# 30stomercury/whisper-char-alignment

Measured on AMD Instinct MI355X. Metric: utterances/sec (whisper-medium, 10s audio, char align) at 1/2/4/8 MI355X, higher is better.
Workload: dtype f16x2 (hi + lo operand pairs on the f16 MFMA pipe: fp32-equivalent operands, fp32 accumulate)

## Files before the change

### include/wca.h

```cpp
#ifndef WCA_H_
#define WCA_H_

#include <stdint.h>

#ifdef __cplusplus
extern "C" {
#endif

typedef struct wca_engine wca_engine;

typedef enum {
  WCA_STATUS_PARTITIONED = 1,
  WCA_OK = 0,
  WCA_ERR_INVALID = -1,
  WCA_ERR_TOO_LONG = -2,
  WCA_ERR_HIP = -3,
  WCA_ERR_STATE = -4,
  WCA_ERR_NOMEM = -5
} wca_status;

typedef struct {
  int32_t n_mels;
  int32_t n_audio_ctx;
  int32_t n_audio_state;
// ... 73 lines not shown
                    int32_t* jump_frame_host);
int wca_probe_strict_tp(wca_engine* e, int n_heads, const int32_t* word_end_row_host, int n_hyp, const double* ref_times_host, int n_ref,
                        const uint8_t* same_word_host, double tolerance, int32_t* tp_host);

int wca_align_batch(wca_engine* e, const float* pcm_dev, int64_t pcm_stride, const int32_t* n_samples_host,
                    const int64_t* tokens_dev, int n_tok_max, const int32_t* n_tok_host,
                    const int32_t* max_frames_host, int batch, const wca_align_opts* opts, int32_t* jump_frame_host,
                    int32_t* sel_idx_host);

typedef struct {
  int32_t sample_len;
  int32_t eot;
  int32_t timestamp_begin;
  int32_t apply_timestamp_rules;
  int32_t max_initial_timestamp_index;
  int32_t no_speech;
} wca_decode_opts;

typedef struct {
  int32_t sample_len;
  int32_t eot;
  int32_t timestamp_begin;
  int32_t apply_timestamp_rules;
  int32_t max_initial_timestamp_index;
  int32_t no_speech;
  int32_t sot_index;
  int32_t prefill;
} wca_decode_opts_ex;

int wca_encode_batch(wca_engine* e, const float* mel_dev, const float* pcm_dev, int64_t pcm_stride,
                     const int32_t* n_samples_host, int batch);

int wca_greedy_decode(wca_engine* e, const float* mel_dev, const float* pcm_dev, int64_t pcm_stride,
                      const int32_t* n_samples_host, int batch, const int32_t* initial_tokens_host, int n_initial,
                      const uint8_t* suppress_mask_host, const uint8_t* blank_mask_host, const wca_decode_opts* opts,
                      int32_t* tokens_out_host, int32_t* n_tokens_host, float* sum_logprob_host,
                      float* no_speech_prob_host);
int wca_greedy_decode_ex(wca_engine* e, const float* mel_dev, const float* pcm_dev, int64_t pcm_stride,
                         const int32_t* n_samples_host, int batch, const int32_t* initial_tokens_host, int n_initial,
                         const uint8_t* suppress_mask_host, const uint8_t* blank_mask_host, const wca_decode_opts_ex* opts,
                         int32_t* tokens_out_host, int32_t* n_tokens_host, float* sum_logprob_host,
                         float* no_speech_prob_host);
int wca_last_decode_positions(wca_engine* e, int32_t* prefill_positions, int32_t* step_positions);

int wca_align_batch_enqueue(wca_engine* e, const float* pcm_dev, int64_t pcm_stride, const int32_t* n_samples_host,
                            const int64_t* tokens_dev, int n_tok_max, const int32_t* n_tok_host,
                            const int32_t* max_frames_host, int batch, const wca_align_opts* opts);
int wca_align_batch_fetch(wca_engine* e, int batch, int n_tok_max, int topk, int32_t* jump_frame_host,
                          int32_t* sel_idx_host);

int wca_align_batch_enqueue_ex(wca_engine* e, const float* pcm_dev, int64_t pcm_stride, const int32_t* n_samples_host,
                               const int64_t* tokens_dev, int n_tok_max, const int32_t* n_tok_host,
                               const int32_t* max_frames_host, int batch, const wca_align_opts* opts, int32_t vocab_end);
int wca_align_batch_fetch_ex(wca_engine* e, int batch, int n_tok_max, int topk, int32_t* jump_frame_host,
                             int32_t* sel_idx_host, float* token_logprob_host);
int wca_token_logprobs(wca_engine* e, const float* logits_dev, int rows, int ld, int vocab_end, const int64_t* targets_dev,
                       float* out_dev);

int wca_flac_info(const uint8_t* buf, int64_t nbytes, int32_t* sample_rate, int32_t* channels, int32_t* bits_per_sample,
                  int64_t* total_samples);
int wca_flac_decode(const uint8_t* buf, int64_t nbytes, float* out, int64_t capacity_per_channel, int64_t* n_decoded);

#define WCA_COMM_ID_BYTES 128
int wca_comm_unique_id(uint8_t* id_out );
int wca_comm_init(wca_engine* e, const uint8_t* id , int rank, int world);
int wca_comm_destroy(wca_engine* e);
int wca_allgather_results(wca_engine* e, const uint8_t* packed_host, int64_t n_bytes, uint8_t* gathered_host,
                          int64_t capacity_per_rank, int64_t* sizes_host );
int wca_allreduce_counters(wca_engine* e, int64_t* counters_host , int n);
int wca_collate_plan(const int64_t* sizes , const int64_t* capacities , int world, int64_t* pad_out);

int wca_test_gemm(wca_engine* e, const void* a_f16_dev, const void* w_f16_dev, const float* bias_dev, void* c_dev, int M,
                  int N, int K, int gelu, int out_mode);
int wca_test_gemm_pairs(wca_engine* e, const void* a2_f16_dev, const void* w_f16_dev, const float* bias_dev, void* c_dev, int M,
                        int N, int K, int gelu, int out_mode);
int wca_test_gemm_ln(wca_engine* e, const void* a_f16_dev, const void* w_f16_dev, const float* bias_dev, float* x_dev,
                     const float* gamma_dev, const float* beta_dev, void* xn_f16_dev, int M, int N, int K, int site);
int wca_test_gemm_rows(wca_engine* e, const void* a_f16_dev, const float* x_f32_dev, const float* gamma_dev, const float* beta_dev,
                       const void* w_f16_dev, const float* bias_dev, void* c_dev, int M, int N, int K, int gelu, int out_mode, int splitk,
                       int groups, void* kv_k_f16_dev, void* kv_v_f16_dev, int T_max, int kv_t);
int wca_test_set_attn_split_drop(int mask);
int wca_test_set_switch(const char* name, int value);
int wca_test_last_scores(wca_engine* e, int batch, float* scores_host);
int wca_test_attention(wca_engine* e, const void* q_dev, const void* k_dev, const void* v_dev, void* o_dev,
                       float* cap_dev, int cap_ld, int cap_cols, int B, int H, int nq, int nk, int causal);
int wca_test_attention_split(wca_engine* e, const void* q2_dev, const void* k2_dev, const void* v2_dev, void* o2_dev,
                             float* cap_dev, int cap_ld, int cap_cols, int B, int H, int nq, int nk, int causal);
int wca_test_decode_select(wca_engine* e, const float* logits_dev, int batch, int n_vocab, int32_t* tokens_dev, int T_max,
                           int cur_len, int n_initial, const uint8_t* suppress_mask_dev, const uint8_t* blank_mask_dev,
                           const wca_decode_opts* opts, float* sum_logprob_dev, int32_t* n_done_dev);
int wca_test_layernorm(wca_engine* e, const float* x_dev, const float* g_dev, const float* b_dev, void* out_f16_dev,
                       int rows, int d);
int wca_test_layernorm_split(wca_engine* e, const float* x_dev, const float* g_dev, const float* b_dev, void* out2_f16_dev,
                             int rows, int d);
int wca_test_encoder(wca_engine* e, const float* mel_dev, int batch, float* xa_out_dev);

int wca_last_stage_ms(wca_engine* e, float* ms8);
enum {
  WCA_SITE_QKV = 0,
  WCA_SITE_ATTN = 1,
  WCA_SITE_OUT = 2,
  WCA_SITE_FC1 = 3,
  WCA_SITE_FC2 = 4,
  WCA_SITE_LN1 = 5,
  WCA_SITE_LN2 = 6,
  WCA_N_SITES = 7
};
int wca_last_kernel_ms(wca_engine* e, int site, int* n_launches, float* total_ms, double* flops_per_launch,
                       double* bytes_per_launch);
int wca_set_fuse_ln(wca_engine* e, int on);
enum { WCA_PRECISION_F16 = 0, WCA_PRECISION_SPLIT = 1, WCA_PRECISION_REFERENCE = 1 };
int wca_set_precision(wca_engine* e, int mode);
int wca_get_precision(wca_engine* e);
int wca_set_overlap(wca_engine* e, int on);
int wca_set_cu_partition(wca_engine* e, int phase2_cus);
int wca_set_decode_mode(wca_engine* e, int fused, int streams);
int wca_set_profiling(wca_engine* e, int on);

#ifdef __cplusplus
}
#endif
#endif
```

### whisper-char-alignment_amd/_lib.py

```python
import ctypes as C
import os

_HERE = os.path.dirname(os.path.abspath(__file__))
LIB_PATH = os.path.join(_HERE, "libwca.so")


class WcaError(RuntimeError):
    def __init__(self, code, msg):
        super().__init__("wca error %d: %s" % (code, msg))
        self.code = code


class TooLongError(WcaError):
    """n_tok > 448 or max_frames > 1500 (the skip condition of infer_ali.py:79)."""


class ModelDims(C.Structure):
    _fields_ = [(n, C.c_int32) for n in (
        "n_mels", "n_audio_ctx", "n_audio_state", "n_audio_head", "n_audio_layer",
        "n_vocab", "n_text_ctx", "n_text_state", "n_text_head", "n_text_layer")]


class AlignOpts(C.Structure):
    _fields_ = [("aggregation", C.c_int32), ("topk", C.c_int32), ("w_colnorm", C.c_float),
                ("w_rownorm", C.c_float), ("w_coverage", C.c_float), ("sot_len", C.c_int32),
                ("medfilt_width", C.c_int32), ("qk_scale", C.c_float)]


class DecodeOpts(C.Structure):
    _fields_ = [("sample_len", C.c_int32), ("eot", C.c_int32), ("timestamp_begin", C.c_int32),
                ("apply_timestamp_rules", C.c_int32), ("max_initial_timestamp_index", C.c_int32), ("no_speech", C.c_int32)]


class DecodeOptsEx(C.Structure):
    _fields_ = DecodeOpts._fields_ + [("sot_index", C.c_int32), ("prefill", C.c_int32)]


ERR_TOO_LONG = -2
AGGR_MEAN, AGGR_TOPK = 0, 1
PRECISION_SITES = ("logmel", "conv", "enc_gemm", "enc_attn", "cross_kv", "dec", "capture")
SITES = {"qkv": 0, "attention": 1, "out_proj": 2, "fc1": 3, "fc2": 4, "ln1": 5, "ln2": 6}
DTYPE_F32, DTYPE_F16 = 0, 1

_vp, _i, _i64, _f = C.c_void_p, C.c_int, C.c_int64, C.c_float
_pi32 = C.POINTER(C.c_int32)
_pf = C.POINTER(C.c_float)

SIGNATURES = {
    "wca_last_error": (C.c_char_p, []),
    "wca_version": (_i, []),
    "wca_engine_create": (_i, [C.POINTER(ModelDims), _i, _i, C.POINTER(_vp)]),
    "wca_engine_create_ex": (_i, [C.POINTER(ModelDims), _i, _i, _i, C.POINTER(_vp)]),
    "wca_engine_destroy": (None, [_vp]),
    "wca_engine_set_stream": (_i, [_vp, _vp]),
    "wca_engine_synchronize": (_i, [_vp]),
    "wca_load_weight": (_i, [_vp, C.c_char_p, _vp, _i, C.POINTER(_i64), _i]),
    "wca_finalize_weights": (_i, [_vp]),
    "wca_weights_inexact": (_i, [_vp, C.POINTER(C.c_longlong), C.POINTER(C.c_longlong), C.c_char_p, _i]),
    "wca_set_allow_rounded_weights": (_i, [_vp, _i]),
    "wca_log_mel": (_i, [_vp, _vp, _i64, _pi32, _i, _vp]),
    "wca_log_mel_long": (_i, [_vp, _vp, _i64, _vp, _i64, C.POINTER(_i64)]),
    "wca_mel_window": (_i, [_vp, _vp, _i64, _i64, _pi32, _pi32, _i, _vp]),
    "wca_get_attentions": (_i, [_vp, _vp, _vp, _i, _i, _pi32, _pi32, _i, _f, _vp, _vp]),
    "wca_median_filter": (_i, [_vp, _vp, _vp, _i64, _i, _i]),
    "wca_filter_attention": (_i, [_vp, _vp, _i, _i, _i, _i, _i, _f, _f, _f, _pf, _pi32, _pf]),
    "wca_force_align": (_i, [_vp, _vp, _i, _i, _i, _i, C.POINTER(AlignOpts), _pf, _pi32, _pi32, _pi32, _pi32, _pf]),
    "wca_default_find_alignment": (_i, [_vp, _vp, _i, _i, _i, _i, _pi32, _i, _i, _vp, _pf, _pi32, _pi32, _pi32]),
    "wca_attention_weights": (_i, [_vp, _vp, _i, _i, _i, _i, _i, _i, _f, _vp]),
    "wca_flac_info": (_i, [_vp, _i64, _pi32, _pi32, _pi32, C.POINTER(_i64)]),
    "wca_flac_decode": (_i, [_vp, _i64, _vp, _i64, C.POINTER(_i64)]),
    "wca_dtw": (_i, [_vp, _pf, _i, _i, _pi32, _pi32, _pi32]),
    "wca_dtw_batch_dev": (_i, [_vp, _vp, _i, _i, _i, _pi32]),
    "wca_probe_heads": (_i, [_vp, _vp, _i, _i, _i, _i, _i, _pf, _pi32]),
    "wca_align_batch": (_i, [_vp, _vp, _i64, _pi32, _vp, _i, _pi32, _pi32, _i, C.POINTER(AlignOpts), _pi32, _pi32]),
    "wca_align_batch_enqueue": (_i, [_vp, _vp, _i64, _pi32, _vp, _i, _pi32, _pi32, _i, C.POINTER(AlignOpts)]),
    "wca_align_batch_fetch": (_i, [_vp, _i, _i, _i, _pi32, _pi32]),
    "wca_align_batch_enqueue_ex": (_i, [_vp, _vp, _i64, _pi32, _vp, _i, _pi32, _pi32, _i, C.POINTER(AlignOpts), C.c_int32]),
    "wca_align_batch_fetch_ex": (_i, [_vp, _i, _i, _i, _pi32, _pi32, _pf]),
    "wca_token_logprobs": (_i, [_vp, _vp, _i, _i, _i, _vp, _vp]),
    "wca_encode_batch": (_i, [_vp, _vp, _vp, _i64, _pi32, _i]),
    "wca_greedy_decode": (_i, [_vp, _vp, _vp, _i64, _pi32, _i, _pi32, _i, _vp, _vp, C.POINTER(DecodeOpts), _pi32, _pi32, _pf, _pf]),
    "wca_greedy_decode_ex": (_i, [_vp, _vp, _vp, _i64, _pi32, _i, _pi32, _i, _vp, _vp, C.POINTER(DecodeOptsEx), _pi32, _pi32, _pf, _pf]),
    "wca_last_decode_positions": (_i, [_vp, _pi32, _pi32]),
    "wca_test_decode_select": (_i, [_vp, _vp, _i, _i, _vp, _i, _i, _i, _vp, _vp, C.POINTER(DecodeOpts), _vp, _vp]),
    "wca_test_gemm": (_i, [_vp, _vp, _vp, _vp, _vp, _i, _i, _i, _i, _i]),
    "wca_test_gemm_ln": (_i, [_vp, _vp, _vp, _vp, _vp, _vp, _vp, _vp, _i, _i, _i, _i]),
    "wca_test_set_attn_split_drop": (_i, [_i]),
    "wca_test_set_switch": (_i, [C.c_char_p, _i]),
    "wca_test_last_scores": (_i, [_vp, _i, _pf]),
    "wca_test_gemm_pairs": (_i, [_vp, _vp, _vp, _vp, _vp, _i, _i, _i, _i, _i]),
    "wca_test_attention": (_i, [_vp, _vp, _vp, _vp, _vp, _vp, _i, _i, _i, _i, _i, _i, _i]),
    "wca_test_attention_split": (_i, [_vp, _vp, _vp, _vp, _vp, _vp, _i, _i, _i, _i, _i, _i, _i]),
    "wca_test_layernorm": (_i, [_vp, _vp, _vp, _vp, _vp, _i, _i]),
    "wca_test_layernorm_split": (_i, [_vp, _vp, _vp, _vp, _vp, _i, _i]),
    "wca_test_encoder": (_i, [_vp, _vp, _i, _vp]),
    "wca_last_stage_ms": (_i, [_vp, _pf]),
    "wca_set_profiling": (_i, [_vp, _i]),
    "wca_last_kernel_ms": (_i, [_vp, _i, C.POINTER(C.c_int), _pf, C.POINTER(C.c_double), C.POINTER(C.c_double)]),
    "wca_set_overlap": (_i, [_vp, _i]),
    "wca_set_cu_partition": (_i, [_vp, _i]),
    "wca_set_fuse_ln": (_i, [_vp, _i]),
    "wca_set_precision": (_i, [_vp, _i]),
    "wca_get_precision": (_i, [_vp]),
    "wca_set_decode_mode": (_i, [_vp, _i, _i]),
    "wca_comm_unique_id": (_i, [_vp]),
    "wca_comm_init": (_i, [_vp, _vp, _i, _i]),
    "wca_comm_destroy": (_i, [_vp]),
    "wca_allgather_results": (_i, [_vp, _vp, _i64, _vp, _i64, C.POINTER(_i64)]),
    "wca_allreduce_counters": (_i, [_vp, C.POINTER(_i64), _i]),
    "wca_collate_plan": (_i, [C.POINTER(_i64), C.POINTER(_i64), _i, C.POINTER(_i64)]),
    "wca_probe_strict_tp": (_i, [_vp, _i, _vp, _i, _vp, _i, _vp, C.c_double, _vp]),
    "wca_test_gemm_rows": (_i, [_vp, _vp, _vp, _vp, _vp, _vp, _vp, _vp, _i, _i, _i, _i, _i, _i, _i, _vp, _vp, _i, _i]),
}

_lib = None


def load():
    global _lib
    if _lib is not None:
        return _lib
    if not os.path.exists(LIB_PATH):
        raise ImportError(
            "libwca.so not found at %s: build it with `python whisper-char-alignment_amd/build.py` "
            "(or __graft_entry__.build()). The alignment engine has no CPU fallback." % LIB_PATH)
    lib = C.CDLL(LIB_PATH)
    for name, (res, args) in SIGNATURES.items():
        fn = getattr(lib, name)
        fn.restype = res
        fn.argtypes = args
    _lib = lib
    return lib


def check(code):
    if code == 0:
        return
    msg = load().wca_last_error()
    msg = msg.decode("utf-8", "replace") if msg else ""
    if code == -2:
        raise TooLongError(code, msg)
    raise WcaError(code, msg)


def i32_array(values):
    arr = (C.c_int32 * len(values))(*[int(v) for v in values])
    return arr
```

### whisper-char-alignment_amd/csrc/attention.hip

```cpp
#include <cstdlib>

#include "kernels.h"
#include "wca_common.h"

namespace wca {

namespace {

constexpr int KT = 64;
constexpr int TILE = 64 * 64;
constexpr float LOG2E = 1.4426950408889634f;
constexpr float RESCALE_THR = 8.0f;

__device__ __forceinline__ float xor16_max(float v) {
  const unsigned u = __float_as_uint(v);
  auto r = __builtin_amdgcn_permlane16_swap(u, u, false, false);
  return fmaxf(__uint_as_float(r[0]), __uint_as_float(r[1]));
}
__device__ __forceinline__ float xor32_max(float v) {
  const unsigned u = __float_as_uint(v);
  auto r = __builtin_amdgcn_permlane32_swap(u, u, false, false);
  return fmaxf(__uint_as_float(r[0]), __uint_as_float(r[1]));
}

__device__ __forceinline__ half4 tr_read4(const half_t* p) {
  s16x4 r = __builtin_amdgcn_ds_read_tr16_b64_v4i16((WCA_LDS s16x4*)(p));
  return __builtin_bit_cast(half4, r);
}

__device__ __forceinline__ unsigned lds_off(const void* p) { return (unsigned)(size_t)(const WCA_LDS char*)p; }
template <int OFF>
__device__ __forceinline__ half8 lds_read_b128_asm(unsigned addr) {
  half8 r;
  asm volatile("ds_read_b128 %0, %1 offset:%2" : "=v"(r) : "v"(addr), "i"(OFF));
  return r;
}
template <int OFF>
__device__ __forceinline__ half4 lds_read_tr_asm(unsigned addr) {
  half4 r;
  asm volatile("ds_read_b64_tr_b16 %0, %1 offset:%2" : "=v"(r) : "v"(addr), "i"(OFF));
  return r;
}
#define WCA_LGKM_WAIT4(N, A, B, C, D)                                                                         \
  do {                                                                                                        \
    asm volatile("s_waitcnt lgkmcnt(" #N ")" : "+v"(A), "+v"(B), "+v"(C), "+v"(D)::"memory");              \
    __builtin_amdgcn_sched_barrier(0);                                                                        \
  } while (0)
#define WCA_LGKM_WAIT8(N, A, B, C, D, E, F, G, H)                                                             \
  do {                                                                                                        \
    asm volatile("s_waitcnt lgkmcnt(" #N ")" : "+v"(A), "+v"(B), "+v"(C), "+v"(D), "+v"(E), "+v"(F), "+v"(G), "+v"(H)::"memory"); \
    __builtin_amdgcn_sched_barrier(0);                                                                        \
  } while (0)

template <bool CAUSAL, bool CAPTURE>
__global__ __launch_bounds__(256) void attn_kernel(AttnArgs a) {
  extern __shared__ __attribute__((aligned(16))) char smem[];
  half_t* lds = reinterpret_cast<half_t*>(smem);
  const int tid = threadIdx.x;
  const int lane = tid & 63;
  const int wave = __builtin_amdgcn_readfirstlane(tid >> 6);
  const int fr = lane & 15, fg = lane >> 4;
  const int n_qt = (a.nq + 127) / 128;
  const int lid = xcd_remap(blockIdx.x, n_qt * a.H * a.B);
  const int bh = lid / n_qt;
  const int b = bh / a.H, h = bh - b * a.H;
  const int q_blk = (lid - bh * n_qt) * 128;
  const int q_wave = q_blk + wave * 32;

  half8 qf[2][2];
  int qrow[2];
#pragma unroll
  for (int sub = 0; sub < 2; ++sub) {
    qrow[sub] = q_wave + sub * 16 + fr;
    const int qc = qrow[sub] < a.nq ? qrow[sub] : a.nq - 1;
    const half_t* qp = a.Q + (long)b * a.q_bs + (long)qc * a.q_rs + h * 64 + fg * 8;
    qf[sub][0] = *reinterpret_cast<const half8*>(qp);
    qf[sub][1] = *reinterpret_cast<const half8*>(qp + 32);
  }

  constexpr bool LAZY = !CAPTURE;
  const float c_log2 = a.scale * LOG2E;
  if (LAZY) {
#pragma unroll
    for (int sub = 0; sub < 2; ++sub)
#pragma unroll
      for (int ks = 0; ks < 2; ++ks)
#pragma unroll
        for (int j = 0; j < 8; ++j) qf[sub][ks][j] = (half_t)((float)qf[sub][ks][j] * c_log2);
  }

  int nk_eff = a.nk;
  if (CAUSAL) {
    const int qhi = q_blk + 128;
    nk_eff = qhi < a.nk ? qhi : a.nk;
  }
  const int nkt = (nk_eff + KT - 1) / KT;

  const half_t* Kb = a.K + (long)b * a.k_bs + h * 64;
  const half_t* Vb = a.V + (long)b * a.v_bs + h * 64;

  auto stage = [&](int buf, int kt) {
    half_t* Kt = lds + buf * (2 * TILE);
    half_t* Vt = Kt + TILE;
#pragma unroll
    for (int i = 0; i < 2; ++i) {
      const int rbase = (wave * 2 + i) * 8;
      const int r = rbase + (lane >> 3);
      int key = kt * KT + r;
      key = key < a.nk ? key : a.nk - 1;
      const int ck = (lane & 7) ^ swz128(r);
      const int cv = (lane & 7) ^ (r & 6);
      glds16(Kb + (long)key * a.k_rs + ck * 8, Kt + rbase * 64);
      glds16(Vb + (long)key * a.v_rs + cv * 8, Vt + rbase * 64);
    }
  };

  f32x4 ot[2][4];
#pragma unroll
  for (int s = 0; s < 2; ++s)
#pragma unroll
    for (int d = 0; d < 4; ++d) ot[s][d] = f32x4{0.f, 0.f, 0.f, 0.f};
  half8 ones;
#pragma unroll
  for (int j = 0; j < 8; ++j) ones[j] = (half_t)1.0f;
  float m_run[2] = {-INFINITY, -INFINITY};
  float l_run[2] = {0.f, 0.f};

  stage(0, 0);
  if (nkt > 1) stage(1, 1);
  int slot = 0;
  for (int kt = 0; kt < nkt; ++kt) {
    if (kt + 1 < nkt) {
      asm volatile("s_waitcnt vmcnt(4)" ::: "memory");
    } else {
      asm volatile("s_waitcnt vmcnt(0)" ::: "memory");
    }
    __builtin_amdgcn_s_barrier();
    asm volatile("" ::: "memory");
    if (kt + 2 < nkt) {
      int nslot = slot + 2;
      nslot = nslot >= 3 ? nslot - 3 : nslot;
      stage(nslot, kt + 2);
    }
    const half_t* Kt = lds + slot * (2 * TILE);
    const half_t* Vt = Kt + TILE;
    slot = (slot == 2) ? 0 : slot + 1;

    f32x4 st[2][4];
    {
      half8 kf0[4], kf1[4];
#pragma unroll
      for (int t = 0; t < 4; ++t) {
        const int r = t * 16 + fr;
        kf0[t] = *reinterpret_cast<const half8*>(Kt + r * 64 + (((0 + fg) ^ swz128(r)) << 3));
        kf1[t] = *reinterpret_cast<const half8*>(Kt + r * 64 + (((4 + fg) ^ swz128(r)) << 3));
      }
      f32x4 cinit[2];
#pragma unroll
      for (int s = 0; s < 2; ++s) {
        const float c0 = (LAZY && m_run[s] != -INFINITY) ? -m_run[s] : 0.f;
        cinit[s] = f32x4{c0, c0, c0, c0};
      }
#pragma unroll
      for (int s = 0; s < 2; ++s)
#pragma unroll
        for (int t = 0; t < 4; ++t) st[s][t] = __builtin_amdgcn_mfma_f32_16x16x32_f16(kf0[t], qf[s][0], cinit[s], 0, 0, 0);
#pragma unroll
      for (int s = 0; s < 2; ++s)
#pragma unroll
        for (int t = 0; t < 4; ++t) st[s][t] = __builtin_amdgcn_mfma_f32_16x16x32_f16(kf1[t], qf[s][1], st[s][t], 0, 0, 0);
    }

    if (CAPTURE) {
#pragma unroll
      for (int s = 0; s < 2; ++s) {
        if (qrow[s] < a.nq) {
#pragma unroll
          for (int t = 0; t < 4; ++t) {
            const int key4 = kt * KT + t * 16 + 4 * fg;
            if (key4 < a.cap_cols) {
              float* cp = a.cap + (long)b * a.cap_bs + (long)h * a.cap_hs + (long)qrow[s] * a.cap_ld + key4;
              *reinterpret_cast<f32x4*>(cp) = st[s][t] * a.scale;
            }
          }
        }
      }
    }
    const bool tail_tile = (kt * KT + KT > a.nk);
    const bool diag_tile = CAUSAL && (kt * KT + KT - 1 > q_wave);
    if (tail_tile || diag_tile) {
#pragma unroll
      for (int s = 0; s < 2; ++s)
#pragma unroll
        for (int t = 0; t < 4; ++t)
#pragma unroll
          for (int r = 0; r < 4; ++r) {
            const int key = kt * KT + t * 16 + 4 * fg + r;
            bool dead = key >= a.nk;
            if (CAUSAL) dead = dead || (key > qrow[s]);
            st[s][t][r] = dead ? -INFINITY : st[s][t][r];
          }
    }
    float mx[2];
#pragma unroll
    for (int s = 0; s < 2; ++s) {
      float m = st[s][0][0];
#pragma unroll
      for (int t = 0; t < 4; ++t)
#pragma unroll
        for (int r = 0; r < 4; r += 2) m = fmaxf(fmaxf(m, st[s][t][r]), st[s][t][r + 1]);
      mx[s] = m;
    }
#pragma unroll
    for (int s = 0; s < 2; ++s) mx[s] = xor16_max(mx[s]);
#pragma unroll
    for (int s = 0; s < 2; ++s) mx[s] = xor32_max(mx[s]);
    if (LAZY) {
      if (__any((mx[0] > RESCALE_THR) || (mx[1] > RESCALE_THR) || (m_run[0] == -INFINITY && mx[0] != -INFINITY) ||
                (m_run[1] == -INFINITY && mx[1] != -INFINITY))) {
#pragma unroll
        for (int s = 0; s < 2; ++s) {
          const float m_eff = (m_run[s] == -INFINITY) ? 0.f : m_run[s];
          const float m_new = fmaxf(m_run[s], mx[s] + m_eff);
          const float delta = (m_new == -INFINITY) ? 0.f : m_new - m_eff;
          const float alpha = (m_run[s] == -INFINITY) ? 1.0f : __builtin_amdgcn_exp2f(m_run[s] - m_new);
          l_run[s] *= alpha;
#pragma unroll
          for (int d = 0; d < 4; ++d) ot[s][d] *= alpha;
#pragma unroll
          for (int t = 0; t < 4; ++t)
#pragma unroll
            for (int r = 0; r < 4; ++r) st[s][t][r] -= delta;
          m_run[s] = m_new;
        }
      }
#pragma unroll
      for (int s = 0; s < 2; ++s)
#pragma unroll
        for (int t = 0; t < 4; ++t)
#pragma unroll
          for (int r = 0; r < 4; ++r) st[s][t][r] = __builtin_amdgcn_exp2f(st[s][t][r]);
    } else {
    if (__any((mx[0] > m_run[0]) || (mx[1] > m_run[1]))) {
#pragma unroll
      for (int s = 0; s < 2; ++s) {
        const float m_new = fmaxf(m_run[s], mx[s]);
        const float alpha = (m_new == -INFINITY) ? 1.0f : __builtin_amdgcn_exp2f((m_run[s] - m_new) * c_log2);
        l_run[s] *= alpha;
#pragma unroll
        for (int d = 0; d < 4; ++d) ot[s][d] *= alpha;
        m_run[s] = m_new;
      }
    }
    float mc[2];
#pragma unroll
    for (int s = 0; s < 2; ++s) mc[s] = (m_run[s] == -INFINITY) ? 0.f : m_run[s] * c_log2;
#pragma unroll
    for (int s = 0; s < 2; ++s)
#pragma unroll
      for (int t = 0; t < 4; ++t)
#pragma unroll
        for (int r = 0; r < 4; ++r) st[s][t][r] = __builtin_amdgcn_exp2f(fmaf(st[s][t][r], c_log2, -mc[s]));
    }
    half8 pf[2][2];
#pragma unroll
    for (int s = 0; s < 2; ++s)
#pragma unroll
      for (int k2 = 0; k2 < 2; ++k2) {
        half8 f;
#pragma unroll
        for (int r = 0; r < 4; ++r) {
          f[r] = (half_t)st[s][2 * k2][r];
          f[4 + r] = (half_t)st[s][2 * k2 + 1][r];
        }
        pf[s][k2] = f;
      }
#pragma unroll
    for (int s = 0; s < 2; ++s) {
      f32x4 rsum = __builtin_amdgcn_mfma_f32_16x16x32_f16(ones, pf[s][0], f32x4{0.f, 0.f, 0.f, 0.f}, 0, 0, 0);
      rsum = __builtin_amdgcn_mfma_f32_16x16x32_f16(ones, pf[s][1], rsum, 0, 0, 0);
      l_run[s] += rsum[0];
    }

    {
      const int qd = fr >> 2, pd = fr & 3;
#pragma unroll
      for (int dt = 0; dt < 4; ++dt) {
        const int d = dt * 16 + 4 * pd;
        const int c = d >> 3, w = d & 7;
#pragma unroll
        for (int k2 = 0; k2 < 2; ++k2) {
          const int key0 = (2 * k2) * 16 + 4 * fg + qd;
          const int key1 = key0 + 16;
          const half4 v0 = tr_read4(Vt + key0 * 64 + ((c ^ (key0 & 6)) << 3) + w);
          const half4 v1 = tr_read4(Vt + key1 * 64 + ((c ^ (key1 & 6)) << 3) + w);
          half8 vf;
#pragma unroll
          for (int r = 0; r < 4; ++r) {
            vf[r] = v0[r];
            vf[4 + r] = v1[r];
          }
#pragma unroll
          for (int s = 0; s < 2; ++s)
            ot[s][dt] = __builtin_amdgcn_mfma_f32_16x16x32_f16(vf, pf[s][k2], ot[s][dt], 0, 0, 0);
        }
      }
    }
  }

#pragma unroll
  for (int s = 0; s < 2; ++s) {
    if (qrow[s] >= a.nq) continue;
    const float inv = 1.0f / l_run[s];
    half_t* op = a.O + (long)b * a.o_bs + (long)qrow[s] * a.o_rs + h * 64 + 4 * fg;
#pragma unroll
    for (int dt = 0; dt < 4; ++dt) {
      half4 o;
#pragma unroll
      for (int r = 0; r < 4; ++r) o[r] = (half_t)(ot[s][dt][r] * inv);
      *reinterpret_cast<half4*>(op + dt * 16) = o;
    }
  }
}


typedef float f32x16 __attribute__((ext_vector_type(16)));

__device__ __forceinline__ float max3f(float a, float b, float c) { return fmaxf(fmaxf(a, b), c); }

template <int V>
struct IntC {
  static constexpr int value = V;
};

__global__ __launch_bounds__(256) void attn32_kernel(AttnArgs a) {
  constexpr int NW = 4;
  extern __shared__ __attribute__((aligned(16))) char smem[];
  half_t* lds = reinterpret_cast<half_t*>(smem);
  const int tid = threadIdx.x;
  const int lane = tid & 63;
  const int wave = __builtin_amdgcn_readfirstlane(tid >> 6);
  const int l31 = lane & 31, hh = lane >> 5;
  constexpr int QB = NW * 32;
  constexpr int SLOT_BYTES = 2 * TILE * (int)sizeof(half_t);
  const int n_qt = (a.nq + QB - 1) / QB;
  const int lid = xcd_remap(blockIdx.x, n_qt * a.H * a.B);
  const int bh = lid / n_qt;
  const int b = bh / a.H, h = bh - b * a.H;
  const int q_wave = (lid - bh * n_qt) * QB + wave * 32;
  const int qrow = q_wave + l31;

  const float c_log2 = a.scale * LOG2E;
  half8 qf[4];
  {
    const int qc = qrow < a.nq ? qrow : a.nq - 1;
    const half_t* qp = a.Q + (long)b * a.q_bs + (long)qc * a.q_rs + h * 64 + hh * 8;
#pragma unroll
    for (int ks = 0; ks < 4; ++ks) {
      const half8 raw = *reinterpret_cast<const half8*>(qp + ks * 16);
#pragma unroll
      for (int j = 0; j < 8; ++j) qf[ks][j] = (half_t)((float)raw[j] * c_log2);
    }
  }
  const int nkt = (a.nk + KT - 1) / KT;
  const __amdgpu_buffer_rsrc_t rk = __builtin_amdgcn_make_buffer_rsrc(const_cast<half_t*>(a.K + (long)b * a.k_bs + h * 64), 0,
                                                                      (int)(((long)(a.nk - 1) * a.k_rs + 64) * 2), 0x00020000);
  const __amdgpu_buffer_rsrc_t rv = __builtin_amdgcn_make_buffer_rsrc(const_cast<half_t*>(a.V + (long)b * a.v_bs + h * 64), 0,
                                                                      (int)(((long)(a.nk - 1) * a.v_rs + 64) * 2), 0x00020000);
  unsigned dk[8 / NW], dv[8 / NW];
#pragma unroll
  for (int i = 0; i < 8 / NW; ++i) {
    const int r = (wave * (8 / NW) + i) * 8 + (lane >> 3);
    dk[i] = (unsigned)(r * a.k_rs * 2 + (((lane & 7) ^ ((r >> 1) & 7)) << 4));
    dv[i] = (unsigned)(r * a.v_rs * 2 + (((lane & 7) ^ ((r & 2) << 1)) << 4));
  }
  const unsigned k_tile_bytes = (unsigned)(KT * a.k_rs * 2), v_tile_bytes = (unsigned)(KT * a.v_rs * 2);
  auto stage = [&](int buf, int kt) {
    half_t* Kt = lds + buf * (2 * TILE);
    half_t* Vt = Kt + TILE;
#pragma unroll
    for (int i = 0; i < 8 / NW; ++i) {
      const int rbase = (wave * (8 / NW) + i) * 8;
      __builtin_amdgcn_raw_ptr_buffer_load_lds(rk, (WCA_LDS void*)(Kt + rbase * 64), 16, (int)dk[i], (int)(kt * k_tile_bytes), 0, 0);
      __builtin_amdgcn_raw_ptr_buffer_load_lds(rv, (WCA_LDS void*)(Vt + rbase * 64), 16, (int)dv[i], (int)(kt * v_tile_bytes), 0, 0);
    }
  };

  const int kswz = (l31 >> 1) & 7;
  const unsigned lds_base = lds_off(lds);
  unsigned ka[4];
#pragma unroll
  for (int ks = 0; ks < 4; ++ks) ka[ks] = lds_base + (unsigned)(l31 * 128 + 16 * ((hh ^ kswz) & 1) + 32 * (ks ^ (kswz >> 1)));
// ... 207 lines not shown
    bool live[U];
#pragma unroll
    for (int u = 0; u < U; ++u) {
      const int key = k0 + u * 8 + grp;
      live[u] = key < k_hi;
      const int kc = live[u] ? key : a.nk - 1;
      kf[u] = *reinterpret_cast<const half8*>(Kb + (long)kc * a.k_rs);
      vf[u] = *reinterpret_cast<const half8*>(Vb + (long)kc * a.v_rs);
    }
    float sc[U];
#pragma unroll
    for (int u = 0; u < U; ++u) {
      float d = 0.f;
#pragma unroll
      for (int j = 0; j < 8; ++j) d = fmaf(q[j], (float)kf[u][j], d);
      d += __shfl_xor(d, 1);
      d += __shfl_xor(d, 2);
      d += __shfl_xor(d, 4);
      sc[u] = live[u] ? d : -INFINITY;
    }
    float mb = sc[0];
#pragma unroll
    for (int u = 1; u < U; ++u) mb = fmaxf(mb, sc[u]);
    const float m_new = fmaxf(m, mb);
    if (m_new != -INFINITY) {
      const float alpha = (m == -INFINITY) ? 0.f : __builtin_amdgcn_exp2f(m - m_new);
      l *= alpha;
#pragma unroll
      for (int j = 0; j < 8; ++j) o[j] *= alpha;
#pragma unroll
      for (int u = 0; u < U; ++u) {
        const float p = __builtin_amdgcn_exp2f(sc[u] - m_new);
        l += p;
#pragma unroll
        for (int j = 0; j < 8; ++j) o[j] = fmaf(p, (float)vf[u][j], o[j]);
      }
      m = m_new;
    }
  }
#pragma unroll
  for (int off = 8; off <= 32; off <<= 1) {
    const float m2 = __shfl_xor(m, off), l2 = __shfl_xor(l, off);
    const float mn = fmaxf(m, m2);
    const float a1 = (m == -INFINITY) ? 0.f : __builtin_amdgcn_exp2f(m - mn);
    const float a2 = (m2 == -INFINITY) ? 0.f : __builtin_amdgcn_exp2f(m2 - mn);
    l = l * a1 + l2 * a2;
#pragma unroll
    for (int j = 0; j < 8; ++j) o[j] = o[j] * a1 + __shfl_xor(o[j], off) * a2;
    m = mn;
  }
  if (lane < 8) {
    if (lane == 0) {
      part[wave][0] = m;
      part[wave][1] = l;
    }
#pragma unroll
    for (int j = 0; j < 8; ++j) part[wave][2 + lane * 8 + j] = o[j];
  }
  __syncthreads();
  if (tid < 64) {
    float mn = part[0][0];
#pragma unroll
    for (int w = 1; w < 4; ++w) mn = fmaxf(mn, part[w][0]);
    float lt = 0.f, ov = 0.f;
#pragma unroll
    for (int w = 0; w < 4; ++w) {
      const float aw = (part[w][0] == -INFINITY) ? 0.f : __builtin_amdgcn_exp2f(part[w][0] - mn);
      lt += part[w][1] * aw;
      ov += part[w][2 + tid] * aw;
    }
    a.O[(long)b * a.o_bs + h * 64 + tid] = (half_t)(ov / lt);
  }
}

}

hipError_t launch_attention(const AttnArgs& a, hipStream_t s) {
  if (a.split) return launch_attention_split(a, s);
  if (a.nq <= 0 || a.B <= 0) return hipSuccess;
  if (a.nk <= 0) return hipErrorInvalidValue;
  if ((a.q_rs % 8) || (a.k_rs % 8) || (a.v_rs % 8) || (a.o_rs % 4)) return hipErrorInvalidValue;
  if (a.cap != nullptr && ((a.cap_ld % 4) != 0 || a.cap_ld < ((a.cap_cols + 3) & ~3))) return hipErrorInvalidValue;
  const bool cap = a.cap != nullptr && a.cap_cols > 0;
  if (a.nq == 1 && !cap && (!a.causal || a.nk == 1)) {
    hipLaunchKernelGGL(attn_decode_kernel, dim3(a.H * a.B), dim3(256), 0, s, a);
    return hipGetLastError();
  }
  dim3 grid(((a.nq + 127) / 128) * a.H * a.B), block(256);
  const size_t shmem = 3 * 2 * TILE * sizeof(half_t);
  const bool use32 = !a.causal && !cap && (a.o_rs % 8) == 0 && a.variant != 1 && (a.nq >= 64 || a.variant == 2);
  if (use32) {
    hipLaunchKernelGGL(attn32_kernel, grid, block, shmem, s, a);
    return hipGetLastError();
  }
  if (a.causal) {
    if (cap) hipLaunchKernelGGL((attn_kernel<true, true>), grid, block, shmem, s, a);
    else hipLaunchKernelGGL((attn_kernel<true, false>), grid, block, shmem, s, a);
  } else {
    if (cap) hipLaunchKernelGGL((attn_kernel<false, true>), grid, block, shmem, s, a);
    else hipLaunchKernelGGL((attn_kernel<false, false>), grid, block, shmem, s, a);
  }
  return hipGetLastError();
}

}
```

### whisper-char-alignment_amd/csrc/attention_split.hip

```cpp
#include <cstdlib>

#include "kernels.h"
#include "wca_common.h"

namespace wca {

namespace {

constexpr int KT = 64;
constexpr int TILE = 64 * 64;
constexpr float LOG2E = 1.4426950408889634f;

__device__ __forceinline__ float xor16_maxf(float v) {
  const unsigned u = __float_as_uint(v);
  auto r = __builtin_amdgcn_permlane16_swap(u, u, false, false);
  return fmaxf(__uint_as_float(r[0]), __uint_as_float(r[1]));
}
__device__ __forceinline__ float xor32_maxf(float v) {
  const unsigned u = __float_as_uint(v);
  auto r = __builtin_amdgcn_permlane32_swap(u, u, false, false);
  return fmaxf(__uint_as_float(r[0]), __uint_as_float(r[1]));
}
__device__ __forceinline__ float xor16_sumf(float v) {
  const unsigned u = __float_as_uint(v);
  auto r = __builtin_amdgcn_permlane16_swap(u, u, false, false);
  return __uint_as_float(r[0]) + __uint_as_float(r[1]);
}
__device__ __forceinline__ float xor32_sumf(float v) {
  const unsigned u = __float_as_uint(v);
  auto r = __builtin_amdgcn_permlane32_swap(u, u, false, false);
  return __uint_as_float(r[0]) + __uint_as_float(r[1]);
}

__device__ __forceinline__ unsigned lds_off_s(const void* p) { return (unsigned)(size_t)(const WCA_LDS char*)p; }
template <int OFF>
__device__ __forceinline__ half4 tr_read_asm(unsigned addr) {
  half4 r;
  asm volatile("ds_read_b64_tr_b16 %0, %1 offset:%2" : "=v"(r) : "v"(addr), "i"(OFF));
  return r;
}
template <int OFF>
__device__ __forceinline__ half8 b128_read_asm(unsigned addr) {
  half8 r;
  asm volatile("ds_read_b128 %0, %1 offset:%2" : "=v"(r) : "v"(addr), "i"(OFF));
  return r;
}
#define WCA_S_LGKM_WAIT4(N, A, B, C, D)                                                                       \
  do {                                                                                                        \
    asm volatile("s_waitcnt lgkmcnt(" #N ")" : "+v"(A), "+v"(B), "+v"(C), "+v"(D)::"memory");              \
    __builtin_amdgcn_sched_barrier(0);                                                                        \
  } while (0)
#define WCA_S_LGKM_WAIT8(N, A, B, C, D, E, F, G, H)                                                                                  \
  do {                                                                                                                               \
    asm volatile("s_waitcnt lgkmcnt(" #N ")" : "+v"(A), "+v"(B), "+v"(C), "+v"(D), "+v"(E), "+v"(F), "+v"(G), "+v"(H)::"memory");  \
    __builtin_amdgcn_sched_barrier(0);                                                                                               \
  } while (0)

template <bool CAUSAL, bool CAPTURE, int NW = 4>
__global__ __launch_bounds__(NW * 64, (2 * NW * 64) / 256) void attn_split_kernel(AttnArgs a) {
  extern __shared__ __attribute__((aligned(16))) char smem[];
  half_t* lds = reinterpret_cast<half_t*>(smem);
  const int tid = threadIdx.x;
  const int lane = tid & 63;
  const int wave = __builtin_amdgcn_readfirstlane(tid >> 6);
  const int fr = lane & 15, fg = lane >> 4;
  constexpr int QB = NW * 32;
  const int n_qt = (a.nq + QB - 1) / QB;
  const int lid = xcd_remap(blockIdx.x, n_qt * a.H * a.B);
  const int bh = lid / n_qt;
  const int b = bh / a.H, h = bh - b * a.H;
  const int q_blk = (lid - bh * n_qt) * QB;
  const int q_wave = q_blk + wave * 32;

  half8 qh[2][2], ql[2][2];
  int qrow[2];
#pragma unroll
  for (int sub = 0; sub < 2; ++sub) {
    qrow[sub] = q_wave + sub * 16 + fr;
    const int qc = qrow[sub] < a.nq ? qrow[sub] : a.nq - 1;
    const half_t* qp = a.Q + (long)b * a.q_bs + (long)qc * a.q_rs + h * 64 + fg * 8;
    qh[sub][0] = *reinterpret_cast<const half8*>(qp);
    qh[sub][1] = *reinterpret_cast<const half8*>(qp + 32);
    ql[sub][0] = *reinterpret_cast<const half8*>(qp + a.q_lo);
    ql[sub][1] = *reinterpret_cast<const half8*>(qp + a.q_lo + 32);
  }
  const float c_log2 = a.scale * LOG2E;
  constexpr bool PRE = !CAPTURE;
  if (PRE) {
#pragma unroll
    for (int sub = 0; sub < 2; ++sub)
#pragma unroll
      for (int ks = 0; ks < 2; ++ks)
#pragma unroll
        for (int j = 0; j < 8; ++j) {
          const HalfPair pr = split_pair(((float)qh[sub][ks][j] + (float)ql[sub][ks][j]) * c_log2);
          qh[sub][ks][j] = pr.hi;
          ql[sub][ks][j] = pr.lo;
        }
  }
  const float cm = PRE ? 1.0f : c_log2;

  int nk_eff = a.nk;
  if (CAUSAL) {
    const int qhi = q_blk + QB;
    nk_eff = qhi < a.nk ? qhi : a.nk;
  }
  const int nkt = (nk_eff + KT - 1) / KT;

  const half_t* Kb = a.K + (long)b * a.k_bs + h * 64;
  const half_t* Vb = a.V + (long)b * a.v_bs + h * 64;

  auto stage = [&](int buf, int kt) {
    half_t* Kh = lds + buf * (4 * TILE);
    half_t* Kl = Kh + TILE;
    half_t* Vh = Kl + TILE;
    half_t* Vl = Vh + TILE;
#pragma unroll
    for (int i = 0; i < (8 + NW - 1) / NW; ++i) {
      const int piece = wave + NW * i;
      if (piece >= 8) break;
      const int rbase = piece * 8;
      const int r = rbase + (lane >> 3);
      int key = kt * KT + r;
      key = key < a.nk ? key : a.nk - 1;
      const int ck = (lane & 7) ^ swz128(r);
      const int cv = (lane & 7) ^ (r & 6);
      const half_t* kp = Kb + (long)key * a.k_rs + ck * 8;
      const half_t* vp = Vb + (long)key * a.v_rs + cv * 8;
      glds16(kp, Kh + rbase * 64);
      glds16(kp + a.k_lo, Kl + rbase * 64);
      glds16(vp, Vh + rbase * 64);
      glds16(vp + a.v_lo, Vl + rbase * 64);
    }
  };

  f32x4 ot[2][4];
#pragma unroll
  for (int s = 0; s < 2; ++s)
#pragma unroll
    for (int d = 0; d < 4; ++d) ot[s][d] = f32x4{0.f, 0.f, 0.f, 0.f};
  unsigned vaddr[4];
  {
    const int qd = fr >> 2, pd = fr & 3;
    const int swz = (4 * (fg & 1)) | (qd & 2);
#pragma unroll
    for (int dt = 0; dt < 4; ++dt)
      vaddr[dt] = lds_off_s(lds) + 2u * (unsigned)((4 * fg + qd) * 64 + (((2 * dt + (pd >> 1)) ^ swz) << 3) + 4 * (pd & 1));
  }
  unsigned kaddr[2][4];
#pragma unroll
  for (int ks = 0; ks < 2; ++ks)
#pragma unroll
    for (int t = 0; t < 4; ++t) {
      const int r = t * 16 + fr;
      kaddr[ks][t] = lds_off_s(lds) + 2u * (unsigned)(r * 64 + (((ks * 4 + fg) ^ swz128(r)) << 3));
    }
  float m_run[2] = {-INFINITY, -INFINITY};
  float l_part[2] = {0.f, 0.f};

  stage(0, 0);
  for (int kt = 0; kt < nkt; ++kt) {
    wait_vm0();
    __builtin_amdgcn_s_barrier();
    asm volatile("" ::: "memory");
    if (kt + 1 < nkt) stage((kt + 1) & 1, kt + 1);
    f32x4 st[2][4];
#pragma unroll
    for (int s = 0; s < 2; ++s)
#pragma unroll
      for (int t = 0; t < 4; ++t) st[s][t] = f32x4{0.f, 0.f, 0.f, 0.f};
    {
      constexpr int KLO = TILE * (int)sizeof(half_t);
      const unsigned sbk = (unsigned)(kt & 1) * (unsigned)(4 * TILE * sizeof(half_t));
      half8 kh[2][4], kl[2][4];
#pragma unroll
      for (int ks = 0; ks < 2; ++ks) {
#pragma unroll
        for (int t = 0; t < 4; ++t) kl[ks][t] = b128_read_asm<KLO>(kaddr[ks][t] + sbk);
#pragma unroll
        for (int t = 0; t < 4; ++t) kh[ks][t] = b128_read_asm<0>(kaddr[ks][t] + sbk);
      }
      WCA_S_LGKM_WAIT4(12, kl[0][0], kl[0][1], kl[0][2], kl[0][3]);
#pragma unroll
      for (int s = 0; s < 2; ++s)
#pragma unroll
        for (int t = 0; t < 4; ++t) st[s][t] = __builtin_amdgcn_mfma_f32_16x16x32_f16(kl[0][t], qh[s][0], st[s][t], 0, 0, 0);
      WCA_S_LGKM_WAIT4(8, kh[0][0], kh[0][1], kh[0][2], kh[0][3]);
#pragma unroll
      for (int s = 0; s < 2; ++s)
#pragma unroll
        for (int t = 0; t < 4; ++t) st[s][t] = __builtin_amdgcn_mfma_f32_16x16x32_f16(kh[0][t], ql[s][0], st[s][t], 0, 0, 0);
#pragma unroll
      for (int s = 0; s < 2; ++s)
#pragma unroll
        for (int t = 0; t < 4; ++t) st[s][t] = __builtin_amdgcn_mfma_f32_16x16x32_f16(kh[0][t], qh[s][0], st[s][t], 0, 0, 0);
      WCA_S_LGKM_WAIT4(4, kl[1][0], kl[1][1], kl[1][2], kl[1][3]);
#pragma unroll
      for (int s = 0; s < 2; ++s)
#pragma unroll
        for (int t = 0; t < 4; ++t) st[s][t] = __builtin_amdgcn_mfma_f32_16x16x32_f16(kl[1][t], qh[s][1], st[s][t], 0, 0, 0);
      WCA_S_LGKM_WAIT4(0, kh[1][0], kh[1][1], kh[1][2], kh[1][3]);
#pragma unroll
      for (int s = 0; s < 2; ++s)
#pragma unroll
        for (int t = 0; t < 4; ++t) st[s][t] = __builtin_amdgcn_mfma_f32_16x16x32_f16(kh[1][t], ql[s][1], st[s][t], 0, 0, 0);
#pragma unroll
      for (int s = 0; s < 2; ++s)
#pragma unroll
        for (int t = 0; t < 4; ++t) st[s][t] = __builtin_amdgcn_mfma_f32_16x16x32_f16(kh[1][t], qh[s][1], st[s][t], 0, 0, 0);
    }

    if (CAPTURE) {
#pragma unroll
      for (int s = 0; s < 2; ++s) {
        if (qrow[s] < a.nq) {
#pragma unroll
          for (int t = 0; t < 4; ++t) {
            const int key4 = kt * KT + t * 16 + 4 * fg;
            if (key4 < a.cap_cols) {
              float* cp = a.cap + (long)b * a.cap_bs + (long)h * a.cap_hs + (long)qrow[s] * a.cap_ld + key4;
              *reinterpret_cast<f32x4*>(cp) = st[s][t] * a.scale;
            }
          }
        }
      }
    }
    const bool tail_tile = (kt * KT + KT > a.nk);
    const bool diag_tile = CAUSAL && (kt * KT + KT - 1 > q_wave);
    if (tail_tile || diag_tile) {
#pragma unroll
      for (int s = 0; s < 2; ++s)
#pragma unroll
        for (int t = 0; t < 4; ++t)
#pragma unroll
          for (int r = 0; r < 4; ++r) {
            const int key = kt * KT + t * 16 + 4 * fg + r;
            bool dead = key >= a.nk;
            if (CAUSAL) dead = dead || (key > qrow[s]);
            st[s][t][r] = dead ? -INFINITY : st[s][t][r];
          }
    }
    float mx[2];
#pragma unroll
    for (int s = 0; s < 2; ++s) {
      float m = fmaxf(fmaxf(st[s][0][0], st[s][0][1]), fmaxf(st[s][0][2], st[s][0][3]));
#pragma unroll
      for (int t = 1; t < 4; ++t) {
        m = fmaxf(fmaxf(m, st[s][t][0]), st[s][t][1]);
        m = fmaxf(fmaxf(m, st[s][t][2]), st[s][t][3]);
      }
      mx[s] = xor32_maxf(xor16_maxf(m));
    }
    const float thr_raw = 8.0f / cm;
    if (__any((mx[0] > m_run[0] + thr_raw) || (mx[1] > m_run[1] + thr_raw) || (m_run[0] == -INFINITY && mx[0] != -INFINITY) ||
              (m_run[1] == -INFINITY && mx[1] != -INFINITY))) {
#pragma unroll
      for (int s = 0; s < 2; ++s) {
        const float m_new = fmaxf(m_run[s], mx[s]);
        const float alpha = (m_run[s] == -INFINITY) ? 1.0f : __builtin_amdgcn_exp2f((m_run[s] - m_new) * cm);
        l_part[s] *= alpha;
#pragma unroll
        for (int d = 0; d < 4; ++d) ot[s][d] *= alpha;
        m_run[s] = m_new;
      }
    }
    half8 ph[2][2], pl[2][2];
#pragma unroll
    for (int s = 0; s < 2; ++s) {
      const float mref = (m_run[s] == -INFINITY) ? 0.f : m_run[s];
      const f32x2 mm = f32x2{mref, mref};
      f32x2 psum2 = f32x2{0.f, 0.f};
#pragma unroll
      for (int k2 = 0; k2 < 2; ++k2) {
        half2_ hh[4], ll[4];
#pragma unroll
        for (int u = 0; u < 4; ++u) {
          const int t = 2 * k2 + (u >> 1), r0 = 2 * (u & 1);
          f32x2 x = f32x2{st[s][t][r0], st[s][t][r0 + 1]} - mm;
          if (!PRE) x = x * f32x2{cm, cm};
          const f32x2 p = f32x2{__builtin_amdgcn_exp2f(x[0]), __builtin_amdgcn_exp2f(x[1])};
          psum2 += p;
          hh[u] = __builtin_convertvector(p, half2_);
          {
            const unsigned hu = __builtin_bit_cast(unsigned, hh[u]);
            unsigned lu;
            asm("v_fma_mixlo_f16 %0, %1, 1.0, -%2 op_sel:[0,0,0] op_sel_hi:[0,0,1]" : "=v"(lu) : "v"(p[0]), "v"(hu));
            asm("v_fma_mixhi_f16 %0, %1, 1.0, -%2 op_sel:[0,0,1] op_sel_hi:[0,0,1]" : "+v"(lu) : "v"(p[1]), "v"(hu));
            ll[u] = __builtin_bit_cast(half2_, lu);
          }
        }
        ph[s][k2] = half8{hh[0][0], hh[0][1], hh[1][0], hh[1][1], hh[2][0], hh[2][1], hh[3][0], hh[3][1]};
        pl[s][k2] = half8{ll[0][0], ll[0][1], ll[1][0], ll[1][1], ll[2][0], ll[2][1], ll[3][0], ll[3][1]};
      }
      l_part[s] += psum2[0] + psum2[1];
    }

    {
      const unsigned sb = (unsigned)(kt & 1) * (unsigned)(4 * TILE * sizeof(half_t));
      constexpr int VH = 2 * TILE * (int)sizeof(half_t), VL = 3 * TILE * (int)sizeof(half_t);
      constexpr int K2 = 32 * 64 * (int)sizeof(half_t), B16 = 16 * 64 * (int)sizeof(half_t);
      half4 c_[8], n_[8];
#define WCA_ISSUE_V(R, A)                                                                    \
  do {                                                                                       \
    R[0] = tr_read_asm<VH>(A);                                                               \
    R[1] = tr_read_asm<VH + B16>(A);                                                         \
    R[2] = tr_read_asm<VL>(A);                                                               \
    R[3] = tr_read_asm<VL + B16>(A);                                                         \
    R[4] = tr_read_asm<VH + K2>(A);                                                          \
    R[5] = tr_read_asm<VH + K2 + B16>(A);                                                    \
    R[6] = tr_read_asm<VL + K2>(A);                                                          \
    R[7] = tr_read_asm<VL + K2 + B16>(A);                                                    \
  } while (0)
      WCA_ISSUE_V(c_, vaddr[0] + sb);
#pragma unroll
      for (int dt = 0; dt < 4; ++dt) {
        if (dt < 3) {
          WCA_ISSUE_V(n_, vaddr[dt + 1] + sb);
          WCA_S_LGKM_WAIT8(8, c_[0], c_[1], c_[2], c_[3], c_[4], c_[5], c_[6], c_[7]);
        } else {
          WCA_S_LGKM_WAIT8(0, c_[0], c_[1], c_[2], c_[3], c_[4], c_[5], c_[6], c_[7]);
        }
#pragma unroll
        for (int k2 = 0; k2 < 2; ++k2) {
          const half8 vh = __builtin_shufflevector(c_[4 * k2], c_[4 * k2 + 1], 0, 1, 2, 3, 4, 5, 6, 7);
          const half8 vl = __builtin_shufflevector(c_[4 * k2 + 2], c_[4 * k2 + 3], 0, 1, 2, 3, 4, 5, 6, 7);
#pragma unroll
          for (int s = 0; s < 2; ++s) {
            ot[s][dt] = __builtin_amdgcn_mfma_f32_16x16x32_f16(vl, ph[s][k2], ot[s][dt], 0, 0, 0);
            ot[s][dt] = __builtin_amdgcn_mfma_f32_16x16x32_f16(vh, pl[s][k2], ot[s][dt], 0, 0, 0);
            ot[s][dt] = __builtin_amdgcn_mfma_f32_16x16x32_f16(vh, ph[s][k2], ot[s][dt], 0, 0, 0);
          }
        }
        if (dt < 3) {
#pragma unroll
          for (int i = 0; i < 8; ++i) c_[i] = n_[i];
        }
      }
#undef WCA_ISSUE_V
    }
  }

#pragma unroll
  for (int s = 0; s < 2; ++s) {
    const float l = xor32_sumf(xor16_sumf(l_part[s]));
    if (qrow[s] >= a.nq) continue;
    const float inv = 1.0f / l;
    half_t* op = a.O + (long)b * a.o_bs + (long)qrow[s] * a.o_rs + h * 64 + 4 * fg;
#pragma unroll
    for (int dt = 0; dt < 4; ++dt) {
      half4 oh, ol;
#pragma unroll
      for (int r = 0; r < 4; ++r) {
        const HalfPair pr = split_pair(ot[s][dt][r] * inv);
        oh[r] = pr.hi;
        ol[r] = pr.lo;
      }
      *reinterpret_cast<half4*>(op + dt * 16) = oh;
      *reinterpret_cast<half4*>(op + a.o_lo + dt * 16) = ol;
    }
  }
}



typedef float f32x16 __attribute__((ext_vector_type(16)));
constexpr float RESCALE_THR32 = 8.0f;

__device__ __forceinline__ float max3f_(float a, float b, float c) { return fmaxf(fmaxf(a, b), c); }
template <int V>
struct IntC32 {
  static constexpr int value = V;
};
#define WCA_S_PIN8(A, B, C, D, E, F, G, H) asm volatile("" : "+v"(A), "+v"(B), "+v"(C), "+v"(D), "+v"(E), "+v"(F), "+v"(G), "+v"(H)::"memory")

template <int DROP>
__global__ __launch_bounds__(256, 2) void attn_split32_kernel(AttnArgs a) {
  constexpr int NW = 4;
  extern __shared__ __attribute__((aligned(16))) char smem[];
  half_t* lds = reinterpret_cast<half_t*>(smem);
  const int tid = threadIdx.x;
  const int lane = tid & 63;
  const int wave = __builtin_amdgcn_readfirstlane(tid >> 6);
  const int l31 = lane & 31, hh = lane >> 5;
  constexpr int QB = NW * 32;
  constexpr int TB = TILE * (int)sizeof(half_t);
  constexpr int SLOT_BYTES = 4 * TB;
  const int n_qt = (a.nq + QB - 1) / QB;
  const int lid = xcd_remap(blockIdx.x, n_qt * a.H * a.B);
  const int bh = lid / n_qt;
  const int b = bh / a.H, h = bh - b * a.H;
  const int q_wave = (lid - bh * n_qt) * QB + wave * 32;
  const int qrow = q_wave + l31;
  const float c_log2 = a.scale * LOG2E;
  half8 qh[4], ql[4];
  {
    const int qc = qrow < a.nq ? qrow : a.nq - 1;
    const half_t* qp = a.Q + (long)b * a.q_bs + (long)qc * a.q_rs + h * 64 + hh * 8;
#pragma unroll
    for (int ks = 0; ks < 4; ++ks) {
      const half8 rh = *reinterpret_cast<const half8*>(qp + ks * 16);
      const half8 rl = *reinterpret_cast<const half8*>(qp + a.q_lo + ks * 16);
#pragma unroll
      for (int j = 0; j < 8; ++j) {
        const HalfPair pr = split_pair(((float)rh[j] + (float)rl[j]) * c_log2);
        qh[ks][j] = pr.hi;
        ql[ks][j] = pr.lo;
      }
    }
  }
  const int nkt = (a.nk + KT - 1) / KT;
  const int kbytes = (int)(((long)(a.nk - 1) * a.k_rs + 64) * 2), vbytes = (int)(((long)(a.nk - 1) * a.v_rs + 64) * 2);
  const half_t* Kb = a.K + (long)b * a.k_bs + h * 64;
  const half_t* Vb = a.V + (long)b * a.v_bs + h * 64;
  const __amdgpu_buffer_rsrc_t rkh = __builtin_amdgcn_make_buffer_rsrc(const_cast<half_t*>(Kb), 0, kbytes, 0x00020000);
  const __amdgpu_buffer_rsrc_t rkl = __builtin_amdgcn_make_buffer_rsrc(const_cast<half_t*>(Kb + a.k_lo), 0, kbytes, 0x00020000);
  const __amdgpu_buffer_rsrc_t rvh = __builtin_amdgcn_make_buffer_rsrc(const_cast<half_t*>(Vb), 0, vbytes, 0x00020000);
  const __amdgpu_buffer_rsrc_t rvl = __builtin_amdgcn_make_buffer_rsrc(const_cast<half_t*>(Vb + a.v_lo), 0, vbytes, 0x00020000);
  unsigned dk[2], dv[2];
#pragma unroll
  for (int i = 0; i < 2; ++i) {
    const int r = (wave * 2 + i) * 8 + (lane >> 3);
    dk[i] = (unsigned)(r * a.k_rs * 2 + (((lane & 7) ^ ((r >> 1) & 7)) << 4));
    dv[i] = (unsigned)(r * a.v_rs * 2 + (((lane & 7) ^ ((r & 2) << 1)) << 4));
  }
// ... 183 lines not shown
          const f32x2 p = f32x2{__builtin_amdgcn_exp2f(st[s4 >> 1][r0]), __builtin_amdgcn_exp2f(st[s4 >> 1][r0 + 1])};
          psum += p;
          hq[u] = __builtin_convertvector(p, half2_);
          const unsigned hu = __builtin_bit_cast(unsigned, hq[u]);
          unsigned lu;
          asm("v_fma_mixlo_f16 %0, %1, 1.0, -%2 op_sel:[0,0,0] op_sel_hi:[0,0,1]" : "=v"(lu) : "v"(p[0]), "v"(hu));
          asm("v_fma_mixhi_f16 %0, %1, 1.0, -%2 op_sel:[0,0,1] op_sel_hi:[0,0,1]" : "+v"(lu) : "v"(p[1]), "v"(hu));
          lq[u] = __builtin_bit_cast(half2_, lu);
        }
        ph[s4] = half8{hq[0][0], hq[0][1], hq[1][0], hq[1][1], hq[2][0], hq[2][1], hq[3][0], hq[3][1]};
        pl[s4] = half8{lq[0][0], lq[0][1], lq[1][0], lq[1][1], lq[2][0], lq[2][1], lq[3][0], lq[3][1]};
      }
      l_run += psum[0] + psum[1];
    }
    WCA_S_LGKM_WAIT8(0, v0ha[0], v0hb[0], v0ha[1], v0hb[1], v0ha[2], v0hb[2], v0ha[3], v0hb[3]);
    WCA_S_PIN8(v0la[0], v0lb[0], v0la[1], v0lb[1], v0la[2], v0lb[2], v0la[3], v0lb[3]);
    WCA_ISSUE_V32(v1, 1);
#pragma unroll
    for (int s4 = 0; s4 < 4; ++s4) {
      const half8 wh = __builtin_shufflevector(v0ha[s4], v0hb[s4], 0, 1, 2, 3, 4, 5, 6, 7);
      const half8 wl = __builtin_shufflevector(v0la[s4], v0lb[s4], 0, 1, 2, 3, 4, 5, 6, 7);
      if (!(DROP & 4)) ot[0] = __builtin_amdgcn_mfma_f32_32x32x16_f16(wl, ph[s4], ot[0], 0, 0, 0);
      if (!(DROP & 8)) ot[0] = __builtin_amdgcn_mfma_f32_32x32x16_f16(wh, pl[s4], ot[0], 0, 0, 0);
      ot[0] = __builtin_amdgcn_mfma_f32_32x32x16_f16(wh, ph[s4], ot[0], 0, 0, 0);
    }
    WCA_S_LGKM_WAIT8(0, v1ha[0], v1hb[0], v1ha[1], v1hb[1], v1ha[2], v1hb[2], v1ha[3], v1hb[3]);
    WCA_S_PIN8(v1la[0], v1lb[0], v1la[1], v1lb[1], v1la[2], v1lb[2], v1la[3], v1lb[3]);
#pragma unroll
    for (int s4 = 0; s4 < 4; ++s4) {
      const half8 wh = __builtin_shufflevector(v1ha[s4], v1hb[s4], 0, 1, 2, 3, 4, 5, 6, 7);
      const half8 wl = __builtin_shufflevector(v1la[s4], v1lb[s4], 0, 1, 2, 3, 4, 5, 6, 7);
      if (!(DROP & 4)) ot[1] = __builtin_amdgcn_mfma_f32_32x32x16_f16(wl, ph[s4], ot[1], 0, 0, 0);
      if (!(DROP & 8)) ot[1] = __builtin_amdgcn_mfma_f32_32x32x16_f16(wh, pl[s4], ot[1], 0, 0, 0);
      ot[1] = __builtin_amdgcn_mfma_f32_32x32x16_f16(wh, ph[s4], ot[1], 0, 0, 0);
    }
#undef WCA_ISSUE_V32
  };
  for (int kt = 0; kt < nkt; kt += 2) {
    tile(IntC32<0>{}, kt);
    if (kt + 1 < nkt) tile(IntC32<1>{}, kt + 1);
  }

  const float inv = 1.0f / xor32_sumf(l_run);
  half_t* op = a.O + (long)b * a.o_bs + (long)qrow * a.o_rs + h * 64;
#pragma unroll
  for (int db = 0; db < 2; ++db)
#pragma unroll
    for (int g2 = 0; g2 < 2; ++g2) {
      unsigned wh[2][2], wl[2][2];
#pragma unroll
      for (int e = 0; e < 2; ++e)
#pragma unroll
        for (int k2 = 0; k2 < 2; ++k2) {
          const Half2Pair pr = split_pair2(ot[db][4 * (2 * g2 + e) + 2 * k2] * inv, ot[db][4 * (2 * g2 + e) + 2 * k2 + 1] * inv);
          wh[e][k2] = __builtin_bit_cast(unsigned, pr.hi);
          wl[e][k2] = __builtin_bit_cast(unsigned, pr.lo);
        }
      typedef unsigned u32x4 __attribute__((ext_vector_type(4)));
      u32x4 oh, ol;
      {
        auto r0 = __builtin_amdgcn_permlane32_swap(wh[0][0], wh[1][0], false, false);
        auto r1 = __builtin_amdgcn_permlane32_swap(wh[0][1], wh[1][1], false, false);
        oh = u32x4{r0[0], r1[0], r0[1], r1[1]};
        auto s0 = __builtin_amdgcn_permlane32_swap(wl[0][0], wl[1][0], false, false);
        auto s1 = __builtin_amdgcn_permlane32_swap(wl[0][1], wl[1][1], false, false);
        ol = u32x4{s0[0], s1[0], s0[1], s1[1]};
      }
      if (qrow < a.nq) {
        *reinterpret_cast<u32x4*>(op + 32 * db + 16 * g2 + 8 * hh) = oh;
        *reinterpret_cast<u32x4*>(op + a.o_lo + 32 * db + 16 * g2 + 8 * hh) = ol;
      }
    }
}

}

hipError_t launch_attention_split(const AttnArgs& a, hipStream_t s) {
  if (a.nq <= 0 || a.B <= 0) return hipSuccess;
  if (a.nk <= 0) return hipErrorInvalidValue;
  if ((a.q_rs % 8) || (a.k_rs % 8) || (a.v_rs % 8) || (a.o_rs % 4)) return hipErrorInvalidValue;
  if ((a.q_lo % 8) || (a.k_lo % 8) || (a.v_lo % 8) || (a.o_lo % 4) || a.q_lo <= 0 || a.k_lo <= 0 || a.v_lo <= 0 || a.o_lo <= 0) return hipErrorInvalidValue;
  if (a.cap != nullptr && ((a.cap_ld % 4) != 0 || a.cap_ld < ((a.cap_cols + 3) & ~3))) return hipErrorInvalidValue;
  const bool cap = a.cap != nullptr && a.cap_cols > 0;
  const size_t shmem = 2 * 4 * TILE * sizeof(half_t);
#define WCA_LAUNCH_AS(C, P, W)                                                                                               \
  do {                                                                                                                       \
    hipError_t e = hipFuncSetAttribute(reinterpret_cast<const void*>(attn_split_kernel<C, P, W>),                            \
                                       hipFuncAttributeMaxDynamicSharedMemorySize, (int)shmem);                             \
    if (e != hipSuccess) return e;                                                                                           \
    hipLaunchKernelGGL((attn_split_kernel<C, P, W>), dim3(((a.nq + (W) * 32 - 1) / ((W) * 32)) * a.H * a.B), dim3((W) * 64), shmem, s, a); \
  } while (0)
  const int variant = a.variant ? a.variant : debug_switch(DBG_ATTN_SPLIT_VARIANT);
  if (!a.causal && !cap && a.nq >= 64 && variant != 1 && (a.o_rs % 8) == 0 && (a.o_lo % 8) == 0) {
#define WCA_LAUNCH_A32(D)                                                                                                             \
  do {                                                                                                                                \
    hipError_t e = hipFuncSetAttribute(reinterpret_cast<const void*>(attn_split32_kernel<D>), hipFuncAttributeMaxDynamicSharedMemorySize, (int)shmem); \
    if (e != hipSuccess) return e;                                                                                                    \
    hipLaunchKernelGGL(attn_split32_kernel<D>, dim3(((a.nq + 127) / 128) * a.H * a.B), dim3(256), shmem, s, a);                       \
  } while (0)
    switch (debug_switch(DBG_ATTN_SPLIT_DROP)) {
      case 0: WCA_LAUNCH_A32(0); break;
      case 1: WCA_LAUNCH_A32(1); break;
      case 2: WCA_LAUNCH_A32(2); break;
      case 3: WCA_LAUNCH_A32(3); break;
      case 4: WCA_LAUNCH_A32(4); break;
      case 8: WCA_LAUNCH_A32(8); break;
      case 9: WCA_LAUNCH_A32(9); break;
      case 12: WCA_LAUNCH_A32(12); break;
      case 15: WCA_LAUNCH_A32(15); break;
      default: return hipErrorInvalidValue;
    }
#undef WCA_LAUNCH_A32
    return hipGetLastError();
  }
  if (a.causal) {
    if (cap) WCA_LAUNCH_AS(true, true, 4); else WCA_LAUNCH_AS(true, false, 4);
  } else {
    if (cap) WCA_LAUNCH_AS(false, true, 4); else WCA_LAUNCH_AS(false, false, 4);
  }
#undef WCA_LAUNCH_AS
  return hipGetLastError();
}

}
```

### whisper-char-alignment_amd/csrc/engine.hip

```cpp
#include <hip/hip_runtime.h>
#include <dlfcn.h>
#include <rccl/rccl.h>

#include <chrono>
#include <cmath>
#include <cstdarg>
#include <cstdio>
#include <cstdlib>
#include <cstring>
#include <deque>
#include <map>
#include <set>
#include <string>
#include <vector>

#include "../../include/wca.h"
#include "kernels.h"

using namespace wca;

namespace {

thread_local std::string g_err;

// ... 337 lines not shown
  e->sw.conv2_w = carve<half_t>(cur, d * 6 * d);
  e->sw.conv1_wlo = carve<half_t>(cur, d * e->sw.k1pad);
  e->sw.conv2_wlo = carve<half_t>(cur, d * 6 * d);
  e->sw.enc.assign(D.n_audio_layer, LayerW{});
  for (auto& l : e->sw.enc) {
    l.qkv_w = carve<half_t>(cur, 3 * d * 2 * d);
    l.out_w = carve<half_t>(cur, d * 2 * d);
    l.fc1_w = carve<half_t>(cur, 4 * d * 2 * d);
    l.fc2_w = carve<half_t>(cur, d * 8 * d);
  }
  e->sw.tok_emb = carve<half_t>(cur, (size_t)D.n_vocab * 2 * dt);
  e->sw.kv_w = carve<half_t>(cur, (size_t)D.n_text_layer * 2 * dt * 2 * d);
  e->sw.dec.assign(D.n_text_layer, LayerW{});
  for (auto& l : e->sw.dec) {
    l.qkv_w = carve<half_t>(cur, 3 * dt * 2 * dt);
    l.out_w = carve<half_t>(cur, dt * 2 * dt);
    l.cq_w = carve<half_t>(cur, dt * 2 * dt);
    l.co_w = carve<half_t>(cur, dt * 2 * dt);
    l.fc1_w = carve<half_t>(cur, 4 * dt * 2 * dt);
    l.fc2_w = carve<half_t>(cur, dt * 8 * dt);
  }
  return (size_t)(cur - base) + 4096;
}

__global__ void dup_cols_kernel(const half_t* __restrict__ src, int ld_src, half_t* __restrict__ dst, int ld_dst, long N, int K, int grp, int second_zero) {
  const long i = (long)blockIdx.x * blockDim.x + threadIdx.x;
  if (i >= N * K) return;
  const long n = i / K;
  const int j = (int)(i - n * K);
  const half_t v = src[n * ld_src + j];
  const int g = j / grp, c = j - g * grp;
  half_t* o = dst + n * ld_dst + (long)g * 2 * grp + c;
  o[0] = v;
  o[grp] = second_zero ? (half_t)0.f : v;
}

int dup_cols(hipStream_t s, const half_t* src, int ld_src, half_t* dst, int ld_dst, long N, int K, int grp, int second_zero = 0) {
  const long tot = N * K;
  hipLaunchKernelGGL(dup_cols_kernel, dim3((unsigned)((tot + 255) / 256)), dim3(256), 0, s, src, ld_src, dst, ld_dst, N, K, grp, second_zero);
  HIPCHK(hipGetLastError());
  return WCA_OK;
}

int ensure_split_weights(wca_engine* e) {
  if (!e->split || !e->sw_dirty) return WCA_OK;
  const wca_model_dims& D = e->dims;
  const int d = D.n_audio_state, dt = D.n_text_state, C = D.n_mels;
  hipStream_t s = e->stream;
  WCA_TRY(dup_cols(s, e->conv1_w, e->k1pad, e->sw.conv1_w, e->sw.k1pad, d, 3 * C, C));
  WCA_TRY(dup_cols(s, e->conv2_w, 3 * d, e->sw.conv2_w, 6 * d, d, 3 * d, d));
  if (e->wslab_lo) {
    WCA_TRY(dup_cols(s, wlo_of(e, e->conv1_w), e->k1pad, e->sw.conv1_wlo, e->sw.k1pad, d, 3 * C, C, 1));
    WCA_TRY(dup_cols(s, wlo_of(e, e->conv2_w), 3 * d, e->sw.conv2_wlo, 6 * d, d, 3 * d, d, 1));
  }
  for (int li = 0; li < D.n_audio_layer; ++li) {
    const LayerW& l = e->enc[li];
    const LayerW& w = e->sw.enc[li];
    WCA_TRY(dup_cols(s, l.qkv_w, d, w.qkv_w, 2 * d, 3 * d, d, d));
    WCA_TRY(dup_cols(s, l.out_w, d, w.out_w, 2 * d, d, d, d));
    WCA_TRY(dup_cols(s, l.fc1_w, d, w.fc1_w, 2 * d, 4 * d, d, d));
    WCA_TRY(dup_cols(s, l.fc2_w, 4 * d, w.fc2_w, 8 * d, d, 4 * d, 4 * d));
  }
  WCA_TRY(dup_cols(s, e->tok_emb, dt, e->sw.tok_emb, 2 * dt, D.n_vocab, dt, dt));
  WCA_TRY(dup_cols(s, e->kv_w, d, e->sw.kv_w, 2 * d, (long)D.n_text_layer * 2 * dt, d, d));
  for (int li = 0; li < D.n_text_layer; ++li) {
    const LayerW& l = e->dec[li];
    const LayerW& w = e->sw.dec[li];
    WCA_TRY(dup_cols(s, l.qkv_w, dt, w.qkv_w, 2 * dt, 3 * dt, dt, dt));
    WCA_TRY(dup_cols(s, l.out_w, dt, w.out_w, 2 * dt, dt, dt, dt));
    WCA_TRY(dup_cols(s, l.cq_w, dt, w.cq_w, 2 * dt, dt, dt, dt));
    WCA_TRY(dup_cols(s, l.co_w, dt, w.co_w, 2 * dt, dt, dt, dt));
    WCA_TRY(dup_cols(s, l.fc1_w, dt, w.fc1_w, 2 * dt, 4 * dt, dt, dt));
    WCA_TRY(dup_cols(s, l.fc2_w, 4 * dt, w.fc2_w, 8 * dt, dt, 4 * dt, 4 * dt));
  }
  HIPCHK(hipStreamSynchronize(s));
  e->sw_dirty = false;
  return WCA_OK;
}

thread_local int g_gemm_cu_limit = 0;

hipError_t gemm(hipStream_t s, const half_t* A, int lda, const half_t* W, int ldw, const float* bias, void* C, int ldc, int M,
                int N, int K, int gelu, int out_mode, int site = 0, float* sk_ws = nullptr, size_t sk_bytes = 0, long c_lo = 0, long a_lo = 0,
                wca_engine* wlo_e = nullptr, const half_t* w_plain = nullptr, int k_plain = 0) {
  GemmArgs g{};
  g.a_lo = a_lo;
  g.cu_limit = g_gemm_cu_limit;
  g.sk_part = sk_ws;
  g.sk_bytes = sk_bytes;
  g.c_lo = c_lo;
  if (c_lo > 0 && out_mode == 0) out_mode = 4;
  g.A = A;
  g.lda = lda;
  g.W = W;
  g.ldw = ldw;
  g.bias = bias;
  g.C = C;
  g.ldc = ldc;
  g.M = M;
  g.N = N;
  g.K = K;
  g.gelu = gelu;
  g.out_mode = out_mode;
  g.site = site;
  if (wlo_e != nullptr && w_plain != nullptr && use_wlo(wlo_e) && wlo_e->wlo_bases.count(w_plain)) {
    GemmArgs x{};
    x.cu_limit = g_gemm_cu_limit;
    x.A = A;
    x.lda = lda;
    x.W = wlo_of(wlo_e, w_plain);
    x.ldw = k_plain;
    x.M = M;
    x.N = N;
    x.K = k_plain;
    x.site = site;
    if (out_mode == 2) {
      x.C = C;
      x.ldc = ldc;
      x.out_mode = 2;
    } else {
      GrowBuf& tmp = wlo_e->wlo_tmp[s == wlo_e->stream ? 0 : 1];
      if (hipError_t he = tmp.ensure((size_t)M * N * sizeof(float)); he != hipSuccess) return he;
      x.C = tmp.p;
      x.ldc = N;
      x.out_mode = 1;
      g.addend = (const float*)tmp.p;
      g.ld_addend = N;
    }
    if (hipError_t he = launch_gemm(x, s); he != hipSuccess) return he;
  }
  return launch_gemm(g, s);
}

int dec_gemm(wca_engine* e, hipStream_t s, int ws, const half_t* A, int lda, const float* xln, const float* ln_g, const float* ln_b,
             half_t* xn_scratch, const half_t* W, int ldw, const float* bias, void* C, int ldc, int M, int N, int K, int gelu, int out_mode,
             int site, half_t* kv_k = nullptr, half_t* kv_v = nullptr, int T_max = 0, int kv_t = 0) {
  const bool ln = xln != nullptr;
  const int sk = gemm_rows_pick_splitk(K);
  const bool fits = sk <= 1 || (kv_k == nullptr && (size_t)((M + 63) / 64) * ((N + 15) / 16) <= e->sk_tiles &&
                                gemm_rows_workspace_bytes(M, N, sk) <= e->sk_floats * sizeof(float));
  if (e->dec_fused && M <= DEC_ROWS_MAX && gemm_rows_supported(M, N, K, ln) && fits) {
    GemmArgs g{};
    g.A = A;
    g.lda = lda;
    g.A32 = xln;
    g.lda32 = K;
    g.ln_gamma = ln_g;
    g.ln_beta = ln_b;
    g.ln_eps = 1e-5f;
    g.W = W;
    g.ldw = ldw;
    g.bias = bias;
    g.C = C;
    g.ldc = ldc;
    g.M = M;
    g.N = N;
    g.K = K;
    g.gelu = gelu;
    g.out_mode = out_mode;
    g.site = site;
    g.splitk = sk;
    g.sk_part = e->sk_part[ws];
    g.sk_cnt = e->sk_cnt[ws];
    g.kv_k = kv_k;
    g.kv_v = kv_v;
    g.kv_bs = (long)T_max * K;
    g.kv_t = kv_t;
    g.kv_d = kv_k ? N / 3 : 0;
    HIPCHK(launch_gemm_rows(g, s));
// ... 237 lines not shown
    g.C = e->x;
    g.ldc = d;
    g.pos = e->enc_pos;
    g.pos_period = N_CTX;
    g.M = B * N_CTX;
    g.N = d;
    g.K = 3 * om * d;
    g.gelu = 1;
    g.out_mode = 1;
    g.site = 3;
    if (sp && use_wlo(e) && e->wlo_bases.count(e->conv2_w)) {
      GemmArgs x = g;
      x.W = e->sw.conv2_wlo;
      x.bias = nullptr;
      x.pos = nullptr;
      x.gelu = 0;
      x.out_mode = 1;
      HIPCHK(e->wlo_tmp[0].ensure((size_t)g.M * g.N * sizeof(float)));
      x.C = e->wlo_tmp[0].p;
      x.ldc = g.N;
      HIPCHK(launch_gemm(x, s));
      g.addend = (const float*)e->wlo_tmp[0].p;
      g.ld_addend = g.N;
    }
    HIPCHK(launch_gemm(g, s));
  }
  const int M = B * N_CTX;
  const float scale = 1.0f / std::sqrt((float)(d / H));
  memset(e->kev_set, 0, sizeof(e->kev_set));
  auto mark = [&](int site, int li, int which) {
    if (e->profiling && li < 33) {
      (void)hipEventRecord(e->kev[site][li][which], s);
      e->kev_set[site][li] = true;
    }
  };
  mark(WCA_SITE_LN1, 0, 0);
  HIPCHK(launch_layernorm_f16(e->x, e->enc[0].ln1_g, e->enc[0].ln1_b, e->xn, M, d, 1e-5f, s, om * d, sp ? d : 0));
  mark(WCA_SITE_LN1, 0, 1);
  for (int li = 0; li < D.n_audio_layer; ++li) {
    const LayerW& l = e->enc[li];
    const LayerW& w2 = sp ? e->sw.enc[li] : l;
    const GemmOpnd oq = pick_operands(sp, l.qkv_w, w2.qkv_w, d, M, 3 * d, sp ? 4 : 0, e);
    mark(WCA_SITE_QKV, li, 0);
    HIPCHK(gemm(s, e->xn, oq.lda, oq.W, oq.ldw, l.qkv_b, e->qkv, om * 3 * d, M, 3 * d, oq.K, 0, 0, 1, nullptr, 0, sp ? 3 * d : 0, oq.a_lo, e, oq.Wp, oq.Kp));
    mark(WCA_SITE_QKV, li, 1);
    AttnArgs a{};
    a.Q = e->qkv;
    a.K = e->qkv + d;
    a.V = e->qkv + 2 * d;
    a.q_bs = a.k_bs = a.v_bs = (long)N_CTX * om * 3 * d;
    a.q_rs = a.k_rs = a.v_rs = om * 3 * d;
    a.O = e->att;
    a.o_bs = (long)N_CTX * om * d;
    a.o_rs = om * d;
    a.split = sp ? 1 : 0;
    a.q_lo = a.k_lo = a.v_lo = 3 * d;
    a.o_lo = d;
    a.nq = N_CTX;
    a.nk = N_CTX;
    a.H = H;
    a.B = B;
    a.scale = scale;
    a.causal = 0;
    mark(WCA_SITE_ATTN, li, 0);
    HIPCHK(launch_attention(a, s));
    mark(WCA_SITE_ATTN, li, 1);
    const GemmOpnd oo = pick_operands(sp, l.out_w, w2.out_w, d, M, d, 2, e);
    if (int rc = gemm_residual_ln(e, s, e->att, oo.lda, oo.W, oo.ldw, l.out_b, e->x, M, d, oo.K, l.ln2_g, l.ln2_b, e->xn, 1, e->fuse_ln, WCA_SITE_OUT, li,
                                  WCA_SITE_LN2, li, oo.a_lo, oo.Wp, oo.Kp))
      return rc;
    const GemmOpnd o1 = pick_operands(sp, l.fc1_w, w2.fc1_w, d, M, 4 * d, sp ? 4 : 0, e);
    mark(WCA_SITE_FC1, li, 0);
    HIPCHK(gemm(s, e->xn, o1.lda, o1.W, o1.ldw, l.fc1_b, e->hid, om * 4 * d, M, 4 * d, o1.K, 1, 0, 1, nullptr, 0, sp ? 4 * d : 0, o1.a_lo, e, o1.Wp, o1.Kp));
    mark(WCA_SITE_FC1, li, 1);
    const bool last = li + 1 == D.n_audio_layer;
    const GemmOpnd o2 = pick_operands(sp, l.fc2_w, w2.fc2_w, 4 * d, M, d, 2, e);
    if (int rc = gemm_residual_ln(e, s, e->hid, o2.lda, o2.W, o2.ldw, l.fc2_b, e->x, M, d, o2.K, last ? e->lnpost_g : e->enc[li + 1].ln1_g,
                                  last ? e->lnpost_b : e->enc[li + 1].ln1_b, e->xn, 4, e->fuse_ln, WCA_SITE_FC2, li, WCA_SITE_LN1, li + 1, o2.a_lo, o2.Wp, o2.Kp))
      return rc;
  }
  return WCA_OK;
}

int run_cross_kv(wca_engine* e, int B, half_t* kvbuf = nullptr, bool skip_last_v = false) {
  if (!kvbuf) kvbuf = e->kv;
  const wca_model_dims& D = e->dims;
  const int d = D.n_audio_state, dt = D.n_text_state, L = D.n_text_layer;
  const int n_cols = L * 2 * dt - (skip_last_v ? dt : 0);
  const bool sp = e->split;
  const GemmOpnd o = pick_operands(sp, e->kv_w, sp ? e->sw.kv_w : e->kv_w, d, B * N_CTX, n_cols, sp ? 4 : 0, e);
  HIPCHK(gemm(e->stream, e->xn, o.lda, o.W, o.ldw, e->kv_b, kvbuf, (sp ? 2 : 1) * L * 2 * dt, B * N_CTX, n_cols, o.K, 0, 0, 3, nullptr, 0,
              sp ? (long)L * 2 * dt : 0, o.a_lo, e, o.Wp, o.Kp));
  return WCA_OK;
}

int run_decoder_split(wca_engine* e, const int64_t* tokens_dev, int B, int n, float* cap, int Fpad, int Fcap, float* logits_out, hipStream_t s,
                      const half_t* kvbuf, bool finish_last = false) {
  const wca_model_dims& D = e->dims;
  const int dt = D.n_text_state, H = D.n_text_head, L = D.n_text_layer;
  const int M = B * n;
  const float scale = 1.0f / std::sqrt((float)(dt / H));
  const int kv_ld = 2 * L * 2 * dt;
  const long kv_lo = (long)L * 2 * dt;
  HIPCHK(launch_embed(tokens_dev, e->tok_emb, e->dec_pos, e->xd, B, n, dt, D.n_vocab, e->err_dev, s,
                      (use_wlo(e) && e->wlo_bases.count(e->tok_emb)) ? wlo_of(e, e->tok_emb) : nullptr));
  auto ln = [&](const float* g, const float* b) -> int {
    HIPCHK(launch_layernorm_f16(e->xd, g, b, e->xdn, M, dt, 1e-5f, s, 2 * dt, dt));
    return WCA_OK;
  };
  auto mm = [&](const half_t* A, const half_t* W1, const half_t* W2, const float* bias, void* C, int ldc, int N, int K, int gelu, int out_mode,
                long c_lo, int site) -> int {
    const GemmOpnd o = pick_operands(true, W1, W2, K, M, N, (c_lo > 0 && out_mode == 0) ? 4 : out_mode, e);
    HIPCHK(gemm(s, A, o.lda, o.W, o.ldw, bias, C, ldc, M, N, o.K, gelu, out_mode, site, e->sk_big[1], e->sk_big_bytes, c_lo, o.a_lo, e, o.Wp, o.Kp));
    return WCA_OK;
  };
  for (int li = 0; li < L; ++li) {
    const LayerW& l = e->dec[li];
    const LayerW& w = e->sw.dec[li];
    WCA_TRY(ln(l.ln1_g, l.ln1_b));
    WCA_TRY(mm(e->xdn, l.qkv_w, w.qkv_w, l.qkv_b, e->qkv_d, 2 * 3 * dt, 3 * dt, dt, 0, 0, 3 * dt, 2));
    {
      AttnArgs a{};
      a.Q = e->qkv_d;
      a.K = e->qkv_d + dt;
      a.V = e->qkv_d + 2 * dt;
      a.q_bs = a.k_bs = a.v_bs = (long)n * 2 * 3 * dt;
      a.q_rs = a.k_rs = a.v_rs = 2 * 3 * dt;
      a.O = e->att_d;
      a.o_bs = (long)n * 2 * dt;
      a.o_rs = 2 * dt;
      a.split = 1;
      a.q_lo = a.k_lo = a.v_lo = 3 * dt;
      a.o_lo = dt;
      a.nq = n;
      a.nk = n;
      a.H = H;
      a.B = B;
      a.scale = scale;
      a.causal = 1;
      HIPCHK(launch_attention(a, s));
    }
    WCA_TRY(mm(e->att_d, l.out_w, w.out_w, l.out_b, e->xd, dt, dt, dt, 0, 2, 0, 2));
    WCA_TRY(ln(l.lnc_g, l.lnc_b));
    WCA_TRY(mm(e->xdn, l.cq_w, w.cq_w, l.cq_b, e->q_d, 2 * dt, dt, dt, 0, 0, dt, 2));
    {
      AttnArgs a{};
      a.Q = e->q_d;
      a.q_bs = (long)n * 2 * dt;
      a.q_rs = 2 * dt;
      a.K = kvbuf + (size_t)(2 * li) * dt;
      a.V = kvbuf + (size_t)(2 * li + 1) * dt;
      a.k_bs = a.v_bs = (long)N_CTX * kv_ld;
      a.k_rs = a.v_rs = kv_ld;
      a.O = e->att_d;
      a.o_bs = (long)n * 2 * dt;
      a.o_rs = 2 * dt;
      a.split = 1;
      a.q_lo = dt;
      a.k_lo = a.v_lo = kv_lo;
      a.o_lo = dt;
      a.cap = cap ? cap + (size_t)li * H * n * Fpad : nullptr;
      a.cap_bs = (long)L * H * n * Fpad;
      a.cap_hs = (long)n * Fpad;
      a.cap_ld = Fpad;
      a.cap_cols = Fcap;
      a.nq = n;
      a.nk = N_CTX;
      a.H = H;
      a.B = B;
      a.scale = scale;
      a.causal = 0;
      HIPCHK(launch_attention(a, s));
    }
    if (li == L - 1 && !logits_out && !finish_last) break;
    WCA_TRY(mm(e->att_d, l.co_w, w.co_w, l.co_b, e->xd, dt, dt, dt, 0, 2, 0, 2));
    WCA_TRY(ln(l.ln2_g, l.ln2_b));
    WCA_TRY(mm(e->xdn, l.fc1_w, w.fc1_w, l.fc1_b, e->hid_d, 2 * 4 * dt, 4 * dt, dt, 1, 0, 4 * dt, 2));
    WCA_TRY(mm(e->hid_d, l.fc2_w, w.fc2_w, l.fc2_b, e->xd, dt, dt, 4 * dt, 0, 2, 0, 2));
  }
  if (logits_out) {
    WCA_TRY(ln(e->lnf_g, e->lnf_b));
    WCA_TRY(mm(e->xdn, e->tok_emb, e->sw.tok_emb, nullptr, logits_out, D.n_vocab, D.n_vocab, dt, 0, 1, 0, 3));
  }
  return WCA_OK;
}

int run_decoder(wca_engine* e, const int64_t* tokens_dev, int B, int n, float* cap, int Fpad, int Fcap, float* logits_out,
                hipStream_t s = nullptr, const half_t* kvbuf = nullptr, bool finish_last = false) {
  const wca_model_dims& D = e->dims;
  const int dt = D.n_text_state, H = D.n_text_head, L = D.n_text_layer;
  if (!s) s = e->stream;
  if (!kvbuf) kvbuf = e->kv;
  if (e->split) return run_decoder_split(e, tokens_dev, B, n, cap, Fpad, Fcap, logits_out, s, kvbuf, finish_last);
  const int M = B * n;
  const float scale = 1.0f / std::sqrt((float)(dt / H));
  HIPCHK(launch_embed(tokens_dev, e->tok_emb, e->dec_pos, e->xd, B, n, dt, D.n_vocab, e->err_dev, s));
  for (int li = 0; li < L; ++li) {
    const LayerW& l = e->dec[li];
    WCA_TRY(dec_gemm(e, s, 0, nullptr, 0, e->xd, l.ln1_g, l.ln1_b, e->xdn, l.qkv_w, dt, l.qkv_b, e->qkv_d, 3 * dt, M, 3 * dt, dt, 0, 0, 2));
    {
      AttnArgs a{};
      a.Q = e->qkv_d;
      a.K = e->qkv_d + dt;
      a.V = e->qkv_d + 2 * dt;
      a.q_bs = a.k_bs = a.v_bs = (long)n * 3 * dt;
      a.q_rs = a.k_rs = a.v_rs = 3 * dt;
      a.O = e->att_d;
      a.o_bs = (long)n * dt;
      a.o_rs = dt;
      a.nq = n;
      a.nk = n;
      a.H = H;
      a.B = B;
      a.scale = scale;
      a.causal = 1;
      HIPCHK(launch_attention(a, s));
    }
    WCA_TRY(dec_gemm(e, s, 0, e->att_d, dt, nullptr, nullptr, nullptr, nullptr, l.out_w, dt, l.out_b, e->xd, dt, M, dt, dt, 0, 2, 2));
    WCA_TRY(dec_gemm(e, s, 0, nullptr, 0, e->xd, l.lnc_g, l.lnc_b, e->xdn, l.cq_w, dt, l.cq_b, e->q_d, dt, M, dt, dt, 0, 0, 2));
    {
      AttnArgs a{};
      a.Q = e->q_d;
      a.q_bs = (long)n * dt;
      a.q_rs = dt;
      a.K = kvbuf + (size_t)(2 * li) * dt;
      a.V = kvbuf + (size_t)(2 * li + 1) * dt;
      a.k_bs = a.v_bs = (long)N_CTX * L * 2 * dt;
      a.k_rs = a.v_rs = L * 2 * dt;
      a.O = e->att_d;
      a.o_bs = (long)n * dt;
      a.o_rs = dt;
      a.cap = cap ? cap + (size_t)li * H * n * Fpad : nullptr;
      a.cap_bs = (long)L * H * n * Fpad;
      a.cap_hs = (long)n * Fpad;
      a.cap_ld = Fpad;
      a.cap_cols = Fcap;
      a.nq = n;
      a.nk = N_CTX;
      a.H = H;
      a.B = B;
      a.scale = scale;
      a.causal = 0;
      HIPCHK(launch_attention(a, s));
    }
    if (li == L - 1 && !logits_out && !finish_last) break;
    WCA_TRY(dec_gemm(e, s, 0, e->att_d, dt, nullptr, nullptr, nullptr, nullptr, l.co_w, dt, l.co_b, e->xd, dt, M, dt, dt, 0, 2, 2));
    WCA_TRY(dec_gemm(e, s, 0, nullptr, 0, e->xd, l.ln2_g, l.ln2_b, e->xdn, l.fc1_w, dt, l.fc1_b, e->hid_d, 4 * dt, M, 4 * dt, dt, 1, 0, 2));
    WCA_TRY(dec_gemm(e, s, 0, e->hid_d, 4 * dt, nullptr, nullptr, nullptr, nullptr, l.fc2_w, 4 * dt, l.fc2_b, e->xd, dt, M, dt, 4 * dt, 0, 2, 2));
  }
  if (logits_out) {
    WCA_TRY(dec_gemm(e, s, 0, nullptr, 0, e->xd, e->lnf_g, e->lnf_b, e->xdn, e->tok_emb, dt, nullptr, logits_out, D.n_vocab, M, D.n_vocab, dt, 0, 1, 3));
  }
  return WCA_OK;
}

int run_decode_step(wca_engine* e, hipStream_t s, int ws, const half_t* kvbuf, const int* tokens, int b0, int B, int B_all, int t, int T_max,
                    bool want_logits, int phase = -2) {
  const wca_model_dims& D = e->dims;
  const int dt = D.n_text_state, H = D.n_text_head, L = D.n_text_layer;
  const float scale = 1.0f / std::sqrt((float)(dt / H));
  half_t* cache = (half_t*)e->dec_cache.p;
  const size_t plane = (size_t)B_all * T_max * dt;
  float* xd = e->xd + (size_t)b0 * dt;
  half_t* xdn = e->xdn + (size_t)b0 * dt;
  half_t* qkv_d = e->qkv_d + (size_t)b0 * 3 * dt;
  half_t* att_d = e->att_d + (size_t)b0 * dt;
  half_t* q_d = e->q_d + (size_t)b0 * dt;
  half_t* hid_d = e->hid_d + (size_t)b0 * 4 * dt;
  const int kv_ld = (e->split ? 2 : 1) * L * 2 * dt;
  const half_t* kvb = kvbuf + (size_t)b0 * N_CTX * kv_ld;
  if (phase == -2 || phase == -1)
    HIPCHK(launch_embed_step(tokens + (size_t)b0 * T_max, T_max, t, e->tok_emb, e->dec_pos, xd, B, dt, D.n_vocab, s));
  for (int li = 0; li < L; ++li) {
    if (phase != -2 && phase != li) continue;
    const LayerW& l = e->dec[li];
    half_t* kc = cache + (size_t)(2 * li) * plane + (size_t)b0 * T_max * dt;
    half_t* vc = kc + plane;
    WCA_TRY(dec_gemm(e, s, ws, nullptr, 0, xd, l.ln1_g, l.ln1_b, xdn, l.qkv_w, dt, l.qkv_b, qkv_d, 3 * dt, B, 3 * dt, dt, 0, 0, 2, kc, vc, T_max, t));
    {
      AttnArgs a{};
      a.Q = qkv_d;
      a.q_bs = 3 * dt;
      a.q_rs = 3 * dt;
      a.K = kc;
      a.V = vc;
      a.k_bs = a.v_bs = (long)T_max * dt;
      a.k_rs = a.v_rs = dt;
      a.O = att_d;
      a.o_bs = dt;
      a.o_rs = dt;
      a.nq = 1;
      a.nk = t + 1;
      a.H = H;
      a.B = B;
      a.scale = scale;
      a.causal = 0;
      HIPCHK(launch_attention(a, s));
    }
    WCA_TRY(dec_gemm(e, s, ws, att_d, dt, nullptr, nullptr, nullptr, nullptr, l.out_w, dt, l.out_b, xd, dt, B, dt, dt, 0, 2, 2));
    WCA_TRY(dec_gemm(e, s, ws, nullptr, 0, xd, l.lnc_g, l.lnc_b, xdn, l.cq_w, dt, l.cq_b, q_d, dt, B, dt, dt, 0, 0, 2));
    {
      AttnArgs a{};
      a.Q = q_d;
      a.q_bs = dt;
      a.q_rs = dt;
      a.K = kvb + (size_t)(2 * li) * dt;
      a.V = kvb + (size_t)(2 * li + 1) * dt;
      a.k_bs = a.v_bs = (long)N_CTX * kv_ld;
      a.k_rs = a.v_rs = kv_ld;
      a.O = att_d;
      a.o_bs = dt;
      a.o_rs = dt;
      a.nq = 1;
      a.nk = N_CTX;
      a.H = H;
      a.B = B;
      a.scale = scale;
      a.causal = 0;
      HIPCHK(launch_attention(a, s));
    }
    WCA_TRY(dec_gemm(e, s, ws, att_d, dt, nullptr, nullptr, nullptr, nullptr, l.co_w, dt, l.co_b, xd, dt, B, dt, dt, 0, 2, 2));
    WCA_TRY(dec_gemm(e, s, ws, nullptr, 0, xd, l.ln2_g, l.ln2_b, xdn, l.fc1_w, dt, l.fc1_b, hid_d, 4 * dt, B, 4 * dt, dt, 1, 0, 2));
    WCA_TRY(dec_gemm(e, s, ws, hid_d, 4 * dt, nullptr, nullptr, nullptr, nullptr, l.fc2_w, 4 * dt, l.fc2_b, xd, dt, B, dt, 4 * dt, 0, 2, 2));
  }
  if (want_logits && (phase == -2 || phase == L))
    WCA_TRY(dec_gemm(e, s, ws, nullptr, 0, xd, e->lnf_g, e->lnf_b, xdn, e->tok_emb, dt, nullptr, (float*)e->dec_logits.p + (size_t)b0 * D.n_vocab,
                     D.n_vocab, B, D.n_vocab, dt, 0, 1, 3));
  return WCA_OK;
}

int run_decode_prefill(wca_engine* e, hipStream_t s, const half_t* kvbuf, const int* tokens, int B, int n, int T_max, int sot_index) {
  const wca_model_dims& D = e->dims;
  const int dt = D.n_text_state, H = D.n_text_head, L = D.n_text_layer;
  const int M = B * n;
  const float scale = 1.0f / std::sqrt((float)(dt / H));
  half_t* cache = (half_t*)e->dec_cache.p;
  const size_t plane = (size_t)B * T_max * dt;
  const int kv_ld = (e->split ? 2 : 1) * L * 2 * dt;
  HIPCHK(launch_embed_prefix(tokens, T_max, n, e->tok_emb, e->dec_pos, e->xd, B, dt, D.n_vocab, s));
  for (int li = 0; li < L; ++li) {
    const LayerW& l = e->dec[li];
    half_t* kc = cache + (size_t)(2 * li) * plane;
    half_t* vc = kc + plane;
    WCA_TRY(dec_gemm(e, s, 0, nullptr, 0, e->xd, l.ln1_g, l.ln1_b, e->xdn, l.qkv_w, dt, l.qkv_b, e->qkv_d, 3 * dt, M, 3 * dt, dt, 0, 0, 2));
    HIPCHK(launch_kv_scatter(e->qkv_d, kc, vc, B, n, T_max, dt, s));
    {
      AttnArgs a{};
      a.Q = e->qkv_d;
      a.K = e->qkv_d + dt;
      a.V = e->qkv_d + 2 * dt;
      a.q_bs = a.k_bs = a.v_bs = (long)n * 3 * dt;
      a.q_rs = a.k_rs = a.v_rs = 3 * dt;
      a.O = e->att_d;
      a.o_bs = (long)n * dt;
      a.o_rs = dt;
      a.nq = n;
      a.nk = n;
      a.H = H;
      a.B = B;
      a.scale = scale;
      a.causal = 1;
      HIPCHK(launch_attention(a, s));
    }
    WCA_TRY(dec_gemm(e, s, 0, e->att_d, dt, nullptr, nullptr, nullptr, nullptr, l.out_w, dt, l.out_b, e->xd, dt, M, dt, dt, 0, 2, 2));
    WCA_TRY(dec_gemm(e, s, 0, nullptr, 0, e->xd, l.lnc_g, l.lnc_b, e->xdn, l.cq_w, dt, l.cq_b, e->q_d, dt, M, dt, dt, 0, 0, 2));
    {
      AttnArgs a{};
      a.Q = e->q_d;
      a.q_bs = (long)n * dt;
      a.q_rs = dt;
      a.K = kvbuf + (size_t)(2 * li) * dt;
      a.V = kvbuf + (size_t)(2 * li + 1) * dt;
      a.k_bs = a.v_bs = (long)N_CTX * kv_ld;
      a.k_rs = a.v_rs = kv_ld;
      a.O = e->att_d;
      a.o_bs = (long)n * dt;
      a.o_rs = dt;
      a.nq = n;
      a.nk = N_CTX;
      a.H = H;
      a.B = B;
      a.scale = scale;
      a.causal = 0;
      HIPCHK(launch_attention(a, s));
    }
    WCA_TRY(dec_gemm(e, s, 0, e->att_d, dt, nullptr, nullptr, nullptr, nullptr, l.co_w, dt, l.co_b, e->xd, dt, M, dt, dt, 0, 2, 2));
    WCA_TRY(dec_gemm(e, s, 0, nullptr, 0, e->xd, l.ln2_g, l.ln2_b, e->xdn, l.fc1_w, dt, l.fc1_b, e->hid_d, 4 * dt, M, 4 * dt, dt, 1, 0, 2));
    WCA_TRY(dec_gemm(e, s, 0, e->hid_d, 4 * dt, nullptr, nullptr, nullptr, nullptr, l.fc2_w, 4 * dt, l.fc2_b, e->xd, dt, M, dt, 4 * dt, 0, 2, 2));
  }
  const int R = (sot_index >= 0 ? 2 : 1) * B;
  float* xg = (float*)e->dec_gather.p;
  HIPCHK(launch_gather_rows(e->xd, xg, B, n, n - 1, sot_index, dt, s));
  WCA_TRY(dec_gemm(e, s, 0, nullptr, 0, xg, e->lnf_g, e->lnf_b, e->xdn, e->tok_emb, dt, nullptr, (float*)e->dec_logits.p, D.n_vocab, R, D.n_vocab,
                   dt, 0, 1, 3));
  return WCA_OK;
}

int check_ready(wca_engine* e) {
  if (!e) return fail(WCA_ERR_INVALID, "null engine");
  if (!e->finalized) return fail(WCA_ERR_STATE, "weights not finalized (call wca_finalize_weights)");
  HIPCHK(hipSetDevice(e->device));
  return ensure_split_weights(e);
}

int stage_meta(wca_engine* e, int B, const int32_t* a0, const int32_t* a1, const int32_t* a2, const int32_t* a3, int** dev_rows,
               hipStream_t s = nullptr) {
  const int slot = e->meta_slot;
  e->meta_slot = (e->meta_slot + 1) % META_SLOTS;
  int* h = e->meta_host + (size_t)slot * 4 * e->max_batch;
  int* dv = e->meta_dev + (size_t)slot * 4 * e->max_batch;
  const int32_t* src[4] = {a0, a1, a2, a3};
  for (int r = 0; r < 4; ++r)
    for (int b = 0; b < B; ++b) h[r * e->max_batch + b] = src[r] ? src[r][b] : 0;
  HIPCHK(hipMemcpyAsync(dv, h, sizeof(int) * 4 * e->max_batch, hipMemcpyHostToDevice, s ? s : e->stream));
  for (int r = 0; r < 4; ++r) dev_rows[r] = dv + r * e->max_batch;
  return WCA_OK;
}

int run_logmel(wca_engine* e, const float* pcm_dev, int64_t pcm_stride, const int* n_samples_dev, int B, float* mel_out, bool want_tm) {
  if (!e->have_filters) return fail(WCA_ERR_STATE, "mel_filters not loaded (wca_load_weight(\"mel_filters\"))");
  LogMelArgs a{};
  a.pcm = pcm_dev;
  a.pcm_stride = pcm_stride;
  a.n_samples = n_samples_dev;
  a.filters = e->mel_filters;
  a.filt_lo = e->filt_lo;
  a.filt_hi = e->filt_hi;
  a.window = e->window;
  a.twiddle = e->twiddle;
  a.mel_out = mel_out;
  a.mel_tm = want_tm ? e->mel_tm : nullptr;
  a.n_mels_pad = (e->split ? 2 : 1) * e->dims.n_mels;
  a.tm_lo = e->split ? e->dims.n_mels : 0;
  a.precise = e->split ? 1 : 0;
  a.scratch = e->mel_scratch;
  a.gmax = e->gmax;
  a.n_mels = e->dims.n_mels;
  a.B = B;
  HIPCHK(launch_logmel(a, e->stream));
  return WCA_OK;
}

__global__ void mel_to_tm_kernel(const float* __restrict__ mel, half_t* __restrict__ tm, int n_mels, int B, int row, int lo_off) {
  const int b = blockIdx.y;
  const long e0 = (long)blockIdx.x * blockDim.x + threadIdx.x;
  if (e0 >= (long)n_mels * N_FRAMES) return;
  const int t = (int)(e0 / n_mels), m = (int)(e0 - (long)t * n_mels);
  const float v = mel[((long)b * n_mels + m) * N_FRAMES + t];
  const half_t hv = (half_t)v;
  half_t* o = tm + ((long)b * (N_FRAMES + 2) + t + 1) * row + m;
  o[0] = hv;
  if (lo_off) o[lo_off] = (half_t)(v - (float)hv);
}

int mel_to_tm(wca_engine* e, const float* mel_dev, int batch) {
// ... 1768 lines not shown
  HIPCHK(hipMemcpyAsync(e->err_host, e->err_dev, sizeof(int), hipMemcpyDeviceToHost, e->stream));
  HIPCHK(hipStreamSynchronize(e->stream));
  if (e->err_host[0] & 2) return fail(WCA_ERR_HIP, "LayerNorm statistics hand-off timed out");
  return WCA_OK;
}

int wca_test_gemm_rows(wca_engine* e, const void* a_f16, const float* x_f32, const float* gamma, const float* beta, const void* w,
                       const float* bias, void* c, int M, int N, int K, int gelu, int out_mode, int splitk, int groups, void* kv_k, void* kv_v,
                       int T_max, int kv_t) {
  if (!e || !w || !c || (!a_f16 && !x_f32) || (x_f32 && (!gamma || !beta))) return fail(WCA_ERR_INVALID, "null argument");
  HIPCHK(hipSetDevice(e->device));
  if (splitk <= 0) splitk = gemm_rows_pick_splitk(K);
  if (splitk <= 0) return fail(WCA_ERR_INVALID, "no split of K=%d fits the few-row kernel", K);
  const size_t tiles = (size_t)((M + 63) / 64) * ((N + 15) / 16);
  if (splitk > 1) {
    HIPCHK(e->tmp0.ensure(gemm_rows_workspace_bytes(M, N, splitk)));
    HIPCHK(e->tmp1.ensure(sizeof(unsigned) * tiles));
    HIPCHK(hipMemsetAsync(e->tmp1.p, 0, sizeof(unsigned) * tiles, e->stream));
  }
  GemmArgs g{};
  g.A = (const half_t*)a_f16;
  g.lda = K;
  g.A32 = x_f32;
  g.lda32 = K;
  g.ln_gamma = gamma;
  g.ln_beta = beta;
  g.ln_eps = 1e-5f;
  g.W = (const half_t*)w;
  g.ldw = K;
  g.bias = bias;
  g.C = c;
  g.ldc = N;
  g.M = M;
  g.N = N;
  g.K = K;
  g.gelu = gelu;
  g.out_mode = out_mode;
  g.splitk = splitk;
  g.groups = groups;
  g.sk_part = (float*)e->tmp0.p;
  g.sk_cnt = (unsigned*)e->tmp1.p;
  g.kv_k = (half_t*)kv_k;
  g.kv_v = (half_t*)kv_v;
  g.kv_bs = (long)T_max * (N / 3);
  g.kv_t = kv_t;
  g.kv_d = kv_k ? N / 3 : 0;
  HIPCHK(launch_gemm_rows(g, e->stream));
  if (splitk > 1) {
    std::vector<unsigned> cnt(tiles);
    HIPCHK(hipMemcpyAsync(cnt.data(), e->tmp1.p, sizeof(unsigned) * tiles, hipMemcpyDeviceToHost, e->stream));
    HIPCHK(hipStreamSynchronize(e->stream));
    for (unsigned v : cnt)
      if (v != 0) return fail(WCA_ERR_HIP, "split-K arrival counter left at %u", v);
  }
  HIPCHK(hipStreamSynchronize(e->stream));
  return WCA_OK;
}

int wca_test_set_attn_split_drop(int mask) {
  if (mask != 0 && mask != 1 && mask != 2 && mask != 3 && mask != 4 && mask != 8 && mask != 9 && mask != 12 && mask != 15)
    return fail(WCA_ERR_INVALID, "attention pass mask %d is not instantiated", mask);
  set_debug_switch("attn_split_drop", mask);
  return WCA_OK;
}

int wca_test_set_switch(const char* name, int value) {
  if (!name) return fail(WCA_ERR_INVALID, "null argument");
  if (set_debug_switch(name, value) != 0) return fail(WCA_ERR_INVALID, "unknown switch %s", name);
  return WCA_OK;
}

int wca_test_last_scores(wca_engine* e, int batch, float* scores_host) {
  if (!e || !scores_host) return fail(WCA_ERR_INVALID, "null argument");
  if (e->enq_count != e->fetch_count) return fail(WCA_ERR_STATE, "fetch the batches in flight first");
  HIPCHK(hipSetDevice(e->device));
  const size_t n = (size_t)batch * e->dims.n_text_layer * e->dims.n_text_head;
  if (batch < 1 || e->scores.bytes < n * sizeof(float)) return fail(WCA_ERR_INVALID, "no head scores of a batch of %d are held", batch);
  HIPCHK(hipStreamSynchronize(e->stream));
  HIPCHK(hipStreamSynchronize(e->stream2));
  HIPCHK(hipMemcpy(scores_host, e->scores.p, n * sizeof(float), hipMemcpyDeviceToHost));
  return WCA_OK;
}

int wca_test_attention(wca_engine* e, const void* q, const void* k, const void* v, void* o, float* cap_dev, int cap_ld, int cap_cols,
                       int B, int H, int nq, int nk, int causal) {
  if (!e) return fail(WCA_ERR_INVALID, "null engine");
  const int variant = (causal >> 8) & 3;
  if (variant == 3) return fail(WCA_ERR_INVALID, "attention variant 3 does not exist");
  HIPCHK(hipSetDevice(e->device));
  AttnArgs a{};
  const int d = H * 64;
  a.Q = (const half_t*)q;
  a.q_bs = (long)nq * d;
  a.q_rs = d;
  a.K = (const half_t*)k;
  a.k_bs = (long)nk * d;
  a.k_rs = d;
  a.V = (const half_t*)v;
  a.v_bs = (long)nk * d;
  a.v_rs = d;
  a.O = (half_t*)o;
  a.o_bs = (long)nq * d;
  a.o_rs = d;
  a.cap = cap_dev;
  a.cap_bs = (long)H * nq * cap_ld;
  a.cap_hs = (long)nq * cap_ld;
  a.cap_ld = cap_ld;
  a.cap_cols = cap_cols;
  a.nq = nq;
  a.nk = nk;
  a.H = H;
  a.B = B;
  a.scale = 0.125f;
  a.causal = causal & 1;
  a.variant = variant;
  HIPCHK(launch_attention(a, e->stream));
  return WCA_OK;
}

int wca_test_attention_split(wca_engine* e, const void* q2, const void* k2, const void* v2, void* o2, float* cap_dev, int cap_ld, int cap_cols,
                             int B, int H, int nq, int nk, int causal) {
  if (!e || !q2 || !k2 || !v2 || !o2) return fail(WCA_ERR_INVALID, "null argument");
  HIPCHK(hipSetDevice(e->device));
  AttnArgs a{};
  const int d = H * 64;
  a.Q = (const half_t*)q2;
  a.q_bs = (long)nq * 2 * d;
  a.q_rs = 2 * d;
  a.K = (const half_t*)k2;
  a.k_bs = (long)nk * 2 * d;
  a.k_rs = 2 * d;
  a.V = (const half_t*)v2;
  a.v_bs = (long)nk * 2 * d;
  a.v_rs = 2 * d;
  a.O = (half_t*)o2;
  a.o_bs = (long)nq * 2 * d;
  a.o_rs = 2 * d;
  a.split = 1;
  a.q_lo = a.k_lo = a.v_lo = a.o_lo = d;
  a.cap = cap_dev;
  a.cap_bs = (long)H * nq * cap_ld;
  a.cap_hs = (long)nq * cap_ld;
  a.cap_ld = cap_ld;
  a.cap_cols = cap_cols;
  a.nq = nq;
  a.nk = nk;
  a.H = H;
  a.B = B;
  a.scale = 0.125f;
  a.causal = causal & 1;
  HIPCHK(launch_attention(a, e->stream));
  return WCA_OK;
}

int wca_test_decode_select(wca_engine* e, const float* logits_dev, int batch, int n_vocab, int32_t* tokens_dev, int T_max, int cur_len,
                           int n_initial, const uint8_t* suppress_mask_dev, const uint8_t* blank_mask_dev, const wca_decode_opts* o,
                           float* sum_logprob_dev, int32_t* n_done_dev) {
  if (!e || !logits_dev || !tokens_dev || !suppress_mask_dev || !o || !sum_logprob_dev || !n_done_dev) return fail(WCA_ERR_INVALID, "null argument");
  HIPCHK(hipSetDevice(e->device));
  DecodeSelectArgs a{};
  a.logits = logits_dev;
  a.ld = n_vocab;
  a.n_vocab = n_vocab;
  a.tokens = tokens_dev;
  a.T_max = T_max;
  a.cur_len = cur_len;
// ... 48 lines not shown
```

### whisper-char-alignment_amd/csrc/gemm.hip

```cpp
#include <atomic>

#include "gemm_epilogue.h"
#include <cstdlib>
#include "kernels.h"
#include "wca_common.h"

namespace wca {

namespace {

constexpr int BM = 128, BN = 128, BK = 64;
constexpr int TILE_ELEMS = 128 * 64;

struct RowPtrs {
  const half_t* p[4];
};

__device__ __forceinline__ half8 ldfrag(const half_t* tile, int r, int c) {
  return *reinterpret_cast<const half8*>(tile + r * 64 + ((c ^ swz128(r)) << 3));
}

template <int OUT_MODE, bool GELU, int MT>
__device__ __forceinline__ void epilogue(const GemmArgs& a, f32x4 (&acc)[MT][4], int mbase, int nb, int fr) {
  float bv[16];
#pragma unroll
  for (int j = 0; j < 16; ++j) bv[j] = (a.bias != nullptr && nb + j < a.N) ? a.bias[nb + j] : 0.f;
  const bool full_n = (nb + 16 <= a.N);

#pragma unroll
  for (int mt = 0; mt < MT; ++mt) {
    const int m = mbase + mt * 16 + fr;
    if (m >= a.M) continue;
    float v[16];
#pragma unroll
    for (int nt = 0; nt < 4; ++nt)
#pragma unroll
      for (int r = 0; r < 4; ++r) v[nt * 4 + r] = acc[mt][nt][r] + bv[nt * 4 + r];
    if (OUT_MODE != 2 && a.addend != nullptr) {
      const float* ap = a.addend + (long)m * a.ld_addend + nb;
#pragma unroll
      for (int j = 0; j < 16; ++j)
        if (nb + j < a.N) v[j] += ap[j];
    }
    if (GELU) {
#pragma unroll
      for (int j = 0; j < 16; j += 2) {
        if (OUT_MODE == 4) {
          const f32x2 g = gelu_erfc2(f32x2{v[j], v[j + 1]});
          v[j] = g[0];
          v[j + 1] = g[1];
        } else {
          v[j] = gelu_erf(v[j]);
          v[j + 1] = gelu_erf(v[j + 1]);
        }
      }
    }
    if (a.pos != nullptr) {
      const float* pp = a.pos + (long)(m % a.pos_period) * a.N + nb;
#pragma unroll
      for (int j = 0; j < 16; ++j)
        if (nb + j < a.N) v[j] += pp[j];
    }
    long coff;
    if (a.c_rows_per_batch > 0) {
      const int b = m / a.c_rows_per_batch;
      const int t = m - b * a.c_rows_per_batch;
      coff = (long)b * a.c_batch_stride + (long)t * a.ldc;
    } else {
      coff = (long)m * a.ldc;
    }
    if (OUT_MODE == 0 || OUT_MODE == 4) {
      half_t* cp = reinterpret_cast<half_t*>(a.C) + coff + nb;
      if (full_n && ((reinterpret_cast<uintptr_t>(cp) & 15) == 0)) {
        half8 h0, h1, l0, l1;
        if (OUT_MODE == 4) {
#pragma unroll
          for (int j = 0; j < 8; j += 2) {
            const Half2Pair p0 = split_pair2(v[j], v[j + 1]), p1 = split_pair2(v[8 + j], v[8 + j + 1]);
            h0[j] = p0.hi[0];
            h0[j + 1] = p0.hi[1];
            l0[j] = p0.lo[0];
            l0[j + 1] = p0.lo[1];
            h1[j] = p1.hi[0];
            h1[j + 1] = p1.hi[1];
            l1[j] = p1.lo[0];
            l1[j + 1] = p1.lo[1];
          }
        } else {
#pragma unroll
          for (int j = 0; j < 8; ++j) {
            h0[j] = (half_t)v[j];
            h1[j] = (half_t)v[8 + j];
          }
        }
        reinterpret_cast<half8*>(cp)[0] = h0;
        reinterpret_cast<half8*>(cp)[1] = h1;
        if (OUT_MODE == 4) {
          reinterpret_cast<half8*>(cp + a.c_lo)[0] = l0;
          reinterpret_cast<half8*>(cp + a.c_lo)[1] = l1;
        }
      } else {
#pragma unroll
        for (int j = 0; j < 16; ++j)
          if (nb + j < a.N) {
            if (OUT_MODE == 4) {
              const HalfPair pr = split_pair(v[j]);
              cp[j] = pr.hi;
              cp[a.c_lo + j] = pr.lo;
            } else {
              cp[j] = (half_t)v[j];
            }
          }
      }
    } else {
      float* cp = reinterpret_cast<float*>(a.C) + coff + nb;
      if (full_n && ((reinterpret_cast<uintptr_t>(cp) & 15) == 0)) {
        f32x4* c4 = reinterpret_cast<f32x4*>(cp);
#pragma unroll
        for (int q = 0; q < 4; ++q) {
          f32x4 o = f32x4{v[q * 4 + 0], v[q * 4 + 1], v[q * 4 + 2], v[q * 4 + 3]};
          if (OUT_MODE == 2) o += c4[q];
          c4[q] = o;
        }
      } else {
#pragma unroll
        for (int j = 0; j < 16; ++j)
          if (nb + j < a.N) cp[j] = (OUT_MODE == 2) ? cp[j] + v[j] : v[j];
      }
    }
  }
}

template <int OUT_MODE, bool GELU, int SITE>
__global__ __launch_bounds__(256, 2) void gemm_f16_kernel(GemmArgs a) {
  extern __shared__ __attribute__((aligned(16))) char smem[];
  half_t* lds = reinterpret_cast<half_t*>(smem);
  const int tid = threadIdx.x;
  const int lane = tid & 63;
  const int wave = __builtin_amdgcn_readfirstlane(tid >> 6);
  const int wm = wave >> 1, wn = wave & 1;

  const int ntn = (a.N + BN - 1) / BN;
  const int ntm = (a.M + BM - 1) / BM;
  const int nwg = ntm * ntn;
  const int id = xcd_remap(blockIdx.x, nwg);
  const int tm = id / ntn, tn = id - tm * ntn;
  const int m0 = tm * BM, n0 = tn * BN;

  const half_t* asrc[4];
  const half_t* wsrc[4];
#pragma unroll
  for (int i = 0; i < 4; ++i) {
    const int r = (wave * 4 + i) * 8 + (lane >> 3);
    const int c = (lane & 7) ^ swz128(r);
    int gm = m0 + r;
    gm = gm < a.M ? gm : a.M - 1;
    long aoff;
    if (a.a_rows_per_batch > 0) {
      const int b = gm / a.a_rows_per_batch;
      const int t = gm - b * a.a_rows_per_batch;
      aoff = (long)b * a.a_batch_stride + (long)t * a.lda;
    } else {
      aoff = (long)gm * a.lda;
    }
    const int kbeg = (int)blockIdx.y * (a.K / (int)gridDim.y);
    asrc[i] = a.A + aoff + c * 8 + kbeg;
    int gn = n0 + r;
    gn = gn < a.N ? gn : a.N - 1;
    wsrc[i] = a.W + (long)gn * a.ldw + c * 8 + kbeg;
  }

  auto stage = [&](int buf, int k0) {
    half_t* At = lds + buf * (2 * TILE_ELEMS);
    half_t* Wt = At + TILE_ELEMS;
#pragma unroll
    for (int i = 0; i < 4; ++i) {
      const int rbase = (wave * 4 + i) * 8;
      glds16(asrc[i] + k0, At + rbase * 64);
      glds16(wsrc[i] + k0, Wt + rbase * 64);
    }
  };

  f32x4 acc[4][4];
#pragma unroll
  for (int i = 0; i < 4; ++i)
#pragma unroll
    for (int j = 0; j < 4; ++j) acc[i][j] = f32x4{0.f, 0.f, 0.f, 0.f};

  const int fr = lane & 15;
  const int fg = lane >> 4;
  int xrow[4], wrow[4];
#pragma unroll
  for (int t = 0; t < 4; ++t) {
    xrow[t] = wm * 64 + t * 16 + fr;
    wrow[t] = wn * 64 + (fr >> 2) * 16 + t * 4 + (fr & 3);
  }

  const int nk = a.K / BK / (int)gridDim.y;
  stage(0, 0);
  wait_vm0();
  __syncthreads();
  int cur = 0;
  for (int kt = 0; kt < nk; ++kt) {
    if (kt + 1 < nk) stage(cur ^ 1, (kt + 1) * BK);
    const half_t* At = lds + cur * (2 * TILE_ELEMS);
    const half_t* Wt = At + TILE_ELEMS;
#pragma unroll
    for (int ks = 0; ks < 2; ++ks) {
      half8 xf[4], wf[4];
#pragma unroll
      for (int t = 0; t < 4; ++t) {
        xf[t] = ldfrag(At, xrow[t], ks * 4 + fg);
        wf[t] = ldfrag(Wt, wrow[t], ks * 4 + fg);
      }
#pragma unroll
      for (int mt = 0; mt < 4; ++mt)
#pragma unroll
        for (int nt = 0; nt < 4; ++nt)
          acc[mt][nt] = __builtin_amdgcn_mfma_f32_16x16x32_f16(wf[nt], xf[mt], acc[mt][nt], 0, 0, 0);
    }
    wait_vm0();
    __syncthreads();
    cur ^= 1;
  }

  if (OUT_MODE == 2 && gridDim.y > 1) {
    GemmArgs p = a;
    p.C = a.sk_part + (long)blockIdx.y * a.M * a.N;
    p.ldc = a.N;
    p.c_rows_per_batch = 0;
    p.bias = nullptr;
    p.pos = nullptr;
    epilogue<1, false, 4>(p, acc, m0 + wm * 64, n0 + wn * 64 + fg * 16, fr);
    return;
  }
  epilogue<OUT_MODE, GELU, 4>(a, acc, m0 + wm * 64, n0 + wn * 64 + fg * 16, fr);
}

__global__ __launch_bounds__(256) void splitk_reduce_kernel(const float* __restrict__ part, int S, int M, int N, const float* __restrict__ bias,
                                                            float* __restrict__ x, int ldc) {
  const long i4 = (long)blockIdx.x * blockDim.x + threadIdx.x;
  const int n4 = N >> 2;
  if (i4 >= (long)M * n4) return;
  const int m = (int)(i4 / n4), n = (int)(i4 - (long)m * n4) * 4;
  f32x4 v = *reinterpret_cast<const f32x4*>(part + (long)m * N + n);
  for (int s = 1; s < S; ++s) v += *reinterpret_cast<const f32x4*>(part + ((long)s * M + m) * N + n);
  if (bias != nullptr) v += *reinterpret_cast<const f32x4*>(bias + n);
  f32x4* xp = reinterpret_cast<f32x4*>(x + (long)m * ldc + n);
  *xp = *xp + v;
}


template <int OUT_MODE, bool GELU, int SITE>
__global__ __launch_bounds__(512) void gemm256_f16_kernel(GemmArgs a) {
  extern __shared__ __attribute__((aligned(16))) char smem[];
  half_t* lds = reinterpret_cast<half_t*>(smem);
  constexpr int TILE256 = 256 * 64;
  const int tid = threadIdx.x;
  const int lane = tid & 63;
  const int wave = __builtin_amdgcn_readfirstlane(tid >> 6);
  const int wr = wave >> 2, wc = wave & 3;

  const int ntn = (a.N + 255) / 256;
  const int ntm = (a.M + 255) / 256;
  const int nwg = ntm * ntn;
  const int id = xcd_remap(blockIdx.x, nwg);
  const int tm = id / ntn, tn = id - tm * ntn;
  const int m0 = tm * 256, n0 = tn * 256;

  const half_t* asrc[4];
  const half_t* wsrc[4];
#pragma unroll
  for (int i = 0; i < 4; ++i) {
    const int r = (wave * 4 + i) * 8 + (lane >> 3);
    const int c = (lane & 7) ^ swz128(r);
    int gm = m0 + r;
    gm = gm < a.M ? gm : a.M - 1;
    long aoff;
    if (a.a_rows_per_batch > 0) {
      const int b = gm / a.a_rows_per_batch;
      const int t = gm - b * a.a_rows_per_batch;
      aoff = (long)b * a.a_batch_stride + (long)t * a.lda;
    } else {
      aoff = (long)gm * a.lda;
    }
    asrc[i] = a.A + aoff + c * 8;
    int gn = n0 + r;
    gn = gn < a.N ? gn : a.N - 1;
    wsrc[i] = a.W + (long)gn * a.ldw + c * 8;
  }

  auto stage = [&](int buf, int k0) {
    half_t* At = lds + buf * (2 * TILE256);
    half_t* Wt = At + TILE256;
#pragma unroll
    for (int i = 0; i < 4; ++i) {
      const int rbase = (wave * 4 + i) * 8;
      glds16(asrc[i] + k0, At + rbase * 64);
      glds16(wsrc[i] + k0, Wt + rbase * 64);
    }
  };

  f32x4 acc[8][4];
#pragma unroll
  for (int i = 0; i < 8; ++i)
#pragma unroll
    for (int j = 0; j < 4; ++j) acc[i][j] = f32x4{0.f, 0.f, 0.f, 0.f};

  const int fr = lane & 15, fg = lane >> 4;
  int xrow[8], wrow[4];
#pragma unroll
  for (int t = 0; t < 8; ++t) xrow[t] = wr * 128 + t * 16 + fr;
#pragma unroll
  for (int t = 0; t < 4; ++t) wrow[t] = wc * 64 + (fr >> 2) * 16 + t * 4 + (fr & 3);

  const int nk = a.K / BK;
  stage(0, 0);
  if (nk > 1) stage(1, BK);
  for (int kt = 0; kt < nk; ++kt) {
    const int cur = kt & 1;
    const half_t* At = lds + cur * (2 * TILE256);
    const half_t* Wt = At + TILE256;
    if (kt + 1 < nk) {
      asm volatile("s_waitcnt vmcnt(8)" ::: "memory");
    } else {
      asm volatile("s_waitcnt vmcnt(0)" ::: "memory");
    }
    __builtin_amdgcn_s_barrier();
    asm volatile("" ::: "memory");

    half8 wf[2][4], xf[2][4];
#pragma unroll
    for (int ks = 0; ks < 2; ++ks)
#pragma unroll
      for (int t = 0; t < 4; ++t) {
        wf[ks][t] = ldfrag(Wt, wrow[t], ks * 4 + fg);
        xf[ks][t] = ldfrag(At, xrow[t], ks * 4 + fg);
      }
    __builtin_amdgcn_s_setprio(1);
#pragma unroll
    for (int ks = 0; ks < 2; ++ks)
#pragma unroll
      for (int mt = 0; mt < 4; ++mt)
#pragma unroll
        for (int nt = 0; nt < 4; ++nt)
          acc[mt][nt] = __builtin_amdgcn_mfma_f32_16x16x32_f16(wf[ks][nt], xf[ks][mt], acc[mt][nt], 0, 0, 0);
    __builtin_amdgcn_s_setprio(0);

    half8 xg[2][4];
#pragma unroll
    for (int ks = 0; ks < 2; ++ks)
#pragma unroll
      for (int t = 0; t < 4; ++t) xg[ks][t] = ldfrag(At, xrow[4 + t], ks * 4 + fg);
    asm volatile("s_waitcnt lgkmcnt(0)" ::: "memory");
    __builtin_amdgcn_s_barrier();
    asm volatile("" ::: "memory");
    if (kt + 2 < nk) stage(cur, (kt + 2) * BK);
    __builtin_amdgcn_s_setprio(1);
#pragma unroll
    for (int ks = 0; ks < 2; ++ks)
#pragma unroll
      for (int mt = 0; mt < 4; ++mt)
#pragma unroll
        for (int nt = 0; nt < 4; ++nt)
          acc[4 + mt][nt] = __builtin_amdgcn_mfma_f32_16x16x32_f16(wf[ks][nt], xg[ks][mt], acc[4 + mt][nt], 0, 0, 0);
    __builtin_amdgcn_s_setprio(0);
  }

  epilogue<OUT_MODE, GELU, 8>(a, acc, m0 + wr * 128, n0 + wc * 64 + fg * 16, fr);
}

template <int V>
struct GemmIntC {
  static constexpr int value = V;
};

template <int OUT_MODE, bool GELU, int SITE, int SPLITW_MODE = 0>
__global__ __launch_bounds__(512) void gemm256p_f16_kernel(GemmArgs a) {
  constexpr bool SPLITW = SPLITW_MODE != 0;
  constexpr bool RING3 = SPLITW_MODE == 2;
  extern __shared__ __attribute__((aligned(16))) char smem[];
  half_t* lds = reinterpret_cast<half_t*>(smem);
  constexpr int TILE256 = 256 * 64;
  float* bias_lds = reinterpret_cast<float*>(smem + 4 * TILE256 * sizeof(half_t));
  float* gamma_lds = bias_lds + 512;
  float* beta_lds = gamma_lds + 512;
  float* ln_lds = beta_lds + 512;
  const int tid = threadIdx.x;
  const int lane = tid & 63;
  const int wave = __builtin_amdgcn_readfirstlane(tid >> 6);
  const int wr = wave >> 2, wc = wave & 3;

  const int ntn = (a.N + 255) / 256;
  const int ntm = (a.M + 255) / 256;
  const int nwg = ntm * ntn;
  const int G = gridDim.x;

  const __amdgpu_buffer_rsrc_t ra = __builtin_amdgcn_make_buffer_rsrc(const_cast<half_t*>(a.A), 0, (int)a.a_bytes, 0x00020000);
  const __amdgpu_buffer_rsrc_t rw = __builtin_amdgcn_make_buffer_rsrc(const_cast<half_t*>(a.W), 0, (int)a.w_bytes, 0x00020000);
  const __amdgpu_buffer_rsrc_t rb = __builtin_amdgcn_make_buffer_rsrc(const_cast<float*>(a.bias), 0, a.bias != nullptr ? a.N * 4 : 0, 0x00020000);
  const __amdgpu_buffer_rsrc_t rg = __builtin_amdgcn_make_buffer_rsrc(const_cast<float*>(a.ln_gamma), 0, OUT_MODE == 3 ? a.N * 4 : 0, 0x00020000);
  const __amdgpu_buffer_rsrc_t rbeta = __builtin_amdgcn_make_buffer_rsrc(const_cast<float*>(a.ln_beta), 0, OUT_MODE == 3 ? a.N * 4 : 0, 0x00020000);
  const int l8 = lane >> 3;
  const int rho = wave * 8 + l8;
  const int c0 = (lane & 7) ^ ((rho >> 1) & 7);
  const int nt_r = rho >> 4, i_r = rho & 15;
  const int wsrc_row = (OUT_MODE == 0 || OUT_MODE == 3 || OUT_MODE == 4) ? ((nt_r >> 1) * 32 + (i_r >> 2) * 8 + (nt_r & 1) * 4 + (i_r & 3)) : rho;
  const unsigned va = (unsigned)(rho * a.lda + c0 * 8) * 2u;
  const unsigned vw = (unsigned)(wsrc_row * a.ldw + c0 * 8) * 2u;
  const unsigned sa64 = 64u * a.lda * 2u, sw64 = 64u * a.ldw * 2u;

  auto a_slot = [&](int buf) -> half_t* { return RING3 ? lds + buf * TILE256 : lds + buf * (2 * TILE256); };
  auto w_slot = [&](int bufw) -> half_t* { return RING3 ? lds + 3 * TILE256 : lds + bufw * (2 * TILE256) + TILE256; };
  auto stage_one = [&](int buf, int bufw, unsigned ta, unsigned tw, int g) {
    half_t* At = a_slot(buf);
    half_t* Wt = w_slot(bufw);
    const int i = g >> 1;
    unsigned so = ((g & 1) == 0) ? ta + i * sa64 : tw + i * sw64;
    asm volatile("" : "+s"(so));
    if ((g & 1) == 0)
      __builtin_amdgcn_raw_ptr_buffer_load_lds(ra, (WCA_LDS void*)(At + (i * 64 + wave * 8) * 64), 16, (int)(va + so), 0, 0, 0);
    else
      __builtin_amdgcn_raw_ptr_buffer_load_lds(rw, (WCA_LDS void*)(Wt + (i * 64 + wave * 8) * 64), 16, (int)(vw + so), 0, 0, 0);
  };

  auto stage_bias = [&](int par, int ncol0) {
    if (wave < 4) {
      __builtin_amdgcn_raw_ptr_buffer_load_lds(rb, (WCA_LDS void*)(bias_lds + par * 256 + wave * 64), 4, (ncol0 + wave * 64 + lane) * 4, 0, 0, 0);
      if (OUT_MODE == 3) {
        __builtin_amdgcn_raw_ptr_buffer_load_lds(rg, (WCA_LDS void*)(gamma_lds + par * 256 + wave * 64), 4, (ncol0 + wave * 64 + lane) * 4, 0, 0, 0);
        __builtin_amdgcn_raw_ptr_buffer_load_lds(rbeta, (WCA_LDS void*)(beta_lds + par * 256 + wave * 64), 4, (ncol0 + wave * 64 + lane) * 4, 0, 0, 0);
      }
    }
  };
  constexpr int RING3_A_REQS_IN_FLIGHT = 4;
  static_assert(RING3_A_REQS_IN_FLIGHT * 64 == 256, "one request per 64-row block of the 256-row A tile");

  const int fr = lane & 15, fg = lane >> 4;
  const int pos0 = fg ^ ((fr >> 1) & 7);
  const int xb0 = (wr * 128 + fr) * 64 + pos0 * 8, xb1 = (wr * 128 + fr) * 64 + (pos0 ^ 4) * 8;
  const int wb0 = (wc * 64 + fr) * 64 + pos0 * 8, wb1 = (wc * 64 + fr) * 64 + (pos0 ^ 4) * 8;

#define WCA_LOAD_HALF(AT, WT, XB, WB, WF, XF)                                                      \
  do {                                                                                             \
    _Pragma("unroll") for (int t = 0; t < 4; ++t) WF[t] = *reinterpret_cast<const half8*>((WT) + (WB) + t * 1024); \
    _Pragma("unroll") for (int t = 0; t < 8; ++t) XF[t] = *reinterpret_cast<const half8*>((AT) + (XB) + t * 1024); \
  } while (0)

  const int nk = SPLITW ? 2 * (a.K / BK) : a.K / BK;
  auto a_koff = [&](int s_) -> unsigned {
    return SPLITW ? (unsigned)(((s_ & 1) * (int)a.a_lo + (s_ >> 1) * BK) * 2) : (unsigned)(s_ * (BK * 2));
  };
// ... 73 lines not shown
    }
    const int m0n = tmn_ * 256, n0n = tnn_ * 256;
    const unsigned tan = (unsigned)m0n * a.lda * 2u, twn = (unsigned)n0n * a.ldw * 2u;
    auto kstep = [&](auto par_c, const int kt) {
      constexpr int PAR = decltype(par_c)::value;
      const int cur = RING3 ? ring_a : (PAR >= 0 ? PAR : (kt & 1));
      const int nxt = RING3 ? (ring_a == 2 ? 0 : ring_a + 1) : (cur ^ 1);
      const int wslot = SPLITW ? ((kt >> 1) & 1) : cur;
      const int wslot_n = SPLITW ? (((kt + 1) >> 1) & 1) : (cur ^ 1);
      const bool W_FRESH = !SPLITW || (PAR >= 0 ? PAR == 0 : (kt & 1) == 0);
      const bool W_NEXT_FRESH = !SPLITW || (PAR >= 0 ? PAR == 1 : (kt & 1) == 1);
      const half_t* At = a_slot(cur);
      const half_t* Wt = w_slot(wslot);
      const bool in_tile2 = kt + 2 < nk;
      const bool more1 = kt + 1 < nk, more2 = in_tile2 || has_next;
      const unsigned ka = (in_tile2 ? ta + a_koff(kt + 2) : tan + a_koff(kt + 2 - nk));
      const unsigned kw = (in_tile2 ? tw + w_koff(kt + 2) : twn + w_koff(kt + 2 - nk));
      const int prv = RING3 ? (ring_a == 0 ? 2 : ring_a - 1) : 0;
#pragma unroll
      for (int g = 0; g < 8; ++g) {
        __builtin_amdgcn_s_setprio(1);
#pragma unroll
        for (int nt = 0; nt < 4; ++nt) acc[g][nt] = __builtin_amdgcn_mfma_f32_16x16x32_f16(w0[nt], x0[g], acc[g][nt], 0, 0, 0);
        __builtin_amdgcn_s_setprio(0);
        __builtin_amdgcn_sched_barrier(0);
        if (g < 2) {
          if (W_FRESH) {
            w1[2 * g] = *reinterpret_cast<const half8*>(Wt + wb1 + (2 * g) * 1024);
            w1[2 * g + 1] = *reinterpret_cast<const half8*>(Wt + wb1 + (2 * g + 1) * 1024);
          }
        } else if (g < 6) {
          x1[2 * (g - 2)] = *reinterpret_cast<const half8*>(At + xb1 + (2 * (g - 2)) * 1024);
          x1[2 * (g - 2) + 1] = *reinterpret_cast<const half8*>(At + xb1 + (2 * (g - 2) + 1) * 1024);
        }
        if (RING3 && (g & 1) == 0 && (g >> 1) < RING3_A_REQS_IN_FLIGHT && more2) stage_one(prv, 0, ka, kw, g);
        __builtin_amdgcn_sched_barrier(0);
      }
      if (RING3 && more2) asm volatile("s_waitcnt vmcnt(%0) lgkmcnt(0)" ::"i"(RING3_A_REQS_IN_FLIGHT) : "memory");
      else asm volatile("s_waitcnt vmcnt(0) lgkmcnt(0)" ::: "memory");
      __builtin_amdgcn_s_barrier();
      asm volatile("" ::: "memory");
      const int wslot_2 = SPLITW ? (wslot ^ 1) : cur;
      const half_t* An = a_slot(nxt);
      const half_t* Wn = w_slot(wslot_n);
#pragma unroll
      for (int g = 0; g < 8; ++g) {
        __builtin_amdgcn_s_setprio(1);
#pragma unroll
        for (int nt = 0; nt < 4; ++nt) acc[g][nt] = __builtin_amdgcn_mfma_f32_16x16x32_f16(w1[nt], x1[g], acc[g][nt], 0, 0, 0);
        __builtin_amdgcn_s_setprio(0);
        __builtin_amdgcn_sched_barrier(0);
        if (RING3) {
          if (W_FRESH && (g & 1) == 1 && more2) stage_one(cur, 0, ka, kw, g);
        } else if (more2 && (W_FRESH || (g & 1) == 0)) {
          stage_one(cur, wslot_2, ka, kw, g);
        }
        if (more1) {
          if (g < 2) {
            if (W_NEXT_FRESH) {
              w0[2 * g] = *reinterpret_cast<const half8*>(Wn + wb0 + (2 * g) * 1024);
              w0[2 * g + 1] = *reinterpret_cast<const half8*>(Wn + wb0 + (2 * g + 1) * 1024);
            }
          } else if (g < 6) {
            x0[2 * (g - 2)] = *reinterpret_cast<const half8*>(An + xb0 + (2 * (g - 2)) * 1024);
            x0[2 * (g - 2) + 1] = *reinterpret_cast<const half8*>(An + xb0 + (2 * (g - 2) + 1) * 1024);
          }
        }
        __builtin_amdgcn_sched_barrier(0);
      }
      if (RING3) ring_a = nxt;
    };
    for (int kt = 0; kt < nk; ++kt) kstep(GemmIntC<-1>{}, kt);

    {
      int fr_e = fr, fg_e = fg;
      asm volatile("" : "+v"(fr_e), "+v"(fg_e));
      typedef __attribute__((address_space(4))) GemmArgs KernArgs;
      const KernArgs* ap = (const KernArgs*)__builtin_amdgcn_kernarg_segment_ptr();
      asm volatile("" : "+s"(ap));
      if constexpr (OUT_MODE == 3)
        epilogue_ln<KernArgs>(*ap, acc, m0, m0 >> 8, n0 >> 8, ntn, wr, wc, fr_e, fg_e, bias_lds + par * 256 + wc * 64, gamma_lds + par * 256,
                              beta_lds + par * 256, ln_lds);
      else
        epilogue_wide<OUT_MODE, GELU, KernArgs>(*ap, acc, m0 + wr * 128, n0 + wc * 64, fr_e, fg_e, bias_lds + par * 256 + wc * 64);
    }
    if (!has_next) break;
    par ^= 1;
    stage_bias(par, n0n);
    v = vn;
    id = idn;
    ++round;
    m0 = m0n;
    n0 = n0n;
    ta = tan;
    tw = twn;
#pragma unroll
    for (int i = 0; i < 8; ++i)
#pragma unroll
      for (int j = 0; j < 4; ++j) acc[i][j] = f32x4{0.f, 0.f, 0.f, 0.f};
    WCA_LOAD_HALF(a_slot(RING3 ? ring_a : 0), w_slot(0), xb0, wb0, w0, x0);
  }
#undef WCA_LOAD_HALF
}


template <int OUT_MODE, bool GELU>
__global__ __launch_bounds__(256) void gemm_skinny_f16_kernel(GemmArgs a) {
  __shared__ float red[4][4][4][64];
  const int tid = threadIdx.x;
  const int lane = tid & 63;
  const int wave = __builtin_amdgcn_readfirstlane(tid >> 6);
  const int fr = lane & 15, fg = lane >> 4;
  const int n0 = blockIdx.x * 16;
  const int kq = a.K >> 2;
  const int kbeg = wave * kq;
  int nrow = n0 + fr;
  nrow = nrow < a.N ? nrow : a.N - 1;
  const half_t* wp = a.W + (long)nrow * a.ldw + kbeg + fg * 8;
  const half_t* xp[4];
#pragma unroll
  for (int mt = 0; mt < 4; ++mt) {
    int m = mt * 16 + fr;
    m = m < a.M ? m : a.M - 1;
    xp[mt] = a.A + (long)m * a.lda + kbeg + fg * 8;
  }
  f32x4 acc[4];
#pragma unroll
  for (int mt = 0; mt < 4; ++mt) acc[mt] = f32x4{0.f, 0.f, 0.f, 0.f};
  half8 wf[2][4], xf[2][4][4];
  auto load_chunk = [&](int buf, int k) {
#pragma unroll
    for (int u = 0; u < 4; ++u) {
      wf[buf][u] = *reinterpret_cast<const half8*>(wp + k + u * 32);
#pragma unroll
      for (int mt = 0; mt < 4; ++mt) xf[buf][u][mt] = *reinterpret_cast<const half8*>(xp[mt] + k + u * 32);
    }
  };
  auto mul_chunk = [&](int buf) {
#pragma unroll
    for (int u = 0; u < 4; ++u)
#pragma unroll
      for (int mt = 0; mt < 4; ++mt) acc[mt] = __builtin_amdgcn_mfma_f32_16x16x32_f16(wf[buf][u], xf[buf][u][mt], acc[mt], 0, 0, 0);
  };
  load_chunk(0, 0);
  for (int k = 0; k < kq; k += 256) {
    if (k + 128 < kq) load_chunk(1, k + 128);
    mul_chunk(0);
    if (k + 256 < kq) load_chunk(0, k + 256);
    if (k + 128 < kq) mul_chunk(1);
  }
#pragma unroll
  for (int mt = 0; mt < 4; ++mt)
#pragma unroll
    for (int r = 0; r < 4; ++r) red[wave][mt][r][lane] = acc[mt][r];
  __syncthreads();
  const int m = wave * 16 + fr;
  float v[4];
#pragma unroll
  for (int r = 0; r < 4; ++r) v[r] = red[0][wave][r][lane] + red[1][wave][r][lane] + red[2][wave][r][lane] + red[3][wave][r][lane];
  if (m >= a.M) return;
  const int nb = n0 + 4 * fg;
#pragma unroll
  for (int r = 0; r < 4; ++r) {
    const int n = nb + r;
    if (a.bias != nullptr && n < a.N) v[r] += a.bias[n];
    if (GELU) v[r] = gelu_erf(v[r]);
  }
  long coff;
  if (a.c_rows_per_batch > 0) {
    const int b = m / a.c_rows_per_batch;
    coff = (long)b * a.c_batch_stride + (long)(m - b * a.c_rows_per_batch) * a.ldc;
  } else {
    coff = (long)m * a.ldc;
  }
  if (OUT_MODE == 0) {
    half_t* cp = reinterpret_cast<half_t*>(a.C) + coff + nb;
    if (nb + 4 <= a.N && (reinterpret_cast<uintptr_t>(cp) & 7) == 0) {
      half4 o;
#pragma unroll
      for (int r = 0; r < 4; ++r) o[r] = (half_t)v[r];
      *reinterpret_cast<half4*>(cp) = o;
    } else {
#pragma unroll
      for (int r = 0; r < 4; ++r)
        if (nb + r < a.N) cp[r] = (half_t)v[r];
    }
  } else {
    float* cp = reinterpret_cast<float*>(a.C) + coff + nb;
#pragma unroll
    for (int r = 0; r < 4; ++r)
      if (nb + r < a.N) cp[r] = (OUT_MODE == 2) ? cp[r] + v[r] : v[r];
  }
}

}

bool gemm_ln_supported(int M, int N, int K, int n_cu) {
  if (N % 256 != 0 || N > 2048 || K % 128 != 0 || M < 1) return false;
  const long tiles = (long)((M + 255) / 256) * (N / 256);
  if (tiles < 192) return false;
  return (n_cu >> 3) >= N / 256;
}

bool gemm_splitw_supported(int M, int N, int K, int lda, int out_mode) {
  if (M < 1 || N < 1 || K < 128 || (K % 128) != 0) return false;
  if (out_mode != 0 && out_mode != 1 && out_mode != 2 && out_mode != 4) return false;
  const long tiles256 = (long)((M + 255) / 256) * ((N + 255) / 256);
  if (tiles256 < 192) return false;
  const size_t a_need = ((size_t)(M - 1) * lda + 2 * (size_t)K) * sizeof(half_t), w_need = ((size_t)(N - 1) * K + K) * sizeof(half_t);
  return a_need < 0x7fffffffull && w_need < 0x7fffffffull;
}

hipError_t launch_gemm(const GemmArgs& a_in, hipStream_t s) {
  GemmArgs a = a_in;
  if (a.M <= 0 || a.N <= 0) return hipSuccess;
  if (a.K <= 0 || (a.K % BK) != 0) return hipErrorInvalidValue;
  if ((a.lda % 8) != 0 || (a.ldw % 8) != 0) return hipErrorInvalidValue;
  if (a.out_mode == 4 && (a.c_lo <= 0 || (a.c_lo & 7))) return hipErrorInvalidValue;
  if (a.addend != nullptr && (a.out_mode == 2 || a.out_mode == 3 || a.a_lo > 0)) return hipErrorInvalidValue;
  if ((a.force_tile == 64 || a.force_tile == 0) && a.M <= 64 && (a.K % 512) == 0 && a.a_rows_per_batch == 0 && a.pos == nullptr && a.addend == nullptr && a.out_mode != 4 && a.a_lo <= 0) {
    const dim3 sgrid((unsigned)((a.N + 15) / 16)), sblock(256);
#define WCA_LAUNCH_SK(OM, G) hipLaunchKernelGGL((gemm_skinny_f16_kernel<OM, G>), sgrid, sblock, 0, s, a)
    if (a.out_mode == 0) {
      if (a.gelu) WCA_LAUNCH_SK(0, true); else WCA_LAUNCH_SK(0, false);
    } else if (a.out_mode == 1) {
      if (a.gelu) WCA_LAUNCH_SK(1, true); else WCA_LAUNCH_SK(1, false);
    } else if (a.out_mode == 2 && !a.gelu) {
      WCA_LAUNCH_SK(2, false);
    } else {
      return hipErrorInvalidValue;
    }
#undef WCA_LAUNCH_SK
    return hipGetLastError();
  }
  if (a.force_tile == 64) return hipErrorInvalidValue;
  const long tiles256 = (long)((a.M + 255) / 256) * ((a.N + 255) / 256);
  const bool splitw = a.a_lo > 0;
  if (splitw && (a.force_tile == 64 || a.force_tile == 128 || a.force_tile == 256 || a.a_rows_per_batch != 0 ||
                 !gemm_splitw_supported(a.M, a.N, a.K, a.lda, a.out_mode) || (a.a_lo & 7) != 0))
    return hipErrorInvalidValue;
  const size_t a_need = ((size_t)(a.M - 1) * a.lda + (splitw ? (size_t)a.a_lo : 0) + a.K) * sizeof(half_t), w_need = ((size_t)(a.N - 1) * a.ldw + a.K) * sizeof(half_t);
  const bool can_buf = a.a_rows_per_batch == 0 && a_need < 0x7fffffffull && w_need < 0x7fffffffull;
  if (a.a_bytes == 0) a.a_bytes = (unsigned)a_need;
  if (a.w_bytes == 0) a.w_bytes = (unsigned)w_need;
  int dev = 0;
  {
    hipError_t e = hipGetDevice(&dev);
    if (e != hipSuccess) return e;
  }
  static std::atomic<int> n_cu_cache[32] = {};
  int n_cu = n_cu_cache[dev & 31].load(std::memory_order_relaxed);
  if (n_cu == 0) {
    hipError_t e = hipDeviceGetAttribute(&n_cu, hipDeviceAttributeMultiprocessorCount, dev);
    if (e != hipSuccess) return e;
    n_cu_cache[dev & 31].store(n_cu, std::memory_order_relaxed);
  }
  if (a.cu_limit > 0 && a.cu_limit < n_cu) n_cu = a.cu_limit;
  const int ring = splitw ? (debug_switch(DBG_GEMM_RING) == 1 ? 1 : 2) : 0;
  const bool want_big = (a.force_tile == 256 || a.force_tile == 257 || a.force_tile == 258) || (a.force_tile == 0 && tiles256 >= 192);
  const bool pipelined = want_big && can_buf && a.force_tile != 256 && a.addend == nullptr;
  const bool big = want_big;
  dim3 grid, block;
  size_t shmem;
  int splitk = 1;
  if (big) {
    grid = dim3((unsigned)tiles256);
    block = dim3(512);
    shmem = 2 * 2 * 256 * 64 * sizeof(half_t);
    if (pipelined) {
      shmem += 2 * 256 * sizeof(float);
      const int nk = (splitw ? 2 : 1) * (a.K / BK);
      if (a.force_tile != 258 && nk >= 2 && (nk & 1) == 0 && tiles256 > n_cu) grid = dim3((unsigned)n_cu);
      if (a.supertile <= 0) a.supertile = ((splitw ? 2 : 1) * a.K <= 2048 && (a.N + 255) / 256 <= 32) ? 8 : 1;
    }
  } else {
    const int ntn = (a.N + BN - 1) / BN, ntm = (a.M + BM - 1) / BM;
    grid = dim3(ntn * ntm);
    block = dim3(256);
    shmem = 2 * 2 * TILE_ELEMS * sizeof(half_t);
    splitk = 1;
    if (a.out_mode == 2 && !a.gelu && a.sk_part != nullptr && a.pos == nullptr && a.c_rows_per_batch == 0 && (a.N % 4) == 0 && (a.ldc % 4) == 0 &&
        ntn * ntm <= n_cu / 2 && a.K >= 2048) {
      for (int sk = 4; sk >= 2; --sk)
        if (a.K % (sk * BK) == 0 && (size_t)sk * a.M * a.N * sizeof(float) <= a.sk_bytes) {
          splitk = sk;
          break;
        }
    }
    grid.y = (unsigned)splitk;
  }
#define WCA_LAUNCH_K(...)                                                                         \
  do {                                                                                            \
    static std::atomic<unsigned> attr_mask{0};                                                    \
    if (!(attr_mask.load(std::memory_order_acquire) & (1u << (dev & 31)))) {                      \
      hipError_t e = hipFuncSetAttribute(reinterpret_cast<const void*>(__VA_ARGS__),              \
                                         hipFuncAttributeMaxDynamicSharedMemorySize, (int)shmem); \
      if (e != hipSuccess) return e;                                                              \
      attr_mask.fetch_or(1u << (dev & 31), std::memory_order_release);                            \
    }                                                                                             \
    hipLaunchKernelGGL((__VA_ARGS__), grid, block, shmem, s, a);                                  \
  } while (0)
// ... 60 lines not shown
```

### whisper-char-alignment_amd/csrc/gemm_epilogue.h

```cpp
#pragma once
#include "kernels.h"
#include "wca_common.h"

namespace wca {

template <int OUT_MODE, bool GELU, typename ArgsT>
__device__ __forceinline__ void epilogue_wide(const ArgsT& a, f32x4 (&acc)[8][4], int mbase, int nbase, int fr, int fg, const float* bias_l) {
  int col[4];
#pragma unroll
  for (int nt = 0; nt < 4; ++nt) col[nt] = (OUT_MODE == 0 || OUT_MODE == 4) ? ((nt >> 1) * 32 + fg * 8 + (nt & 1) * 4) : (nt * 16 + fg * 4);
  float bv[16];
#pragma unroll
  for (int nt = 0; nt < 4; ++nt) {
    const f32x4 b4 = *reinterpret_cast<const f32x4*>(bias_l + col[nt]);
#pragma unroll
    for (int r = 0; r < 4; ++r) bv[nt * 4 + r] = b4[r];
  }
  const bool full_n = (nbase + 64 <= a.N);
  if (OUT_MODE == 2) {
    float* cbase = reinterpret_cast<float*>(a.C) + nbase;
    if (full_n && a.pos == nullptr && (a.ldc & 3) == 0 && (a.c_batch_stride & 3) == 0 && ((reinterpret_cast<uintptr_t>(cbase + fg * 4) & 15) == 0)) {
#pragma unroll
      for (int mt = 0; mt < 8; ++mt)
#pragma unroll
        for (int nt = 0; nt < 4; ++nt)
#pragma unroll
          for (int r = 0; r < 4; ++r) acc[mt][nt][r] += bv[nt * 4 + r];
      constexpr int NB = 3;
#pragma unroll
      for (int base = 0; base < 8; base += NB) {
        f32x4 cv[NB][4];
        long coff[NB];
#pragma unroll
        for (int j = 0; j < NB; ++j) {
          if (base + j >= 8) continue;
          const int m = mbase + (base + j) * 16 + fr;
          if (a.c_rows_per_batch > 0) {
            const int b = m / a.c_rows_per_batch;
            coff[j] = (long)b * a.c_batch_stride + (long)(m - b * a.c_rows_per_batch) * a.ldc;
          } else {
            coff[j] = (long)m * a.ldc;
          }
          if (m < a.M) {
            const f32x4* cp = reinterpret_cast<const f32x4*>(cbase + coff[j] + fg * 4);
#pragma unroll
            for (int nt = 0; nt < 4; ++nt) cv[j][nt] = cp[nt * 4];
          }
        }
#pragma unroll
        for (int j = 0; j < NB; ++j) {
          if (base + j >= 8) continue;
          const int m = mbase + (base + j) * 16 + fr;
          if (m < a.M) {
            f32x4* cp = reinterpret_cast<f32x4*>(cbase + coff[j] + fg * 4);
#pragma unroll
            for (int nt = 0; nt < 4; ++nt) cp[nt * 4] = acc[base + j][nt] + cv[j][nt];
          }
        }
      }
      return;
    }
  }
#pragma unroll
  for (int mt = 0; mt < 8; ++mt) {
    const int m = mbase + mt * 16 + fr;
    float v[16];
#pragma unroll
    for (int nt = 0; nt < 4; ++nt)
#pragma unroll
      for (int r = 0; r < 4; ++r) v[nt * 4 + r] = acc[mt][nt][r] + bv[nt * 4 + r];
    if (m >= a.M) continue;
    if (GELU) {
#pragma unroll
      for (int j = 0; j < 16; j += 2) {
        if (OUT_MODE == 4) {
          const f32x2 g = gelu_erfc2(f32x2{v[j], v[j + 1]});
          v[j] = g[0];
          v[j + 1] = g[1];
        } else {
          v[j] = gelu_erf(v[j]);
          v[j + 1] = gelu_erf(v[j + 1]);
        }
      }
    }
    if (a.pos != nullptr) {
      const float* pp = a.pos + (long)(m % a.pos_period) * a.N + nbase;
#pragma unroll
      for (int nt = 0; nt < 4; ++nt)
#pragma unroll
        for (int r = 0; r < 4; ++r)
          if (nbase + col[nt] + r < a.N) v[nt * 4 + r] += pp[col[nt] + r];
    }
    long coff;
    if (a.c_rows_per_batch > 0) {
      const int b = m / a.c_rows_per_batch;
      const int t = m - b * a.c_rows_per_batch;
      coff = (long)b * a.c_batch_stride + (long)t * a.ldc;
    } else {
      coff = (long)m * a.ldc;
    }
    if (OUT_MODE == 0 || OUT_MODE == 4) {
      half_t* cp = reinterpret_cast<half_t*>(a.C) + coff + nbase;
      if (full_n && ((reinterpret_cast<uintptr_t>(cp + fg * 8) & 15) == 0)) {
#pragma unroll
        for (int hh = 0; hh < 2; ++hh) {
          half8 o, ol;
          if (OUT_MODE == 4) {
#pragma unroll
            for (int j = 0; j < 8; j += 2) {
              const Half2Pair pr = split_pair2(v[hh * 8 + j], v[hh * 8 + j + 1]);
              o[j] = pr.hi[0];
              o[j + 1] = pr.hi[1];
              ol[j] = pr.lo[0];
              ol[j + 1] = pr.lo[1];
            }
          } else {
#pragma unroll
            for (int j = 0; j < 8; ++j) o[j] = (half_t)v[hh * 8 + j];
          }
          *reinterpret_cast<half8*>(cp + hh * 32 + fg * 8) = o;
          if (OUT_MODE == 4) *reinterpret_cast<half8*>(cp + a.c_lo + hh * 32 + fg * 8) = ol;
        }
      } else {
#pragma unroll
        for (int nt = 0; nt < 4; ++nt)
#pragma unroll
          for (int r = 0; r < 4; ++r)
            if (nbase + col[nt] + r < a.N) {
              if (OUT_MODE == 4) {
                const HalfPair pr = split_pair(v[nt * 4 + r]);
                cp[col[nt] + r] = pr.hi;
                cp[a.c_lo + col[nt] + r] = pr.lo;
              } else {
                cp[col[nt] + r] = (half_t)v[nt * 4 + r];
              }
            }
      }
    } else {
      float* cp = reinterpret_cast<float*>(a.C) + coff + nbase;
      if (full_n && ((reinterpret_cast<uintptr_t>(cp + fg * 4) & 15) == 0)) {
#pragma unroll
        for (int nt = 0; nt < 4; ++nt) {
          f32x4* c4 = reinterpret_cast<f32x4*>(cp + col[nt]);
          f32x4 o = f32x4{v[nt * 4 + 0], v[nt * 4 + 1], v[nt * 4 + 2], v[nt * 4 + 3]};
          if (OUT_MODE == 2) o += *c4;
          *c4 = o;
        }
      } else {
#pragma unroll
        for (int nt = 0; nt < 4; ++nt)
#pragma unroll
          for (int r = 0; r < 4; ++r)
            if (nbase + col[nt] + r < a.N) cp[col[nt] + r] = (OUT_MODE == 2) ? cp[col[nt] + r] + v[nt * 4 + r] : v[nt * 4 + r];
      }
    }
  }
}

__device__ __forceinline__ float xor16_sum(float v) {
  const unsigned u = __float_as_uint(v);
  auto r = __builtin_amdgcn_permlane16_swap(u, u, false, false);
  return __uint_as_float(r[0]) + __uint_as_float(r[1]);
}
__device__ __forceinline__ float xor32_sum(float v) {
  const unsigned u = __float_as_uint(v);
  auto r = __builtin_amdgcn_permlane32_swap(u, u, false, false);
  return __uint_as_float(r[0]) + __uint_as_float(r[1]);
}
__device__ __forceinline__ void chan_merge(float& mean_a, float& m2_a, float na, float mean_b, float m2_b, float nb) {
  const float dlt = mean_b - mean_a, nt = na + nb;
  mean_a += dlt * (nb / nt);
  m2_a += m2_b + dlt * dlt * (na * nb / nt);
}

typedef __attribute__((address_space(1))) unsigned long long gu64_t;
typedef __attribute__((address_space(1))) unsigned gu32_t;

template <typename ArgsT>
__device__ __forceinline__ void epilogue_ln(const ArgsT& a, f32x4 (&acc)[8][4], int m0, int tm, int tn, int ntn, int wr, int wc, int fr, int fg,
                                            const float* bias_l, const float* gamma_l, const float* beta_l, float* ln_lds) {
  const int tid = threadIdx.x;
  const int mbase = m0 + wr * 128, nbase = tn * 256 + wc * 64;
  int col[4];
#pragma unroll
  for (int nt = 0; nt < 4; ++nt) col[nt] = (nt >> 1) * 32 + fg * 8 + (nt & 1) * 4;
// ... 149 lines not shown
```

### whisper-char-alignment_amd/csrc/kernels.h

```cpp
#pragma once
#include <hip/hip_runtime.h>
#include <stdint.h>

namespace wca {

typedef _Float16 half_t;

enum { DBG_ATTN_SPLIT_VARIANT = 0, DBG_HEAD_STATS_GENERAL, DBG_FAIL_PRECISION_ALLOC, DBG_ATTN_SPLIT_DROP, DBG_GEMM_RING, DBG_SWITCH_COUNT };
int debug_switch(int id);
int set_debug_switch(const char* name, int value);

struct GemmArgs {
  const half_t* A;
  long a_lo;
  int lda;
  int a_rows_per_batch;
  long a_batch_stride;
  const half_t* W;
  int ldw;
  const float* bias;
  void* C;
  int ldc;
  int c_rows_per_batch;
  long c_batch_stride;
  long c_lo;
  const float* addend;
  int ld_addend;
  const float* pos;
  int pos_period;
  int M, N, K;
  int gelu;
  int out_mode;
  unsigned a_bytes, w_bytes;
  int force_tile;
  const float* ln_gamma;
  const float* ln_beta;
  half_t* ln_out;
  int ln_ld;
  float ln_eps;
  unsigned long long* ln_stats;
  unsigned* ln_cnt;
  int* ln_err;
  int site;
  int supertile;
  int cu_limit;
  const float* A32;
  int lda32;
  half_t* kv_k;
  half_t* kv_v;
  long kv_bs;
  int kv_t, kv_d;
  size_t sk_bytes;
  float* sk_part;
  unsigned* sk_cnt;
  int splitk;
  int groups;
};
hipError_t launch_gemm(const GemmArgs& a, hipStream_t s);
hipError_t launch_gemm_rows(const GemmArgs& a, hipStream_t s);
bool gemm_rows_supported(int M, int N, int K, bool layernorm_a);
int gemm_rows_pick_splitk(int K);
size_t gemm_rows_workspace_bytes(int M, int N, int splitk);
bool gemm_ln_supported(int M, int N, int K, int n_cu);
bool gemm_splitw_supported(int M, int N, int K, int lda, int out_mode);

struct AttnArgs {
  const half_t* Q; long q_bs; int q_rs;
  const half_t* K; long k_bs; int k_rs;
  const half_t* V; long v_bs; int v_rs;
  half_t* O; long o_bs; int o_rs;
  float* cap;
  long cap_bs; long cap_hs; int cap_ld;
  int cap_cols;
  int nq, nk, H, B;
  float scale;
  int causal;
  int variant;
  int split;
  long q_lo, k_lo, v_lo, o_lo;
};
hipError_t launch_attention(const AttnArgs& a, hipStream_t s);
hipError_t launch_attention_split(const AttnArgs& a, hipStream_t s);

hipError_t launch_layernorm_f16(const float* x, const float* gamma, const float* beta, half_t* out,
                                int rows, int d, float eps, hipStream_t s, int ld_out = 0, long lo_off = 0);
hipError_t launch_embed(const int64_t* tokens, const half_t* tok_emb, const float* pos_emb, float* x,
                        int B, int n, int d, int n_vocab, int* err, hipStream_t s, const half_t* tok_emb_lo = nullptr);
hipError_t launch_fill_f16(half_t* p, size_t n, float v, hipStream_t s);

hipError_t launch_embed_step(const int* tokens, int T_max, int t, const half_t* tok_emb, const float* pos_emb, float* x, int B, int d,
                             int n_vocab, hipStream_t s);
hipError_t launch_kv_append(const half_t* qkv, half_t* kc, half_t* vc, int B, int T_max, int t, int d, hipStream_t s);
hipError_t launch_embed_prefix(const int* tokens, int T_max, int n, const half_t* tok_emb, const float* pos_emb, float* x, int B, int d,
                               int n_vocab, hipStream_t s);
hipError_t launch_kv_scatter(const half_t* qkv, half_t* kc, half_t* vc, int B, int n, int T_max, int d, hipStream_t s);
hipError_t launch_gather_rows(const float* x, float* out, int B, int n, int p0, int p1, int d, hipStream_t s);
struct DecodeSelectArgs {
  const float* logits;
  int ld, n_vocab;
  int* tokens;
  int T_max, cur_len, n_initial;
  const unsigned char* suppress_mask;
  const unsigned char* blank_mask;
  int eot, timestamp_begin;
  int apply_timestamp_rules, max_initial_timestamp_index;
  float* sum_logprob;
  int* n_done;
};
hipError_t launch_decode_select(const DecodeSelectArgs& a, int B, hipStream_t s);
hipError_t launch_token_prob(const float* logits, int ld, int n_vocab, int token, float* out, int B, hipStream_t s);
hipError_t launch_f32_to_f16(const float* in, half_t* out, size_t n, hipStream_t s);
hipError_t launch_gather_text_rows(const float* x, int n_tok_max, int d, int sot_len, const int* n_tok, const int* row_off, int B, int n_text_max,
                                   float* out, int* row_map, hipStream_t s);
hipError_t launch_token_logprob(const float* logits, long ld, int vocab_end, int rows, const int64_t* targets, const int* row_map, int tgt_off,
                                float* out, int* err, int err_bit, hipStream_t s);

struct LogMelTables {
  const float* filters;
  const int* filt_lo;
  const int* filt_hi;
  const float* window;
  const float* twiddle;
  int precise;
  int n_mels;
};
struct LogMelArgs : LogMelTables {
  const float* pcm;
  long pcm_stride;
  const int* n_samples;
  float* mel_out;
  half_t* mel_tm;
  int n_mels_pad;
  int tm_lo;
  float* scratch;
  unsigned* gmax;
  int B;
};
hipError_t launch_logmel(const LogMelArgs& a, hipStream_t s);

struct LogMelLongArgs : LogMelTables {
  const float* pcm;
  long n_samples;
  float* mel_out;
  long ld;
  long n_frames;
  unsigned* gmax;
};
hipError_t launch_logmel_long(const LogMelLongArgs& a, hipStream_t s);

hipError_t launch_mel_window(const float* mel_long, long ld, int n_mels, const int* seek, const int* size, int B, float* out, hipStream_t s);

struct HeadStatsArgs {
  const float* qk;
  long qk_bs; long qk_hs; int qk_ld;
  float* weights;
  long w_bs;
  const int* n_tok;
  const int* n_frames;
  int n_tok_max, n_frames_max;
  float* colnorm;
// ... 51 lines not shown
```

Before: 343.9.

## Store cross-attention K/V as per-layer planes and skip V in last-layer logits capture

```diff
diff --git a/include/wca.h b/include/wca.h
--- a/include/wca.h
+++ b/include/wca.h
@@ -179,6 +179,7 @@
 int wca_test_set_attn_split_drop(int mask);
 int wca_test_set_switch(const char* name, int value);
 int wca_test_last_scores(wca_engine* e, int batch, float* scores_host);
+int wca_test_last_capture(wca_engine* e, int64_t n_floats, float* cap_host);
 int wca_test_attention(wca_engine* e, const void* q_dev, const void* k_dev, const void* v_dev, void* o_dev,
                        float* cap_dev, int cap_ld, int cap_cols, int B, int H, int nq, int nk, int causal);
 int wca_test_attention_split(wca_engine* e, const void* q2_dev, const void* k2_dev, const void* v2_dev, void* o2_dev,
diff --git a/whisper-char-alignment_amd/_lib.py b/whisper-char-alignment_amd/_lib.py
--- a/whisper-char-alignment_amd/_lib.py
+++ b/whisper-char-alignment_amd/_lib.py
@@ -88,6 +88,7 @@
     "wca_test_set_attn_split_drop": (_i, [_i]),
     "wca_test_set_switch": (_i, [C.c_char_p, _i]),
     "wca_test_last_scores": (_i, [_vp, _i, _pf]),
+    "wca_test_last_capture": (_i, [_vp, _i64, _pf]),
     "wca_test_gemm_pairs": (_i, [_vp, _vp, _vp, _vp, _vp, _i, _i, _i, _i, _i]),
     "wca_test_attention": (_i, [_vp, _vp, _vp, _vp, _vp, _vp, _i, _i, _i, _i, _i, _i, _i]),
     "wca_test_attention_split": (_i, [_vp, _vp, _vp, _vp, _vp, _vp, _i, _i, _i, _i, _i, _i, _i]),
diff --git a/whisper-char-alignment_amd/csrc/attention.hip b/whisper-char-alignment_amd/csrc/attention.hip
--- a/whisper-char-alignment_amd/csrc/attention.hip
+++ b/whisper-char-alignment_amd/csrc/attention.hip
@@ -52,8 +52,9 @@
     __builtin_amdgcn_sched_barrier(0);                                                                        \
   } while (0)
 
-template <bool CAUSAL, bool CAPTURE>
+template <bool CAUSAL, bool CAPTURE, bool LOGITS = false>
 __global__ __launch_bounds__(256) void attn_kernel(AttnArgs a) {
+  static_assert(!LOGITS || (CAPTURE && !CAUSAL), "the logits-only form is a capture form without a mask");
   extern __shared__ __attribute__((aligned(16))) char smem[];
   half_t* lds = reinterpret_cast<half_t*>(smem);
   const int tid = threadIdx.x;
@@ -94,6 +95,7 @@
     const int qhi = q_blk + 128;
     nk_eff = qhi < a.nk ? qhi : a.nk;
   }
+  if (LOGITS) nk_eff = a.cap_cols < a.nk ? a.cap_cols : a.nk;
   const int nkt = (nk_eff + KT - 1) / KT;
 
   const half_t* Kb = a.K + (long)b * a.k_bs + h * 64;
@@ -111,7 +113,7 @@
       const int ck = (lane & 7) ^ swz128(r);
       const int cv = (lane & 7) ^ (r & 6);
       glds16(Kb + (long)key * a.k_rs + ck * 8, Kt + rbase * 64);
-      glds16(Vb + (long)key * a.v_rs + cv * 8, Vt + rbase * 64);
+      if (!LOGITS) glds16(Vb + (long)key * a.v_rs + cv * 8, Vt + rbase * 64);
     }
   };
 
@@ -131,7 +133,8 @@
   int slot = 0;
   for (int kt = 0; kt < nkt; ++kt) {
     if (kt + 1 < nkt) {
-      asm volatile("s_waitcnt vmcnt(4)" ::: "memory");
+      if (LOGITS) asm volatile("s_waitcnt vmcnt(2)" ::: "memory");
+      else asm volatile("s_waitcnt vmcnt(4)" ::: "memory");
     } else {
       asm volatile("s_waitcnt vmcnt(0)" ::: "memory");
     }
@@ -186,6 +189,7 @@
         }
       }
     }
+    if (LOGITS) continue;
     const bool tail_tile = (kt * KT + KT > a.nk);
     const bool diag_tile = CAUSAL && (kt * KT + KT - 1 > q_wave);
     if (tail_tile || diag_tile) {
@@ -308,6 +312,7 @@
     }
   }
 
+  if (LOGITS) return;
 #pragma unroll
   for (int s = 0; s < 2; ++s) {
     if (qrow[s] >= a.nq) continue;
@@ -681,6 +686,7 @@
   if ((a.q_rs % 8) || (a.k_rs % 8) || (a.v_rs % 8) || (a.o_rs % 4)) return hipErrorInvalidValue;
   if (a.cap != nullptr && ((a.cap_ld % 4) != 0 || a.cap_ld < ((a.cap_cols + 3) & ~3))) return hipErrorInvalidValue;
   const bool cap = a.cap != nullptr && a.cap_cols > 0;
+  if (a.logits_only && (!cap || a.causal)) return hipErrorInvalidValue;
   if (a.nq == 1 && !cap && (!a.causal || a.nk == 1)) {
     hipLaunchKernelGGL(attn_decode_kernel, dim3(a.H * a.B), dim3(256), 0, s, a);
     return hipGetLastError();
@@ -692,6 +698,10 @@
     hipLaunchKernelGGL(attn32_kernel, grid, block, shmem, s, a);
     return hipGetLastError();
   }
+  if (a.logits_only) {
+    hipLaunchKernelGGL((attn_kernel<false, true, true>), grid, block, shmem, s, a);
+    return hipGetLastError();
+  }
   if (a.causal) {
     if (cap) hipLaunchKernelGGL((attn_kernel<true, true>), grid, block, shmem, s, a);
     else hipLaunchKernelGGL((attn_kernel<true, false>), grid, block, shmem, s, a);
diff --git a/whisper-char-alignment_amd/csrc/attention_split.hip b/whisper-char-alignment_amd/csrc/attention_split.hip
--- a/whisper-char-alignment_amd/csrc/attention_split.hip
+++ b/whisper-char-alignment_amd/csrc/attention_split.hip
@@ -56,8 +56,9 @@
     __builtin_amdgcn_sched_barrier(0);                                                                                               \
   } while (0)
 
-template <bool CAUSAL, bool CAPTURE, int NW = 4>
+template <bool CAUSAL, bool CAPTURE, int NW = 4, bool LOGITS = false>
 __global__ __launch_bounds__(NW * 64, (2 * NW * 64) / 256) void attn_split_kernel(AttnArgs a) {
+  static_assert(!LOGITS || (CAPTURE && !CAUSAL), "the logits-only form is a capture form without a mask");
   extern __shared__ __attribute__((aligned(16))) char smem[];
   half_t* lds = reinterpret_cast<half_t*>(smem);
   const int tid = threadIdx.x;
@@ -105,6 +106,7 @@
     const int qhi = q_blk + QB;
     nk_eff = qhi < a.nk ? qhi : a.nk;
   }
+  if (LOGITS) nk_eff = a.cap_cols < a.nk ? a.cap_cols : a.nk;
   const int nkt = (nk_eff + KT - 1) / KT;
 
   const half_t* Kb = a.K + (long)b * a.k_bs + h * 64;
@@ -129,6 +131,7 @@
       const half_t* vp = Vb + (long)key * a.v_rs + cv * 8;
       glds16(kp, Kh + rbase * 64);
       glds16(kp + a.k_lo, Kl + rbase * 64);
+      if (LOGITS) continue;
       glds16(vp, Vh + rbase * 64);
       glds16(vp + a.v_lo, Vl + rbase * 64);
     }
@@ -225,6 +228,7 @@
         }
       }
     }
+    if (LOGITS) continue;
     const bool tail_tile = (kt * KT + KT > a.nk);
     const bool diag_tile = CAUSAL && (kt * KT + KT - 1 > q_wave);
     if (tail_tile || diag_tile) {
@@ -340,6 +344,7 @@
     }
   }
 
+  if (LOGITS) return;
 #pragma unroll
   for (int s = 0; s < 2; ++s) {
     const float l = xor32_sumf(xor16_sumf(l_part[s]));
@@ -689,6 +694,7 @@
   if ((a.q_lo % 8) || (a.k_lo % 8) || (a.v_lo % 8) || (a.o_lo % 4) || a.q_lo <= 0 || a.k_lo <= 0 || a.v_lo <= 0 || a.o_lo <= 0) return hipErrorInvalidValue;
   if (a.cap != nullptr && ((a.cap_ld % 4) != 0 || a.cap_ld < ((a.cap_cols + 3) & ~3))) return hipErrorInvalidValue;
   const bool cap = a.cap != nullptr && a.cap_cols > 0;
+  if (a.logits_only && (!cap || a.causal)) return hipErrorInvalidValue;
   const size_t shmem = 2 * 4 * TILE * sizeof(half_t);
 #define WCA_LAUNCH_AS(C, P, W)                                                                                               \
   do {                                                                                                                       \
@@ -697,6 +703,12 @@
     if (e != hipSuccess) return e;                                                                                           \
     hipLaunchKernelGGL((attn_split_kernel<C, P, W>), dim3(((a.nq + (W) * 32 - 1) / ((W) * 32)) * a.H * a.B), dim3((W) * 64), shmem, s, a); \
   } while (0)
+  if (a.logits_only) {
+    hipError_t e = hipFuncSetAttribute(reinterpret_cast<const void*>(attn_split_kernel<false, true, 4, true>), hipFuncAttributeMaxDynamicSharedMemorySize, (int)shmem);
+    if (e != hipSuccess) return e;
+    hipLaunchKernelGGL((attn_split_kernel<false, true, 4, true>), dim3(((a.nq + 127) / 128) * a.H * a.B), dim3(256), shmem, s, a);
+    return hipGetLastError();
+  }
   const int variant = a.variant ? a.variant : debug_switch(DBG_ATTN_SPLIT_VARIANT);
   if (!a.causal && !cap && a.nq >= 64 && variant != 1 && (a.o_rs % 8) == 0 && (a.o_lo % 8) == 0) {
 #define WCA_LAUNCH_A32(D)                                                                                                             \
diff --git a/whisper-char-alignment_amd/csrc/engine.hip b/whisper-char-alignment_amd/csrc/engine.hip
--- a/whisper-char-alignment_amd/csrc/engine.hip
+++ b/whisper-char-alignment_amd/csrc/engine.hip
@@ -443,9 +443,11 @@
 
 hipError_t gemm(hipStream_t s, const half_t* A, int lda, const half_t* W, int ldw, const float* bias, void* C, int ldc, int M,
                 int N, int K, int gelu, int out_mode, int site = 0, float* sk_ws = nullptr, size_t sk_bytes = 0, long c_lo = 0, long a_lo = 0,
-                wca_engine* wlo_e = nullptr, const half_t* w_plain = nullptr, int k_plain = 0) {
+                wca_engine* wlo_e = nullptr, const half_t* w_plain = nullptr, int k_plain = 0, int c_block = 0, long c_block_stride = 0) {
   GemmArgs g{};
   g.a_lo = a_lo;
+  g.c_block = c_block;
+  g.c_block_stride = c_block_stride;
   g.cu_limit = g_gemm_cu_limit;
   g.sk_part = sk_ws;
   g.sk_bytes = sk_bytes;
@@ -849,15 +851,30 @@
   return WCA_OK;
 }
 
+struct CrossKvLayout {
+  int ld;
+  long lo, plane;
+};
+CrossKvLayout cross_kv_layout(const wca_engine* e) {
+  const int dt = e->dims.n_text_state;
+  const int ld = (e->split ? 2 : 1) * dt;
+  return {ld, (long)dt, (long)e->max_batch * N_CTX * ld};
+}
+const half_t* cross_kv_plane(const wca_engine* e, const half_t* kvbuf, int p, int b0 = 0) {
+  const CrossKvLayout k = cross_kv_layout(e);
+  return kvbuf + (size_t)p * k.plane + (size_t)b0 * N_CTX * k.ld;
+}
+
 int run_cross_kv(wca_engine* e, int B, half_t* kvbuf = nullptr, bool skip_last_v = false) {
   if (!kvbuf) kvbuf = e->kv;
   const wca_model_dims& D = e->dims;
   const int d = D.n_audio_state, dt = D.n_text_state, L = D.n_text_layer;
-  const int n_cols = L * 2 * dt - (skip_last_v ? dt : 0);
+  const int n_cols = (2 * L - (skip_last_v ? 1 : 0)) * dt;
   const bool sp = e->split;
+  const CrossKvLayout k = cross_kv_layout(e);
   const GemmOpnd o = pick_operands(sp, e->kv_w, sp ? e->sw.kv_w : e->kv_w, d, B * N_CTX, n_cols, sp ? 4 : 0, e);
-  HIPCHK(gemm(e->stream, e->xn, o.lda, o.W, o.ldw, e->kv_b, kvbuf, (sp ? 2 : 1) * L * 2 * dt, B * N_CTX, n_cols, o.K, 0, 0, 3, nullptr, 0,
-              sp ? (long)L * 2 * dt : 0, o.a_lo, e, o.Wp, o.Kp));
+  HIPCHK(gemm(e->stream, e->xn, o.lda, o.W, o.ldw, e->kv_b, kvbuf, k.ld, B * N_CTX, n_cols, o.K, 0, 0, 3, nullptr, 0, sp ? k.lo : 0, o.a_lo, e, o.Wp,
+              o.Kp, dt, k.plane));
   return WCA_OK;
 }
 
@@ -867,8 +884,7 @@
   const int dt = D.n_text_state, H = D.n_text_head, L = D.n_text_layer;
   const int M = B * n;
   const float scale = 1.0f / std::sqrt((float)(dt / H));
-  const int kv_ld = 2 * L * 2 * dt;
-  const long kv_lo = (long)L * 2 * dt;
+  const CrossKvLayout kvl = cross_kv_layout(e);
   HIPCHK(launch_embed(tokens_dev, e->tok_emb, e->dec_pos, e->xd, B, n, dt, D.n_vocab, e->err_dev, s,
                       (use_wlo(e) && e->wlo_bases.count(e->tok_emb)) ? wlo_of(e, e->tok_emb) : nullptr));
   auto ln = [&](const float* g, const float* b) -> int {
@@ -915,16 +931,18 @@
       a.Q = e->q_d;
       a.q_bs = (long)n * 2 * dt;
       a.q_rs = 2 * dt;
-      a.K = kvbuf + (size_t)(2 * li) * dt;
-      a.V = kvbuf + (size_t)(2 * li + 1) * dt;
-      a.k_bs = a.v_bs = (long)N_CTX * kv_ld;
-      a.k_rs = a.v_rs = kv_ld;
+      const bool last_logits = li == L - 1 && !logits_out && !finish_last && cap != nullptr && Fcap > 0;
+      a.K = cross_kv_plane(e, kvbuf, 2 * li);
+      a.V = last_logits ? a.K : cross_kv_plane(e, kvbuf, 2 * li + 1);
+      a.k_bs = a.v_bs = (long)N_CTX * kvl.ld;
+      a.k_rs = a.v_rs = kvl.ld;
       a.O = e->att_d;
       a.o_bs = (long)n * 2 * dt;
       a.o_rs = 2 * dt;
       a.split = 1;
+      a.logits_only = last_logits ? 1 : 0;
       a.q_lo = dt;
-      a.k_lo = a.v_lo = kv_lo;
+      a.k_lo = a.v_lo = kvl.lo;
       a.o_lo = dt;
       a.cap = cap ? cap + (size_t)li * H * n * Fpad : nullptr;
       a.cap_bs = (long)L * H * n * Fpad;
@@ -990,10 +1008,12 @@
       a.Q = e->q_d;
       a.q_bs = (long)n * dt;
       a.q_rs = dt;
-      a.K = kvbuf + (size_t)(2 * li) * dt;
-      a.V = kvbuf + (size_t)(2 * li + 1) * dt;
-      a.k_bs = a.v_bs = (long)N_CTX * L * 2 * dt;
-      a.k_rs = a.v_rs = L * 2 * dt;
+      const bool last_logits = li == L - 1 && !logits_out && !finish_last && cap != nullptr && Fcap > 0;
+      a.K = cross_kv_plane(e, kvbuf, 2 * li);
+      a.V = last_logits ? a.K : cross_kv_plane(e, kvbuf, 2 * li + 1);
+      a.k_bs = a.v_bs = (long)N_CTX * dt;
+      a.k_rs = a.v_rs = dt;
+      a.logits_only = last_logits ? 1 : 0;
       a.O = e->att_d;
       a.o_bs = (long)n * dt;
       a.o_rs = dt;
@@ -1034,8 +1054,7 @@
   half_t* att_d = e->att_d + (size_t)b0 * dt;
   half_t* q_d = e->q_d + (size_t)b0 * dt;
   half_t* hid_d = e->hid_d + (size_t)b0 * 4 * dt;
-  const int kv_ld = (e->split ? 2 : 1) * L * 2 * dt;
-  const half_t* kvb = kvbuf + (size_t)b0 * N_CTX * kv_ld;
+  const int kv_ld = cross_kv_layout(e).ld;
   if (phase == -2 || phase == -1)
     HIPCHK(launch_embed_step(tokens + (size_t)b0 * T_max, T_max, t, e->tok_emb, e->dec_pos, xd, B, dt, D.n_vocab, s));
   for (int li = 0; li < L; ++li) {
@@ -1071,8 +1090,8 @@
       a.Q = q_d;
       a.q_bs = dt;
       a.q_rs = dt;
-      a.K = kvb + (size_t)(2 * li) * dt;
-      a.V = kvb + (size_t)(2 * li + 1) * dt;
+      a.K = cross_kv_plane(e, kvbuf, 2 * li, b0);
+      a.V = cross_kv_plane(e, kvbuf, 2 * li + 1, b0);
       a.k_bs = a.v_bs = (long)N_CTX * kv_ld;
       a.k_rs = a.v_rs = kv_ld;
       a.O = att_d;
@@ -1103,7 +1122,7 @@
   const float scale = 1.0f / std::sqrt((float)(dt / H));
   half_t* cache = (half_t*)e->dec_cache.p;
   const size_t plane = (size_t)B * T_max * dt;
-  const int kv_ld = (e->split ? 2 : 1) * L * 2 * dt;
+  const int kv_ld = cross_kv_layout(e).ld;
   HIPCHK(launch_embed_prefix(tokens, T_max, n, e->tok_emb, e->dec_pos, e->xd, B, dt, D.n_vocab, s));
   for (int li = 0; li < L; ++li) {
     const LayerW& l = e->dec[li];
@@ -1136,8 +1155,8 @@
       a.Q = e->q_d;
       a.q_bs = (long)n * dt;
       a.q_rs = dt;
-      a.K = kvbuf + (size_t)(2 * li) * dt;
-      a.V = kvbuf + (size_t)(2 * li + 1) * dt;
+      a.K = cross_kv_plane(e, kvbuf, 2 * li);
+      a.V = cross_kv_plane(e, kvbuf, 2 * li + 1);
       a.k_bs = a.v_bs = (long)N_CTX * kv_ld;
       a.k_rs = a.v_rs = kv_ld;
       a.O = e->att_d;
@@ -3072,6 +3091,17 @@
   return WCA_OK;
 }
 
+int wca_test_last_capture(wca_engine* e, int64_t n_floats, float* cap_host) {
+  if (!e || !cap_host) return fail(WCA_ERR_INVALID, "null argument");
+  if (e->enq_count != e->fetch_count) return fail(WCA_ERR_STATE, "fetch the batches in flight first");
+  HIPCHK(hipSetDevice(e->device));
+  if (n_floats < 1 || e->cap.bytes < (size_t)n_floats * sizeof(float)) return fail(WCA_ERR_INVALID, "no %lld captured logits are held", (long long)n_floats);
+  HIPCHK(hipStreamSynchronize(e->stream));
+  HIPCHK(hipStreamSynchronize(e->stream2));
+  HIPCHK(hipMemcpy(cap_host, e->cap.p, (size_t)n_floats * sizeof(float), hipMemcpyDeviceToHost));
+  return WCA_OK;
+}
+
 int wca_test_attention(wca_engine* e, const void* q, const void* k, const void* v, void* o, float* cap_dev, int cap_ld, int cap_cols,
                        int B, int H, int nq, int nk, int causal) {
   if (!e) return fail(WCA_ERR_INVALID, "null engine");
diff --git a/whisper-char-alignment_amd/csrc/gemm.hip b/whisper-char-alignment_amd/csrc/gemm.hip
--- a/whisper-char-alignment_amd/csrc/gemm.hip
+++ b/whisper-char-alignment_amd/csrc/gemm.hip
@@ -20,8 +20,15 @@
   return *reinterpret_cast<const half8*>(tile + r * 64 + ((c ^ swz128(r)) << 3));
 }
 
-template <int OUT_MODE, bool GELU, int MT>
+constexpr bool c_blocked(int out_mode, bool gelu, int site) { return site == 3 && !gelu && (out_mode == 0 || out_mode == 4); }
+
+template <int OUT_MODE, bool GELU, int MT, bool BLOCKED = false>
 __device__ __forceinline__ void epilogue(const GemmArgs& a, f32x4 (&acc)[MT][4], int mbase, int nb, int fr) {
+  long cn = nb;
+  if (BLOCKED && a.c_block > 0) {
+    const int plane = nb / a.c_block;
+    cn = (long)plane * a.c_block_stride + (nb - plane * a.c_block);
+  }
   float bv[16];
 #pragma unroll
   for (int j = 0; j < 16; ++j) bv[j] = (a.bias != nullptr && nb + j < a.N) ? a.bias[nb + j] : 0.f;
@@ -70,7 +77,7 @@
       coff = (long)m * a.ldc;
     }
     if (OUT_MODE == 0 || OUT_MODE == 4) {
-      half_t* cp = reinterpret_cast<half_t*>(a.C) + coff + nb;
+      half_t* cp = reinterpret_cast<half_t*>(a.C) + coff + cn;
       if (full_n && ((reinterpret_cast<uintptr_t>(cp) & 15) == 0)) {
         half8 h0, h1, l0, l1;
         if (OUT_MODE == 4) {
@@ -234,7 +241,7 @@
     epilogue<1, false, 4>(p, acc, m0 + wm * 64, n0 + wn * 64 + fg * 16, fr);
     return;
   }
-  epilogue<OUT_MODE, GELU, 4>(a, acc, m0 + wm * 64, n0 + wn * 64 + fg * 16, fr);
+  epilogue<OUT_MODE, GELU, 4, c_blocked(OUT_MODE, GELU, SITE)>(a, acc, m0 + wm * 64, n0 + wn * 64 + fg * 16, fr);
 }
 
 __global__ __launch_bounds__(256) void splitk_reduce_kernel(const float* __restrict__ part, int S, int M, int N, const float* __restrict__ bias,
@@ -367,7 +374,7 @@
     __builtin_amdgcn_s_setprio(0);
   }
 
-  epilogue<OUT_MODE, GELU, 8>(a, acc, m0 + wr * 128, n0 + wc * 64 + fg * 16, fr);
+  epilogue<OUT_MODE, GELU, 8, c_blocked(OUT_MODE, GELU, SITE)>(a, acc, m0 + wr * 128, n0 + wc * 64 + fg * 16, fr);
 }
 
 template <int V>
@@ -607,7 +614,7 @@
         epilogue_ln<KernArgs>(*ap, acc, m0, m0 >> 8, n0 >> 8, ntn, wr, wc, fr_e, fg_e, bias_lds + par * 256 + wc * 64, gamma_lds + par * 256,
                               beta_lds + par * 256, ln_lds);
       else
-        epilogue_wide<OUT_MODE, GELU, KernArgs>(*ap, acc, m0 + wr * 128, n0 + wc * 64, fr_e, fg_e, bias_lds + par * 256 + wc * 64);
+        epilogue_wide<OUT_MODE, GELU, KernArgs, c_blocked(OUT_MODE, GELU, SITE)>(*ap, acc, m0 + wr * 128, n0 + wc * 64, fr_e, fg_e, bias_lds + par * 256 + wc * 64);
     }
     if (!has_next) break;
     par ^= 1;
@@ -742,6 +749,8 @@
   if (a.K <= 0 || (a.K % BK) != 0) return hipErrorInvalidValue;
   if ((a.lda % 8) != 0 || (a.ldw % 8) != 0) return hipErrorInvalidValue;
   if (a.out_mode == 4 && (a.c_lo <= 0 || (a.c_lo & 7))) return hipErrorInvalidValue;
+  if (a.c_block != 0 && (a.c_block < 0 || (a.c_block % 64) != 0 || (a.c_block_stride & 7) != 0 || a.site != 3 || a.gelu || (a.out_mode != 0 && a.out_mode != 4)))
+    return hipErrorInvalidValue;
   if (a.addend != nullptr && (a.out_mode == 2 || a.out_mode == 3 || a.a_lo > 0)) return hipErrorInvalidValue;
   if ((a.force_tile == 64 || a.force_tile == 0) && a.M <= 64 && (a.K % 512) == 0 && a.a_rows_per_batch == 0 && a.pos == nullptr && a.addend == nullptr && a.out_mode != 4 && a.a_lo <= 0) {
     const dim3 sgrid((unsigned)((a.N + 15) / 16)), sblock(256);
diff --git a/whisper-char-alignment_amd/csrc/gemm_epilogue.h b/whisper-char-alignment_amd/csrc/gemm_epilogue.h
--- a/whisper-char-alignment_amd/csrc/gemm_epilogue.h
+++ b/whisper-char-alignment_amd/csrc/gemm_epilogue.h
@@ -4,7 +4,7 @@
 
 namespace wca {
 
-template <int OUT_MODE, bool GELU, typename ArgsT>
+template <int OUT_MODE, bool GELU, typename ArgsT, bool BLOCKED = false>
 __device__ __forceinline__ void epilogue_wide(const ArgsT& a, f32x4 (&acc)[8][4], int mbase, int nbase, int fr, int fg, const float* bias_l) {
   int col[4];
 #pragma unroll
@@ -17,6 +17,11 @@
     for (int r = 0; r < 4; ++r) bv[nt * 4 + r] = b4[r];
   }
   const bool full_n = (nbase + 64 <= a.N);
+  long cn = nbase;
+  if (BLOCKED && a.c_block > 0) {
+    const int plane = nbase / a.c_block;
+    cn = (long)plane * a.c_block_stride + (nbase - plane * a.c_block);
+  }
   if (OUT_MODE == 2) {
     float* cbase = reinterpret_cast<float*>(a.C) + nbase;
     if (full_n && a.pos == nullptr && (a.ldc & 3) == 0 && (a.c_batch_stride & 3) == 0 && ((reinterpret_cast<uintptr_t>(cbase + fg * 4) & 15) == 0)) {
@@ -100,7 +105,7 @@
       coff = (long)m * a.ldc;
     }
     if (OUT_MODE == 0 || OUT_MODE == 4) {
-      half_t* cp = reinterpret_cast<half_t*>(a.C) + coff + nbase;
+      half_t* cp = reinterpret_cast<half_t*>(a.C) + coff + cn;
       if (full_n && ((reinterpret_cast<uintptr_t>(cp + fg * 8) & 15) == 0)) {
 #pragma unroll
         for (int hh = 0; hh < 2; ++hh) {
diff --git a/whisper-char-alignment_amd/csrc/kernels.h b/whisper-char-alignment_amd/csrc/kernels.h
--- a/whisper-char-alignment_amd/csrc/kernels.h
+++ b/whisper-char-alignment_amd/csrc/kernels.h
@@ -24,6 +24,8 @@
   int c_rows_per_batch;
   long c_batch_stride;
   long c_lo;
+  int c_block;
+  long c_block_stride;
   const float* addend;
   int ld_addend;
   const float* pos;
@@ -76,6 +78,7 @@
   float scale;
   int causal;
   int variant;
+  int logits_only;
   int split;
   long q_lo, k_lo, v_lo, o_lo;
 };
```

After: 344.5, median of 4. About the same (+0.2%).
